# HITRainer/EAVSR

Measured on AMD Instinct MI355X. Metric: SR frames/sec at 4x 7-frame 180x320->720x1280, higher is better.
Workload: dtype f32

## Files before the change

### eavsr_amd/_native.py

```python
from __future__ import annotations

import ctypes as C
import os
import threading

_HERE = os.path.dirname(os.path.abspath(__file__))
LIB_PATH = os.environ.get("EAVSR_LIB_PATH") or os.path.join(
    _HERE, "lib", "libeavsr_lab.so" if os.environ.get("EAVSR_BUILD_LAB", "0") == "1" else "libeavsr_hip.so")

ABI_VERSION = 32

p_f32 = C.c_void_p
i32 = C.c_int32
i64 = C.c_int64
f32 = C.c_float
vp = C.c_void_p


class ConvDesc(C.Structure):
    _fields_ = [
        ("src", vp * 5),
        ("src_c", i32 * 5),
        ("n_src", i32),
        ("ksize", i32),
        ("weight_packed", vp),
        ("bias", vp),
        ("residual", vp),
        ("out", vp),
        ("chan_partial", vp),
        ("n", i32), ("h", i32), ("w", i32), ("cin", i32), ("cout", i32),
        ("act", i32),
        ("slope", f32),
        ("ca_scale", vp),
        ("ca_x", vp),
        ("ca_out", vp),
        ("out_shuffle", i32),
        ("res_scale", vp),
        ("border_pieces", vp),
        ("border_stride", i32),
        ("sum_mul", vp),
    ]


SIGNATURES = {
    "eavsr_abi_version": (C.c_int, []),
    "eavsr_version": (C.c_char_p, []),
    "eavsr_conv2d_desc_size": (C.c_size_t, []),
    "eavsr_lab_build": (C.c_int, []),
    "eavsr_last_error": (C.c_char_p, []),
    "eavsr_selftest_mfma_f32": (C.c_int, [vp, vp]),
    "eavsr_flow_warp_f32": (C.c_int, [vp, vp, vp, vp, i32, i32, i32, i32, i32, i32, vp]),
    "eavsr_flow_warp_pair_f32": (C.c_int, [vp, vp, vp, vp, vp, vp, i32, i32, i32, i32, i32, vp]),
    "eavsr_dcnv2_f32": (C.c_int, [vp, vp, vp, vp, vp, vp, i32, i32, i32, i32, i32, i32, vp]),
    "eavsr_dcnv2_generic_f32": (C.c_int, [vp] * 6 + [i32] * 15 + [vp]),
    "eavsr_dcn_weight_x9_bytes": (C.c_int64, [i32, i32]),
    "eavsr_pack_dcn_weight_x9": (C.c_int, [vp, vp, i32, i32, vp]),
    "eavsr_nchw_to_il8_f32": (C.c_int, [vp, vp, i32, i32, i32, i32, vp]),
    "eavsr_dcnv2_il_f32": (C.c_int, [vp, vp, vp, vp, vp, vp, i32, i32, i32, i32, i32, i32, i32, i32, vp]),
    "eavsr_dcn_weight_il2_bytes": (C.c_int64, [i32, i32]),
    "eavsr_pack_dcn_weight_il2": (C.c_int, [vp, vp, i32, i32, vp]),
    "eavsr_dcnv2_il2_f32": (C.c_int, [vp, vp, vp, vp, vp, vp, i32, i32, i32, i32, i32, i32, i32, i32, vp]),
    "eavsr_dcn_il16_weight_bytes": (C.c_int64, [i32, i32]),
    "eavsr_pack_dcn_il16_weight": (C.c_int, [vp, vp, i32, i32, i32, vp]),
    "eavsr_nchw_to_il8_h16": (C.c_int, [vp, vp, i32, i32, i32, i32, i32, vp]),
    "eavsr_dcnv2_il16": (C.c_int, [vp, vp, vp, vp, vp, vp, i32, i32, i32, i32, i32, i32, i32, i32, vp]),
    "eavsr_wino4_schedule": (C.c_int, []),
    "eavsr_conv3x3_wino4_border_pieces": (C.c_int, [i32, i32, C.POINTER(i32), C.POINTER(i32)]),
    "eavsr_ca_scale_pre_pieces": (C.c_int, [vp, vp, i32, vp, i32, i32, i32, vp, vp, vp, vp, vp, vp, vp, i32, i32, i32, i32, i32, vp]),
    "eavsr_conv2d_f32": (C.c_int, [C.POINTER(ConvDesc), vp]),
    "eavsr_wino4_weight_elems": (C.c_int64, [i32, i32]),
    "eavsr_pack_conv_weight_wino4": (C.c_int, [vp, vp, i32, i32, vp]),
    "eavsr_conv3x3_wino4_tiles": (i32, [i32, i32]),
    "eavsr_conv3x3_wino4_f32": (C.c_int, [vp, vp, vp]),
    "eavsr_wgrad3_mode": (C.c_int, []),
    "eavsr_conv3x3_x6s_tiles": (i32, [i32, i32]),
    "eavsr_conv3x3_f32x6s": (C.c_int, [vp, vp, vp]),
    "eavsr_pack_conv_weight_wino5x5": (C.c_int, [vp, vp, i32, i32, vp]),
    "eavsr_conv5x5_wino_tiles": (i32, [i32, i32]),
    "eavsr_conv5x5_wino_f32": (C.c_int, [vp, vp, vp]),
    "eavsr_conv2d_ck": (i32, [i32]),
    "eavsr_conv2d_tile_rows": (i32, [i32, i32, i32, i32]),
    "eavsr_conv2d_tiles": (i32, [i32, i32, i32, i32]),
    "eavsr_route_batch": (i32, [i32]),
    "eavsr_packed_weight_elems": (i64, [i32, i32, i32]),
    "eavsr_pack_conv_weight_f32": (C.c_int, [vp, vp, i32, i32, i32, vp]),
    "eavsr_conv3x3_smallco_f32": (C.c_int, [vp, vp, vp, vp, vp, i32, i32, i32, i32, i32, i32, f32, vp]),
    "eavsr_smallco_packed_elems": (C.c_int64, [i32, i32]),
    "eavsr_pack_smallco_weight": (C.c_int, [vp, vp, i32, i32, vp]),
    "eavsr_conv3x3_smallco_lite_f32": (C.c_int, [vp, vp, vp, vp, vp, i32, i32, i32, i32, i32, i32, f32, vp]),
    "eavsr_conv_weight_x6_bytes": (C.c_size_t, [i32, i32, i32]),
    "eavsr_pack_conv_weight_x6": (C.c_int, [vp, vp, i32, i32, i32, vp]),
    "eavsr_pack_conv_weight_x6_dgrad": (C.c_int, [vp, vp, i32, i32, i32, vp]),
    "eavsr_pack_conv_weight_x6_multi": (C.c_int, [vp, vp, vp, i32, i32, i32, vp]),
    "eavsr_conv_f32x6": (C.c_int, [vp, vp, vp, vp, i32, i32, i32, i32, i32, i32, i32, f32, i32, vp]),
    "eavsr_ca_scale_f32": (C.c_int, [vp, i32, i32, vp, vp, vp, vp, vp, i32, i32, i32, vp]),
    "eavsr_ca_scale_mean_f32": (C.c_int, [vp, i32, i32, vp, vp, vp, vp, vp, vp, i32, i32, i32, vp]),
    "eavsr_scale_residual_f32": (C.c_int, [vp, vp, vp, vp, i32, i32, i32, vp]),
    "eavsr_ca_tail_f32": (C.c_int, [vp, vp, i32, vp, vp, vp, vp, vp, vp, i32, i32, i32, i32, vp]),
    "eavsr_ca_tail_stats_f32": (C.c_int, [vp, vp, i32, vp, vp, vp, vp, vp, vp, vp, vp, i32, i32, i32, i32, vp]),
    "eavsr_adapt_frontend_f32": (C.c_int, [vp, vp, vp, vp, vp, vp, vp, i32, i32, i32, i32, vp]),
    "eavsr_affine_offsets_f32": (C.c_int, [vp, vp, vp, i32, i32, i32, i32, vp]),
    "eavsr_resize_bilinear_ac_f32": (C.c_int, [vp, vp, vp, vp, i32, i32, i32, i32, i32, i32, f32, vp]),
    "eavsr_pyramid_f32": (C.c_int, [vp, vp, vp, i32, i32, i32, vp]),
    "eavsr_add_f32": (C.c_int, [vp, vp, vp, vp, i64, vp]),
    "eavsr_normalize_f32": (C.c_int, [vp, vp, vp, vp, i32, i32, i32, vp]),
    "eavsr_avg_pool2_f32": (C.c_int, [vp, vp, i32, i32, i32, vp]),
    "eavsr_resize_bilinear_f32": (C.c_int, [vp, vp, i32, i32, i32, i32, i32, i32, i32, f32, f32, vp]),
    "eavsr_concat3_f32": (C.c_int, [vp, i32, vp, i32, vp, i32, vp, i32, i32, vp]),
    "eavsr_act_bwd_f32": (C.c_int, [vp, vp, vp, i64, i32, f32, vp]),
    "eavsr_plane_sum_f32": (C.c_int, [vp, vp, vp, i32, i32, f32, vp]),
    "eavsr_channel_sum_f32": (C.c_int, [vp, vp, i32, i32, i32, i32, vp]),
    "eavsr_channel_sum_multi_f32": (C.c_int, [vp, i32, vp, i32, i32, i32, i32, vp]),
    "eavsr_scale_residual_bwd_f32": (C.c_int, [vp, vp, vp, vp, i32, i32, i32, vp]),
    "eavsr_rcab_tail_bwd_f32": (C.c_int, [vp] * 13 + [i32] * 7 + [vp]),
    "eavsr_ca_mlp_bwd_f32": (C.c_int, [vp] * 11 + [i32, i32, i32, vp]),
    "eavsr_flow_warp_bwd_f32": (C.c_int, [vp] * 6 + [i32, i32, i32, i32, vp]),
    "eavsr_resize_bilinear_ac_bwd_f32": (C.c_int, [vp, vp, i32, i32, i32, i32, i32, i32, f32, vp]),
    "eavsr_pyramid_bwd_f32": (C.c_int, [vp, vp, vp, i32, i32, i32, vp]),
    "eavsr_affine_offsets_bwd_f32": (C.c_int, [vp, vp, vp, vp, i32, i32, i32, i32, vp]),
    "eavsr_conv_wgrad_blocks": (i32, [i32, i32, i32, i32]),
    "eavsr_conv_wgrad_f32": (C.c_int, [vp, vp, vp, vp] + [i32] * 11 + [vp]),
    "eavsr_conv_wgrad_multi_f32": (C.c_int, [vp, vp, i32, vp, vp] + [i32] * 11 + [vp]),
    "eavsr_conv_wgrad_span_f32": (C.c_int, [vp, vp, vp, vp] + [i32] * 9 + [vp]),
# ... 136 lines not shown
```

### eavsr_amd/csrc/common.h

```cpp
#pragma once
#include <hip/hip_runtime.h>
#include <stdint.h>
#include <stddef.h>

#include <mutex>

#include "../../include/eavsr_hip.h"

#ifndef EAVSR_LAB
#define EAVSR_LAB 0
#endif

namespace eavsr {

void set_error(const char* fmt, ...);
void clear_error();
int launch_status(const char* what);

static inline hipStream_t as_stream(void* s) { return reinterpret_cast<hipStream_t>(s); }

static inline int cdiv(int a, int b) { return (a + b - 1) / b; }

constexpr int kMaxDevices = 64;
struct PerDeviceOnce {
  std::once_flag flag[kMaxDevices];
};
static inline int current_device() {
  int d = 0;
  (void)hipGetDevice(&d);
  return (d >= 0 && d < kMaxDevices) ? d : 0;
}

}

#define EAVSR_REQUIRE(cond, code, ...)      \
  do {                                      \
    if (!(cond)) {                          \
      ::eavsr::set_error(__VA_ARGS__);      \
      return (code);                        \
    }                                       \
  } while (0)

typedef float f32x16 __attribute__((ext_vector_type(16)));
typedef float f32x4 __attribute__((ext_vector_type(4)));

#ifdef __HIPCC__
__device__ __forceinline__ int eavsr_xcd_remap(int bid, int nblk) {
  const int q = nblk >> 3, r = nblk & 7;
  const int xcd = bid & 7, pos = bid >> 3;
  const int base = xcd < r ? xcd * (q + 1) : r * (q + 1) + (xcd - r) * q;
  return base + pos;
}
#endif

#ifdef __HIPCC__
__device__ __forceinline__ void eavsr_stagger_priority(int wave) {
#if defined(EAVSR_PRIO_LOW_HALF)
  if (wave < 4) __builtin_amdgcn_s_setprio(3);
#elif !defined(EAVSR_NO_WAVE_PRIO)
  if (wave >= 4) __builtin_amdgcn_s_setprio(3);
#else
  (void)wave;
#endif
}
#endif


#ifdef __HIPCC__
__device__ __forceinline__ float eavsr_sigmoid_fast(float x) { return __builtin_amdgcn_rcpf(1.f + __expf(-x)); }

__device__ __forceinline__ float eavsr_mul_legacy(float a, float b) {
  float r;
  asm("v_mul_legacy_f32 %0, %1, %2" : "=v"(r) : "v"(a), "v"(b));
  return r;
}

__device__ __forceinline__ float eavsr_act(float v, float act_s) {
  const float z = eavsr_mul_legacy(v, act_s);
  return !(v <= 0.f) ? v : z;
}
#endif

#define EAVSR_CONV_TW 32
```

### eavsr_amd/csrc/conv3_h16.hip

```cpp
#include "common.h"

#include <hip/hip_bf16.h>
#include <mutex>

namespace {

typedef const __attribute__((address_space(1))) void* gptr_t;
typedef __attribute__((address_space(3))) void* lptr_t;
typedef unsigned u32x4 __attribute__((ext_vector_type(4)));
typedef __bf16 bf16x8 __attribute__((ext_vector_type(8)));
typedef _Float16 h16x8 __attribute__((ext_vector_type(8)));

constexpr int G_TH = 16, G_TW = 32, G_CO = 64, G_CK = 16;
constexpr int G_IH = G_TH + 2;
constexpr int G_QW = 10;
constexpr int G_IW = G_TW + 2;
constexpr int G_PLANE_B = G_IH * G_IW * 16;
constexpr int G_PATCH_B = 2 * G_PLANE_B;
constexpr int G_W_B = 9 * 2 * G_CO * 16;
constexpr int G_STAGE_B = G_PATCH_B + G_W_B;
constexpr int G_LDS_BYTES = 2 * G_STAGE_B + G_CO * 4;
constexpr int G_UNITS = 2 * G_IH * G_QW;

struct G16Args {
// ... 137 lines not shown
    }
    asm volatile("s_waitcnt vmcnt(0) lgkmcnt(0)" ::: "memory");
    __syncthreads();
  }

  const float act_s = a.act == EAVSR_ACT_NONE ? 1.f : a.act == EAVSR_ACT_RELU ? 0.f : a.slope;
  const int gx = x0 + l31;
  if (gx < w) {
#pragma unroll
    for (int t = 0; t < 2; ++t) {
      const int gy = y0 + 2 * wave + t;
      if (gy < h) {
#pragma unroll
        for (int m = 0; m < 2; ++m)
#pragma unroll
          for (int e = 0; e < 16; ++e) {
            const int co = cot * G_CO + m * 32 + (e & 3) + 8 * (e >> 2) + 4 * half;
            if (co < a.cout) {
              const float v = acc[m][t][e];
              a.out[((size_t)bn * a.cout + co) * plane + (size_t)gy * w + gx] = eavsr_act(v, act_s);
            }
          }
      }
    }
  }
}

template <bool BF16>
__global__ void pack_weight_h16g_kernel(const float* __restrict__ w, unsigned short* __restrict__ p, int cout, int cin, long total) {
  const long i = (long)blockIdx.x * 256 + threadIdx.x;
  if (i >= total) return;
  const int j = (int)(i & 7), co = (int)((i >> 3) & 63), hf = (int)((i >> 9) & 1);
  long r = i >> 10;
  const int tap = (int)(r % 9);
  r /= 9;
  const int nch = cin / G_CK;
  const int ch = (int)(r % nch), cot = (int)(r / nch);
  const int o = cot * G_CO + co, ci = ch * G_CK + hf * 8 + j;
  const float v = o < cout ? w[((size_t)o * cin + ci) * 9 + tap] : 0.f;
  p[i] = BF16 ? __builtin_bit_cast(unsigned short, __float2bfloat16(v)) : __builtin_bit_cast(unsigned short, (_Float16)v);
}

template <bool BF16>
int launch_h16g(const G16Args& a, dim3 grid, hipStream_t st) {
  static eavsr::PerDeviceOnce once_pd;
  const int dev_ = eavsr::current_device();
  static hipError_t attr_err_pd[eavsr::kMaxDevices] = {};
  hipError_t& attr_err = attr_err_pd[dev_];
  std::call_once(once_pd.flag[dev_], [&] {
    attr_err = hipFuncSetAttribute(reinterpret_cast<const void*>(&conv3x3_h16g_kernel<BF16>),
                                   hipFuncAttributeMaxDynamicSharedMemorySize, G_LDS_BYTES);
  });
  if (attr_err != hipSuccess) {
    eavsr::set_error("conv3x3_h16g: hipFuncSetAttribute: %s", hipGetErrorString(attr_err));
    return (int)attr_err;
  }
  hipLaunchKernelGGL(conv3x3_h16g_kernel<BF16>, grid, dim3(512), G_LDS_BYTES, st, a);
  return eavsr::launch_status("conv3x3_h16g");
}

}

extern "C" int64_t eavsr_conv3x3_h16g_weight_bytes(int32_t cout, int32_t cin) {
  if (cout <= 0 || cin <= 0 || cin % G_CK) return -1;
  return (int64_t)eavsr::cdiv(cout, G_CO) * (cin / G_CK) * G_W_B;
}

extern "C" int eavsr_pack_conv3x3_h16g(const float* weight, void* packed, int32_t cout, int32_t cin, int32_t dtype, void* stream) {
  EAVSR_REQUIRE(weight && packed, -1, "pack_conv3x3_h16g: NULL pointer");
  EAVSR_REQUIRE(dtype == 1 || dtype == 2, -1, "pack_conv3x3_h16g: dtype %d (1 = f16, 2 = bf16)", dtype);
  EAVSR_REQUIRE(cout > 0 && cin > 0 && cin % G_CK == 0, -2, "pack_conv3x3_h16g: cin %d must be a multiple of 16", cin);
  const long total = eavsr_conv3x3_h16g_weight_bytes(cout, cin) / 2;
  hipStream_t st = eavsr::as_stream(stream);
  const unsigned blocks = (unsigned)((total + 255) / 256);
  if (dtype == 2) hipLaunchKernelGGL(pack_weight_h16g_kernel<true>, dim3(blocks), dim3(256), 0, st, weight, (unsigned short*)packed, cout, cin, total);
  else hipLaunchKernelGGL(pack_weight_h16g_kernel<false>, dim3(blocks), dim3(256), 0, st, weight, (unsigned short*)packed, cout, cin, total);
  return eavsr::launch_status("pack_conv3x3_h16g");
}

extern "C" int eavsr_conv3x3_h16g_f32(const eavsr_conv2d_desc* d, int32_t dtype, void* stream) {
  EAVSR_REQUIRE(d && d->out && d->weight_packed, -1, "conv3x3_h16g: NULL pointer");
  EAVSR_REQUIRE(dtype == 1 || dtype == 2, -1, "conv3x3_h16g: dtype %d (1 = f16, 2 = bf16)", dtype);
  EAVSR_REQUIRE(d->ksize == 3 && d->n_src >= 1 && d->n_src <= 5, -2, "conv3x3_h16g: 3x3, 1..5 sources");
  EAVSR_REQUIRE(!d->residual && !d->chan_partial && !d->ca_scale && !d->ca_x && !d->ca_out && d->out_shuffle == 0 && !d->res_scale && !d->border_pieces && !d->sum_mul, -2,
                "conv3x3_h16g: plain convolution only (no residual / channel sums / channel-attention prologue / pixel shuffle)");
  EAVSR_REQUIRE(d->n >= 0 && d->h > 0 && d->w > 0 && d->cout > 0 && d->w % 4 == 0, -2, "conv3x3_h16g: bad dims (w %% 4 == 0)");
  int cin = 0;
  G16Args a;
  for (int i = 0; i < 5; ++i) {
    a.src[i] = i < d->n_src ? d->src[i] : nullptr;
    a.src_c[i] = i < d->n_src ? d->src_c[i] : 0;
    if (i < d->n_src) {
      EAVSR_REQUIRE(d->src[i] && d->src_c[i] > 0 && d->src_c[i] % G_CK == 0, -2, "conv3x3_h16g: source %d: %d channels (multiples of 16)", i, d->src_c[i]);
      EAVSR_REQUIRE(((uintptr_t)d->src[i] & 15) == 0, -2, "conv3x3_h16g: sources must be 16-byte aligned");
      cin += d->src_c[i];
    }
  }
  EAVSR_REQUIRE(cin == d->cin, -1, "conv3x3_h16g: cin %d != sum of the sources %d", d->cin, cin);
  if (d->n == 0) return 0;
  a.n_src = d->n_src; a.wp = d->weight_packed; a.bias = d->bias; a.out = d->out;
  a.n = d->n; a.h = d->h; a.w = d->w; a.cin = cin; a.cout = d->cout;
  a.tiles_x = eavsr::cdiv(d->w, G_TW);
  a.tiles_y = eavsr::cdiv(d->h, G_TH);
  a.act = d->act; a.slope = d->slope;
  const long blocks = (long)a.tiles_x * a.tiles_y * d->n;
  EAVSR_REQUIRE(blocks < (1L << 31), -1, "conv3x3_h16g: too many tiles");
  dim3 grid((unsigned)blocks, (unsigned)eavsr::cdiv(d->cout, G_CO));
  return dtype == 2 ? launch_h16g<true>(a, grid, eavsr::as_stream(stream)) : launch_h16g<false>(a, grid, eavsr::as_stream(stream));
}
```

### eavsr_amd/csrc/conv3_x6s.hip

```cpp
#include "common.h"

#include <mutex>

namespace {

typedef const __attribute__((address_space(1))) void* gptr_t;
typedef __attribute__((address_space(3))) void* lptr_t;
typedef unsigned u32x4 __attribute__((ext_vector_type(4)));
typedef __bf16 bf16x8 __attribute__((ext_vector_type(8)));

constexpr int Q_NW = 8, Q_TW = 32, Q_TH = 8;
constexpr int Q_IW = Q_TW + 2, Q_IH = Q_TH + 2, Q_NPIX = Q_IW * Q_IH;
constexpr int Q_PLANE_B = Q_NPIX * 16;
constexpr int Q_KSTEPS = 5;

template <int NCH, int NP> struct QCfg {
  static constexpr int CHUNK_B = NP * Q_PLANE_B;
  static constexpr int SLAB_U4 = Q_KSTEPS * NP * 64;
  static constexpr int PATCH_B = NCH * CHUNK_B;
  static constexpr size_t LDS_BYTES = (size_t)PATCH_B + 2 * (size_t)SLAB_U4 * 16 + 32 * 4 + Q_NW * 32 * 4;
  static_assert(LDS_BYTES <= 160 * 1024, "LDS");
  static_assert(PATCH_B >= Q_NW * 32 * 36 * 4, "the VEC epilogue's transpose tiles live in the patch region");
};

// ... 376 lines not shown
      sum = v;
      a.out[obase + (size_t)cu * plane] = a.act == EAVSR_ACT_RELU_MASK ? (rr[r] > 0.f ? v : 0.f) : v + rr[r];
    }
    if (a.chan_partial) {
      sum += __shfl_xor(sum, 16);
      sum += __shfl_xor(sum, 8);
      sum += __shfl_xor(sum, 4);
      sum += __shfl_xor(sum, 2);
      sum += __shfl_xor(sum, 1);
      if (l31 == 0) s_red[wave * 32 + cu + 4 * kg] = sum;
    }
  }
#ifdef EAVSR_X6S_STAMPS
  Q_STAMP(4);
  asm volatile("s_waitcnt vmcnt(0)" ::: "memory");
  Q_STAMP(5);
  if (tid == 0)
    for (int i = 0; i < 8; ++i) atomicAdd(&g_q_stamps[i], st_acc[i]);
#endif
  if (a.chan_partial) {
    __syncthreads();
    if (tid < 32) {
      const int co = cot * 32 + tid;
      if (co < a.cout) {
        float v = s_red[tid];
#pragma unroll
        for (int k = 1; k < Q_NW; ++k) v += s_red[k * 32 + tid];
        a.chan_partial[((size_t)bn * (a.tiles_x * a.tiles_y) + ty * a.tiles_x + tx) * a.cout + co] = v;
      }
    }
  }
}

template <int NCH, bool VEC, int NP>
int launch_q(const QArgs& a, void* stream, const char* name) {
  using K = QCfg<NCH, NP>;
  static eavsr::PerDeviceOnce once_pd;
  const int dev_ = eavsr::current_device();
  static hipError_t attr_err_pd[eavsr::kMaxDevices] = {};
  hipError_t& attr_err = attr_err_pd[dev_];
  std::call_once(once_pd.flag[dev_], [&] {
    attr_err = hipFuncSetAttribute(reinterpret_cast<const void*>(&conv3x3_x6s_kernel<NCH, VEC, NP>), hipFuncAttributeMaxDynamicSharedMemorySize,
                                   (int)K::LDS_BYTES);
  });
  if (attr_err != hipSuccess) {
    eavsr::set_error("%s: hipFuncSetAttribute(%zu B of LDS): %s", name, K::LDS_BYTES, hipGetErrorString(attr_err));
    return (int)attr_err;
  }
  const long blocks = (long)a.tiles_x * a.tiles_y * a.n;
  EAVSR_REQUIRE(blocks < (1L << 31), -1, "%s: too many tiles", name);
  dim3 grid((unsigned)blocks, eavsr::cdiv(a.cout, 32));
  hipLaunchKernelGGL((conv3x3_x6s_kernel<NCH, VEC, NP>), grid, dim3(64 * Q_NW), K::LDS_BYTES, eavsr::as_stream(stream), a);
  return eavsr::launch_status(name);
}

}

#ifdef EAVSR_X6S_STAMPS
extern "C" int eavsr_debug_x6s_stamps(unsigned long long* host_out, int reset) {
  hipError_t e = hipMemcpyFromSymbol(host_out, HIP_SYMBOL(g_q_stamps), sizeof(unsigned long long) * 8);
  if (e != hipSuccess) return (int)e;
  if (reset) {
    unsigned long long z[8] = {0, 0, 0, 0, 0, 0, 0, 0};
    e = hipMemcpyToSymbol(HIP_SYMBOL(g_q_stamps), z, sizeof(z));
  }
  return (int)e;
}
#endif

extern "C" int32_t eavsr_conv3x3_x6s_tiles(int32_t h, int32_t w) {
  if (h <= 0 || w <= 0) return 0;
  return eavsr::cdiv(h, Q_TH) * eavsr::cdiv(w, Q_TW);
}

namespace {

int q_args(const eavsr_conv2d_desc* d, const void* wpacked, const char* name, QArgs& a, bool& vec) {
  EAVSR_REQUIRE(d && wpacked, -1, "%s: NULL pointer", name);
  EAVSR_REQUIRE(d->ksize == 3 && d->n_src == 1 && d->src_c[0] == d->cin, -2, "%s: one source, 3x3", name);
  EAVSR_REQUIRE(d->cin == 64, -2, "%s: cin %d (64 only; use eavsr_conv2d_f32)", name, d->cin);
  EAVSR_REQUIRE(d->n >= 0 && d->cout > 0 && d->h > 0 && d->w > 0, -1, "%s: bad dims", name);
  if (d->n == 0) return 1;
  EAVSR_REQUIRE(d->src[0] && d->out, -1, "%s: NULL pointer", name);
  EAVSR_REQUIRE(d->ca_scale == nullptr && d->ca_x == nullptr && d->ca_out == nullptr && d->out_shuffle == 0 && d->res_scale == nullptr && d->border_pieces == nullptr, -2,
                "%s: no channel-attention prologue, no pixel-shuffle store", name);
  EAVSR_REQUIRE(d->act >= 0 && d->act <= EAVSR_ACT_RELU_MASK, -1, "%s: act %d", name, d->act);
  EAVSR_REQUIRE(d->act != EAVSR_ACT_LRELU || (d->slope >= 0.f && d->slope <= 1.f), -2,
                "%s: leaky-ReLU slope %g outside [0, 1] (the epilogue evaluates max(v, slope v))", name, (double)d->slope);
  EAVSR_REQUIRE(d->act != EAVSR_ACT_RELU_MASK || (d->residual != nullptr && d->chan_partial == nullptr), -1,
                "%s: EAVSR_ACT_RELU_MASK takes the mask source in `residual` (no channel sums)", name);
  EAVSR_REQUIRE(d->sum_mul == nullptr || d->act != EAVSR_ACT_RELU_MASK, -1, "%s: sum_mul with EAVSR_ACT_RELU_MASK", name);
  EAVSR_REQUIRE((long)d->h * d->w < (1L << 31), -1, "%s: image plane too large for 32-bit pixel offsets", name);
  a.x = d->src[0]; a.wsplit = reinterpret_cast<const u32x4*>(wpacked); a.bias = d->bias; a.residual = d->residual;
  a.out = d->out; a.chan_partial = d->chan_partial; a.sum_mul = d->sum_mul;
  a.n = d->n; a.cout = d->cout; a.h = d->h; a.w = d->w;
  a.tiles_x = eavsr::cdiv(d->w, Q_TW); a.tiles_y = eavsr::cdiv(d->h, Q_TH);
  a.wmt = d->cout > 32 ? 2 : 1;
  a.act = d->act; a.slope = d->slope;
  vec = d->w % 4 == 0 && ((reinterpret_cast<uintptr_t>(a.x) | reinterpret_cast<uintptr_t>(a.out) |
                           reinterpret_cast<uintptr_t>(a.residual)) & 15) == 0;
  EAVSR_REQUIRE(a.sum_mul == nullptr || (a.chan_partial != nullptr && vec && (reinterpret_cast<uintptr_t>(a.sum_mul) & 15) == 0), -2,
                "%s: sum_mul needs chan_partial, w %% 4 == 0 and 16-byte aligned tensors", name);
  return 0;
}

}

extern "C" int eavsr_conv3x3_f32x6s(const eavsr_conv2d_desc* d, const void* weight_x6, void* stream) {
  QArgs a;
  bool vec = false;
  const int rc = q_args(d, weight_x6, "conv3x3_f32x6s", a, vec);
  if (rc) return rc > 0 ? 0 : rc;
#ifdef EAVSR_X6S_NO_VEC
  return launch_q<8, false, 3>(a, stream, "conv3x3_f32x6s");
#endif
  return vec ? launch_q<8, true, 3>(a, stream, "conv3x3_f32x6s") : launch_q<8, false, 3>(a, stream, "conv3x3_f32x6s");
}

extern "C" int eavsr_conv3x3_bf16x1s(const eavsr_conv2d_desc* d, const void* weight_bf16x1, void* stream) {
  QArgs a;
  bool vec = false;
  const int rc = q_args(d, weight_bf16x1, "conv3x3_bf16x1s", a, vec);
  if (rc) return rc > 0 ? 0 : rc;
  return vec ? launch_q<8, true, 1>(a, stream, "conv3x3_bf16x1s") : launch_q<8, false, 1>(a, stream, "conv3x3_bf16x1s");
}
```

### eavsr_amd/csrc/conv_mfma.hip

```cpp
#include "common.h"

#include <atomic>
#include <mutex>

namespace {

struct ConvArgs {
  const float* src[5];
  int src_c[5];
  int n_src;
  const float* wp;
  const float* bias;
  const float* residual;
  float* out;
  float* chan_partial;
  const float* ca_scale;
  const float* ca_x;
  float* ca_out;
  int n, h, w, cin, cout, cin_pad, tiles_x, tiles_y;
  int act;
  float slope;
};

__device__ float g_zero_word[4];
// ... 512 lines not shown
  static hipError_t attr_err_pd[eavsr::kMaxDevices] = {};
  hipError_t& attr_err = attr_err_pd[dev_];
  std::call_once(once, [&] {
    attr_err = hipFuncSetAttribute(reinterpret_cast<const void*>(&conv2d_mfma_kernel<KS, MT, VEC, FUSE, NT_>),
                                   hipFuncAttributeMaxDynamicSharedMemorySize, (int)Cfg::LDS_BYTES);
  });
  if (attr_err != hipSuccess) {
    eavsr::set_error("conv2d: hipFuncSetAttribute(%zu B of LDS): %s", Cfg::LDS_BYTES, hipGetErrorString(attr_err));
    return (int)attr_err;
  }
  hipLaunchKernelGGL((conv2d_mfma_kernel<KS, MT, VEC, FUSE, NT_>), grid, dim3(64 * Cfg::NW), Cfg::LDS_BYTES, st, a);
  return eavsr::launch_status("conv2d");
}

template <int KS, int NT_>
int launch_ks(const ConvArgs& a, dim3 grid, int CO, bool vec, hipStream_t st) {
  if (vec) return CO == 32 ? launch_one<KS, 1, true, false, NT_>(a, grid, st) : launch_one<KS, 2, true, false, NT_>(a, grid, st);
  return CO == 32 ? launch_one<KS, 1, false, false, NT_>(a, grid, st) : launch_one<KS, 2, false, false, NT_>(a, grid, st);
}

std::atomic<int> g_route_batch{0};

inline int tile_rows_of(int n, int h, int w, int ksize) {
  if (ksize == 7) return 4;
  const int routed = g_route_batch.load(std::memory_order_relaxed);
  if (routed > 0) n = routed;
  int best = 4;
  long best_cost = -1;
  for (int nt = 4; nt >= 1; nt >>= 1) {
    const long tiles = (long)n * eavsr::cdiv(h, 8 * nt) * eavsr::cdiv(w, EAVSR_CONV_TW);
    const long rounds = (tiles + 255) / 256;
    const long cost = rounds * (2 * nt + 1);
    if (best_cost < 0 || cost < best_cost) { best_cost = cost; best = nt; }
  }
  return best;
}

template <int KS>
int launch_nt(const ConvArgs& a, dim3 grid, int CO, bool vec, int nt, hipStream_t st) {
  if (nt == 1) return launch_ks<KS, 1>(a, grid, CO, vec, st);
  if (nt == 2) return launch_ks<KS, 2>(a, grid, CO, vec, st);
  return launch_ks<KS, 4>(a, grid, CO, vec, st);
}

}

extern "C" int32_t eavsr_conv2d_ck(int32_t ksize) { return chunk_of(ksize); }

extern "C" int32_t eavsr_route_batch(int32_t n) { return g_route_batch.exchange(n > 0 ? n : 0, std::memory_order_relaxed); }

extern "C" int32_t eavsr_conv2d_tile_rows(int32_t n, int32_t h, int32_t w, int32_t ksize) {
  return 8 * tile_rows_of(n > 0 ? n : 1, h, w, ksize);
}

extern "C" int32_t eavsr_conv2d_tiles(int32_t n, int32_t h, int32_t w, int32_t ksize) {
  return eavsr::cdiv(h, eavsr_conv2d_tile_rows(n, h, w, ksize)) * eavsr::cdiv(w, EAVSR_CONV_TW);
}

extern "C" int64_t eavsr_packed_weight_elems(int32_t cout, int32_t cin, int32_t ksize) {
  if (cout <= 0 || cin <= 0 || !(ksize == 1 || ksize == 3 || ksize == 5 || ksize == 7)) return -1;
  const int CO = co_tile_of(cout), ck = chunk_of(ksize);
  const int64_t cots = eavsr::cdiv(cout, CO), cin_pad = (int64_t)eavsr::cdiv(cin, ck) * ck;
  return cots * cin_pad * ksize * ksize * CO;
}

extern "C" int eavsr_pack_conv_weight_f32(const float* weight, float* packed, int32_t cout, int32_t cin,
                                          int32_t ksize, void* stream) {
  EAVSR_REQUIRE(weight && packed, -1, "pack_conv_weight: NULL pointer");
  const int64_t total = eavsr_packed_weight_elems(cout, cin, ksize);
  EAVSR_REQUIRE(total > 0, -1, "pack_conv_weight: bad shape cout=%d cin=%d k=%d", cout, cin, ksize);
  const int CO = co_tile_of(cout), ck = chunk_of(ksize);
  const int cin_pad = eavsr::cdiv(cin, ck) * ck;
  hipLaunchKernelGGL(pack_weight_kernel, dim3((unsigned)((total + 255) / 256)), dim3(256), 0,
                     eavsr::as_stream(stream), weight, packed, cout, cin, ksize * ksize, cin_pad, CO, (long)total);
  return eavsr::launch_status("pack_conv_weight");
}

extern "C" int eavsr_conv2d_f32(const eavsr_conv2d_desc* d, void* stream) {
  EAVSR_REQUIRE(d != nullptr, -1, "conv2d: NULL descriptor");
  EAVSR_REQUIRE(d->n_src >= 1 && d->n_src <= 5, -1, "conv2d: n_src %d not in 1..5", d->n_src);
  EAVSR_REQUIRE(d->ksize == 1 || d->ksize == 3 || d->ksize == 5 || d->ksize == 7, -2,
                "conv2d: kernel size %d unsupported (1,3,5,7)", d->ksize);
  EAVSR_REQUIRE(d->weight_packed && d->out, -1, "conv2d: NULL weight/out");
  EAVSR_REQUIRE(d->out_shuffle == 0 && d->res_scale == nullptr && d->border_pieces == nullptr && d->sum_mul == nullptr, -2, "conv2d: the pixel-shuffle and scaled-residual epilogues exist in eavsr_conv3x3_wino4_f32 only");
  EAVSR_REQUIRE(d->n >= 0 && d->h > 0 && d->w > 0 && d->cin > 0 && d->cout > 0, -1, "conv2d: bad dims");
  EAVSR_REQUIRE(d->act >= 0 && d->act <= EAVSR_ACT_RELU_MASK, -1, "conv2d: act %d", d->act);
  EAVSR_REQUIRE(d->act != EAVSR_ACT_RELU_MASK || (d->residual != nullptr && d->chan_partial == nullptr && d->ca_scale == nullptr), -1,
                "conv2d: EAVSR_ACT_RELU_MASK takes the mask source in `residual` (no channel sums, no fused prologue)");
  EAVSR_REQUIRE(d->act != EAVSR_ACT_LRELU || (d->slope >= 0.f && d->slope <= 1.f), -2,
                "conv2d: leaky-ReLU slope %g outside [0, 1] (the epilogue evaluates max(v, slope v))", (double)d->slope);
  const int ck = chunk_of(d->ksize);
  ConvArgs a;
  int csum = 0;
  for (int s = 0; s < 5; ++s) {
    a.src[s] = s < d->n_src ? d->src[s] : nullptr;
    a.src_c[s] = s < d->n_src ? d->src_c[s] : 0;
    if (s < d->n_src) {
      EAVSR_REQUIRE(d->src[s] != nullptr && d->src_c[s] > 0, -1, "conv2d: source %d is empty", s);
      EAVSR_REQUIRE(s == d->n_src - 1 || d->src_c[s] % ck == 0, -2,
                    "conv2d: source %d has %d channels, not a multiple of %d (only the last may be ragged)", s,
                    d->src_c[s], ck);
      csum += d->src_c[s];
    }
  }
  EAVSR_REQUIRE(csum == d->cin, -1, "conv2d: sources sum to %d channels, cin = %d", csum, d->cin);
  if (d->n == 0) return 0;
  const int CO = co_tile_of(d->cout);
  a.n_src = d->n_src;
  a.wp = d->weight_packed;
  a.bias = d->bias;
  a.residual = d->residual;
  a.out = d->out;
  a.chan_partial = d->chan_partial;
  a.ca_scale = d->ca_scale;
  a.ca_x = d->ca_x;
  a.ca_out = d->ca_out;
  a.n = d->n; a.h = d->h; a.w = d->w; a.cin = d->cin; a.cout = d->cout;
  a.cin_pad = eavsr::cdiv(d->cin, ck) * ck;
  const int nt = tile_rows_of(d->n, d->h, d->w, d->ksize);
  a.tiles_x = eavsr::cdiv(d->w, EAVSR_CONV_TW);
  a.tiles_y = eavsr::cdiv(d->h, 8 * nt);
  a.act = d->act;
  a.slope = d->slope;
  const long blocks = (long)a.tiles_x * a.tiles_y * d->n;
  EAVSR_REQUIRE(blocks < (1L << 31), -1, "conv2d: too many tiles");
  EAVSR_REQUIRE((long)d->h * d->w * 16 < (1L << 31), -1, "conv2d: image plane too large for 32-bit tile offsets");
  dim3 grid((unsigned)blocks, eavsr::cdiv(d->cout, CO));
  hipStream_t st = eavsr::as_stream(stream);
  bool vec = (d->w % 4) == 0;
  for (int s = 0; s < d->n_src; ++s)
    vec = vec && (((uintptr_t)d->src[s]) & 15) == 0 && (d->src_c[s] % ck) == 0;
  if (d->ca_scale != nullptr) {
    EAVSR_REQUIRE(d->ca_x != nullptr, -1, "conv2d: ca_scale without ca_x");
    EAVSR_REQUIRE(d->ksize == 3 && d->n_src == 1 && vec && (((uintptr_t)d->ca_x) & 15) == 0 && d->cin % 4 == 0 &&
                      d->cin <= 256 && CO == 64 && d->cout <= 64,
                  -2, "conv2d: the fused channel-attention prologue needs a single 16-byte aligned source, k = 3, "
                      "w %% 4 == 0, cin %% 4 == 0, cin <= 256 and 33..64 output channels; use eavsr_scale_residual_f32 + "
                      "a plain conv otherwise");
    EAVSR_REQUIRE(nt == 4, -2, "conv2d: the fused channel-attention prologue exists for the 32-row tile only "
                               "(this problem size runs %d-row tiles)", 8 * nt);
    return launch_one<3, 2, true, true>(a, grid, st);
  }
  EAVSR_REQUIRE(d->ca_x == nullptr && d->ca_out == nullptr, -1, "conv2d: ca_x / ca_out without ca_scale");
  switch (d->ksize) {
    case 1: return launch_nt<1>(a, grid, CO, vec, nt, st);
    case 3:
      if (nt == 1 && vec) {
        if (CO == 32) return launch_small<1>(a, grid, st);
        if (blocks * grid.y <= 128) return launch_small<1, true>(a, grid, st);
        return launch_small<2>(a, grid, st);
      }
      return launch_nt<3>(a, grid, CO, vec, nt, st);
    case 5: return launch_nt<5>(a, grid, CO, vec, nt, st);
    default: return launch_ks<7, 4>(a, grid, CO, vec, st);
  }
}
```

### eavsr_amd/csrc/conv_wino.hip

```cpp
#include "common.h"

#include <mutex>

namespace {

typedef const __attribute__((address_space(1))) void* gptr_t;
typedef __attribute__((address_space(3))) void* lptr_t;
typedef float f32x2 __attribute__((ext_vector_type(2)));

__device__ __attribute__((aligned(16))) float g_wino_zero[4];

struct WnArgs {
  const float* src[5];
  int src_c[5];
  int n_src;
  const float* wu;
  const float* bias;
  const float* residual;
  float* out;
  float* chan_partial;
  const float* ca_scale;
  const float* ca_x;
  float* ca_out;
  int n, h, w, cin, cout, tiles_x, tiles_y;
// ... 291 lines not shown
    }
    if (a.chan_partial) {
      __syncthreads();
#pragma unroll
      for (int r = 0; r < 4; ++r) {
        float v = csum[r];
        v += __shfl_xor(v, 8);
        v += __shfl_xor(v, 4);
        v += __shfl_xor(v, 2);
        v += __shfl_xor(v, 1);
        if (l15 == 0) s_red[(wave & 1) * 64 + cb * 16 + 4 * kq + r] = v;
      }
      __syncthreads();
      if (tid < 64) {
        const int co = cot * 64 + tid;
        if (co < a.cout)
          a.chan_partial[((size_t)bn * (a.tiles_x * a.tiles_y) + tile_lin) * a.cout + co] = s_red[tid] + s_red[64 + tid];
      }
    }
#pragma unroll
    for (int b = 0; b < 2; ++b)
#pragma unroll
      for (int x = 0; x < 16; ++x) acc[b][x] = f32x4{0.f, 0.f, 0.f, 0.f};
    if (it + 1 < total_iters) {
      tile_coords((it + 1) / total_chunks, bn, y0, x0, tile_lin);
      if (FUSE) {
        for (int c = tid; c < a.cin; c += 64 * NW) s_y[c] = a.ca_scale[(size_t)bn * a.cin + c];
      }
    }
  }
  }
}


__global__ void pack_wino_kernel(const float* __restrict__ wt, float* __restrict__ out, int cout, int cin, long total) {
  const long e = (long)blockIdx.x * 256 + threadIdx.x;
  if (e >= total) return;
  const int col = (int)(e & 63);
  long u = e >> 6;
  const int c = (int)(u % CK); u /= CK;
  const int xi = (int)(u % 16); u /= 16;
  const int nchunks = cin / CK;
  const int chunk = (int)(u % nchunks);
  const int cot = (int)(u / nchunks);
  const int co = cot * 64 + col, ci = chunk * CK + c;
  float v = 0.f;
  if (co < cout) {
    const float* g = wt + ((size_t)co * cin + ci) * 9;
    const int r = xi >> 2, q = xi & 3;
    float gr[3];
#pragma unroll
    for (int j = 0; j < 3; ++j) {
      const float g0 = g[0 * 3 + j], g1 = g[1 * 3 + j], g2 = g[2 * 3 + j];
      gr[j] = r == 0 ? g0 : (r == 1 ? 0.5f * (g0 + g1 + g2) : (r == 2 ? 0.5f * (g0 - g1 + g2) : g2));
    }
    v = q == 0 ? gr[0] : (q == 1 ? 0.5f * (gr[0] + gr[1] + gr[2]) : (q == 2 ? 0.5f * (gr[0] - gr[1] + gr[2]) : gr[2]));
  }
  out[e - col + (col ^ ((c & 1) << 4))] = v;
}

}

extern "C" int64_t eavsr_wino_weight_elems(int32_t cout, int32_t cin) {
  if (cout <= 0 || cin <= 0 || cin % CK != 0) return 0;
  return (int64_t)eavsr::cdiv(cout, 64) * (cin / CK) * UV;
}

extern "C" int eavsr_pack_conv_weight_wino(const float* weight, float* packed, int32_t cout, int32_t cin, void* stream) {
  EAVSR_REQUIRE(weight && packed, -1, "pack_conv_weight_wino: NULL pointer");
  EAVSR_REQUIRE(cout > 0 && cin > 0 && cin % CK == 0, -1, "pack_conv_weight_wino: cin %d must be a multiple of 8", cin);
  const long total = eavsr_wino_weight_elems(cout, cin);
  hipLaunchKernelGGL(pack_wino_kernel, dim3((unsigned)((total + 255) / 256)), dim3(256), 0, eavsr::as_stream(stream), weight, packed,
                     cout, cin, total);
  return eavsr::launch_status("pack_conv_weight_wino");
}

extern "C" int32_t eavsr_conv3x3_wino_tiles(int32_t h, int32_t w) { return eavsr::cdiv(h, TOH) * eavsr::cdiv(w, TOW); }

extern "C" int eavsr_conv3x3_wino_f32(const eavsr_conv2d_desc* d, const float* weight_wino, void* stream) {
  EAVSR_REQUIRE(d != nullptr && weight_wino != nullptr, -1, "conv3x3_wino: NULL descriptor / weights");
  EAVSR_REQUIRE(d->n_src >= 1 && d->n_src <= 5, -1, "conv3x3_wino: n_src %d not in 1..5", d->n_src);
  EAVSR_REQUIRE(d->ksize == 3, -2, "conv3x3_wino: kernel size %d (3 only)", d->ksize);
  EAVSR_REQUIRE(d->out, -1, "conv3x3_wino: NULL out");
  EAVSR_REQUIRE(d->out_shuffle == 0 && d->res_scale == nullptr && d->border_pieces == nullptr && d->sum_mul == nullptr, -2, "conv3x3_wino: the pixel-shuffle and scaled-residual epilogues exist in eavsr_conv3x3_wino4_f32 only");
  EAVSR_REQUIRE(d->n >= 0 && d->h > 0 && d->w > 0 && d->cin > 0 && d->cout > 0, -1, "conv3x3_wino: bad dims");
  EAVSR_REQUIRE(d->act >= 0 && d->act <= 2, -1, "conv3x3_wino: act %d", d->act);
  EAVSR_REQUIRE(d->act != EAVSR_ACT_LRELU || (d->slope >= 0.f && d->slope <= 1.f), -2,
                "conv3x3_wino: leaky-ReLU slope %g outside [0, 1] (the epilogue evaluates max(v, slope v))", (double)d->slope);
  const bool fuse = d->ca_scale != nullptr;
  if (fuse) {
    EAVSR_REQUIRE(d->ca_x != nullptr, -1, "conv3x3_wino: ca_scale without ca_x");
    EAVSR_REQUIRE(d->n_src == 1 && d->cin <= F_MAXC && (((uintptr_t)d->ca_x) & 15) == 0 &&
                      (d->ca_out == nullptr || (((uintptr_t)d->ca_out) & 7) == 0), -2,
                  "conv3x3_wino: the fused channel-attention prologue needs a single source, cin <= %d and aligned ca_x / "
                  "ca_out", F_MAXC);
  } else {
    EAVSR_REQUIRE(d->ca_x == nullptr && d->ca_out == nullptr, -1, "conv3x3_wino: ca_x / ca_out without ca_scale");
  }
  EAVSR_REQUIRE(d->w % 4 == 0, -2, "conv3x3_wino: w %% 4 != 0 (use eavsr_conv2d_f32)");
  EAVSR_REQUIRE((((uintptr_t)d->out) & 7) == 0 && (d->residual == nullptr || (((uintptr_t)d->residual) & 7) == 0), -2,
                "conv3x3_wino: out / residual must be 8-byte aligned");
  WnArgs a;
  int csum = 0;
  for (int s = 0; s < 5; ++s) {
    a.src[s] = s < d->n_src ? d->src[s] : nullptr;
    a.src_c[s] = s < d->n_src ? d->src_c[s] : 0;
    if (s < d->n_src) {
      EAVSR_REQUIRE(d->src[s] != nullptr && d->src_c[s] > 0 && d->src_c[s] % CK == 0 && (((uintptr_t)d->src[s]) & 15) == 0, -2,
                    "conv3x3_wino: source %d must be 16-byte aligned with a multiple of 8 channels", s);
      csum += d->src_c[s];
    }
  }
  EAVSR_REQUIRE(csum == d->cin, -1, "conv3x3_wino: sources sum to %d channels, cin = %d", csum, d->cin);
  if (d->n == 0) return 0;
  a.n_src = d->n_src;
  a.wu = weight_wino;
  a.bias = d->bias; a.residual = d->residual; a.out = d->out; a.chan_partial = d->chan_partial;
  a.ca_scale = d->ca_scale; a.ca_x = d->ca_x; a.ca_out = d->ca_out;
  a.n = d->n; a.h = d->h; a.w = d->w; a.cin = d->cin; a.cout = d->cout;
  a.tiles_x = eavsr::cdiv(d->w, TOW);
  a.tiles_y = eavsr::cdiv(d->h, TOH);
  a.act = d->act; a.slope = d->slope;
  const long blocks = (long)a.tiles_x * a.tiles_y * d->n;
  EAVSR_REQUIRE(blocks < (1L << 31), -1, "conv3x3_wino: too many tiles");
  EAVSR_REQUIRE((long)d->h * d->w * 16 < (1L << 31), -1, "conv3x3_wino: image plane too large for 32-bit tile offsets");
  static eavsr::PerDeviceOnce once_pd;
  const int dev_ = eavsr::current_device();
  std::once_flag& once = once_pd.flag[dev_];
  static hipError_t attr_err_pd[eavsr::kMaxDevices] = {};
  hipError_t& attr_err = attr_err_pd[dev_];
  std::call_once(once, [&] {
    attr_err = hipFuncSetAttribute(reinterpret_cast<const void*>(&conv3x3_wino_kernel<false>),
                                   hipFuncAttributeMaxDynamicSharedMemorySize, (int)LDS_BYTES);
    if (attr_err == hipSuccess)
      attr_err = hipFuncSetAttribute(reinterpret_cast<const void*>(&conv3x3_wino_kernel<true>),
                                     hipFuncAttributeMaxDynamicSharedMemorySize, (int)F_LDS_BYTES);
  });
  if (attr_err != hipSuccess) {
    eavsr::set_error("conv3x3_wino: hipFuncSetAttribute(%zu B of LDS): %s", LDS_BYTES, hipGetErrorString(attr_err));
    return (int)attr_err;
  }
  const long per_cot = blocks < 256 ? blocks : 256;
  dim3 grid((unsigned)per_cot, eavsr::cdiv(d->cout, 64));
  if (fuse) hipLaunchKernelGGL(conv3x3_wino_kernel<true>, grid, dim3(64 * NW), F_LDS_BYTES, eavsr::as_stream(stream), a);
  else hipLaunchKernelGGL(conv3x3_wino_kernel<false>, grid, dim3(64 * NW), LDS_BYTES, eavsr::as_stream(stream), a);
  return eavsr::launch_status("conv3x3_wino");
}
```

### eavsr_amd/csrc/conv_wino6.hip

```cpp
#include "common.h"

#ifdef EAVSR_W4_REG_WEIGHTS
#define EAVSR_W4_UREGS 1
#endif
#ifndef EAVSR_W4_ROUND2_DUTY
#define EAVSR_W4_DUTY_NO_U 1
#define EAVSR_W4_DUTYPRIO 1
#endif

#include <mutex>
#include <type_traits>
#include <cstdlib>
#include <cstring>

namespace {

static bool w6_grouped_schedule() {
#ifdef EAVSR_W4_NOGRP
  return false;
#else
  static const bool on = [] { const char* e = getenv("EAVSR_W4_GRP"); return e == nullptr || atoi(e) != 0; }();
  return on;
#endif
}

typedef const __attribute__((address_space(1))) void* gptr_t;
typedef __attribute__((address_space(3))) void* lptr_t;
typedef float f32x2 __attribute__((ext_vector_type(2)));

__device__ __attribute__((aligned(16))) float g_wino4_zero[4];

typedef __amdgpu_buffer_rsrc_t w6_rsrc;
constexpr unsigned W6_OOB = 0x80000000u;
__device__ __forceinline__ w6_rsrc w6_make_rsrc(const void* base, unsigned bytes) {
  return __builtin_amdgcn_make_buffer_rsrc(const_cast<void*>(base), 0, (int)bytes, 0x00020000);
}
__device__ __forceinline__ f32x4 w6_ld4(w6_rsrc r, unsigned voff, unsigned soff) {
  return __builtin_bit_cast(f32x4, __builtin_amdgcn_raw_buffer_load_b128(r, voff, soff, 0));
}
__device__ __forceinline__ void w6_st4(w6_rsrc r, unsigned voff, unsigned off, f32x4 v) {
  typedef unsigned u32x4_t __attribute__((ext_vector_type(4)));
  __builtin_amdgcn_raw_buffer_store_b128(__builtin_bit_cast(u32x4_t, v), r, voff + off, 0, 0);
}

struct W4Args {
  const float* src[5];
  int src_c[5];
  int n_src;
  const float* wu;
  const float* bias;
  const float* residual;
  float* out;
  float* chan_partial;
  const float* ca_scale;
  const float* ca_x;
  float* ca_out;
  int n, h, w, cin, cout, tiles_x, tiles_y;
  int act;
  float slope;
  int out_shuffle;
  const float* res_scale;
  float* border;
  int border_stride;
};

constexpr int CK = 4, NW = 8, NPOS = 36;
constexpr int MARG = 4;
constexpr int U_ELEMS = NPOS * CK * 64;
constexpr int U_SEGS = U_ELEMS / 256;
constexpr int U_IT = (U_SEGS + NW - 1) / NW;
constexpr int V_ELEMS = NPOS * CK * 32;

__host__ __device__ constexpr int w6_pair_of(int q) { return (q == 1 || q == 2) ? 0 : (q == 3 || q == 4) ? 1 : 2; }
__host__ __device__ constexpr int w6_half_of(int q) { return (q == 1 || q == 3 || q == 0) ? 0 : 1; }
__host__ __device__ constexpr int w6_slot(int i, int q) { return 2 * (3 * i + w6_pair_of(q)) + w6_half_of(q); }
__host__ __device__ constexpr int w6_col_of(int pp, int half) { return pp == 0 ? 1 + half : pp == 1 ? 3 + half : (half ? 5 : 0); }

template <int R>
struct WCfg {
  static_assert(R == 3 || R == 5, "F(4x4,3x3) or F(2x2,5x5)");
  static constexpr int M = 7 - R, PADR = R / 2;
  static constexpr int TOH = 2 * M, TOW = 16 * M;
  static constexpr int IH = TOH + 2 * PADR, IW = TOW + 2 * MARG;
  static constexpr int IN_ELEMS = CK * IH * IW;
  static constexpr int IN_SEGS = (IN_ELEMS / 4 + 63) / 64;
  static constexpr int IN_PAD = IN_SEGS * 256;
  static constexpr int IN_IT = (IN_SEGS + NW - 1) / NW;
  static constexpr int OFF_U = 2 * IN_PAD;
  static constexpr int OFF_V = OFF_U + 2 * U_ELEMS;
  static constexpr int LDS_MAIN = OFF_V + 2 * V_ELEMS;
#ifdef EAVSR_W4_ITSTAMP
  static constexpr int LDS_FLOATS = LDS_MAIN + 128 + 512;
#else
  static constexpr int LDS_FLOATS = LDS_MAIN + 128;
#endif
  static constexpr size_t LDS_BYTES = (size_t)LDS_FLOATS * sizeof(float);
};

template <typename T>
__device__ __forceinline__ void in1d(const T (&d)[6], T (&t)[6]) {
  const T a = d[4] - 4.f * d[2];
  const T b = d[3] - 4.f * d[1];
  const T c = d[4] - d[2];
  const T e = d[3] - d[1];
  t[0] = 4.f * d[0] + (d[4] - 5.f * d[2]);
  t[1] = a + b;
  t[2] = a - b;
  t[3] = c + 2.f * e;
  t[4] = c - 2.f * e;
  t[5] = 4.f * d[1] + (d[5] - 5.f * d[3]);
}

__device__ __forceinline__ void out1d(const float (&m)[6], float (&s)[4]) {
  const float p1 = m[1] + m[2], p2 = m[1] - m[2], p3 = m[3] + m[4], p4 = m[3] - m[4];
  s[0] = m[0] + p1 + p3;
  s[1] = p2 + 2.f * p4;
  s[2] = p1 + 4.f * p3;
  s[3] = (p2 + 8.f * p4) + m[5];
}

#ifdef EAVSR_W4_STAMPS
__device__ unsigned long long g_w4_stamps[32];
#define W4_STAMP(i)                                                   \
  do {                                                                \
    const unsigned long long t_ = __builtin_amdgcn_s_memtime();       \
    st_acc[i] += t_ - st_last;                                        \
    st_last = t_;                                                     \
  } while (0)
#else
#define W4_STAMP(i) do { } while (0)
#endif

#ifdef EAVSR_W4_TIMELINE
__device__ unsigned long long g_w4_tl[512 * 16];
#define W4_TL(i)                                                                           \
  do {                                                                                     \
    if (tid == 0) {                                                                        \
      g_w4_tl[(blockIdx.y * gridDim.x + blockIdx.x) * 16 + 2 * (i)] = __builtin_amdgcn_s_memrealtime(); \
      g_w4_tl[(blockIdx.y * gridDim.x + blockIdx.x) * 16 + 2 * (i) + 1] = __builtin_amdgcn_s_memtime(); \
    }                                                                                      \
  } while (0)
#else
#define W4_TL(i) do { } while (0)
#endif

#ifdef EAVSR_W4_ITSTAMP
__device__ unsigned long long g_w4_it[256 * 256];
#define W4_IT(i)                                                                                       \
  do {                                                                                                 \
    if (it >= 8 && it < 12 && lane == 0) s_its[((it - 8) * 8 + wave) * 8 + (i)] = __builtin_amdgcn_s_memtime(); \
  } while (0)
#else
#define W4_IT(i) do { } while (0)
#endif

template <int R, bool FUSE = false, bool GRP = false, bool RSC = false>
__global__ __launch_bounds__(512, 2) void conv_wino6_kernel(W4Args a) {
  static_assert(!RSC || (GRP && R == 3 && !FUSE), "the scaled-residual epilogue exists for the grouped 3x3 kernel");
  static_assert(!FUSE || R == 3, "the fused channel-attention prologue exists for the 3x3 kernel");
  static_assert(!GRP || (R == 3 && !FUSE), "the grouped schedule exists for the plain 3x3 kernel");
  using C = WCfg<R>;
  constexpr int M = C::M, PADR = C::PADR, TOH = C::TOH, TOW = C::TOW, IH = C::IH, IW = C::IW, IN_ELEMS = C::IN_ELEMS;
  constexpr int IN_SEGS = C::IN_SEGS, IN_PAD = C::IN_PAD, IN_IT = C::IN_IT;
  constexpr int X_OFF = 2 * IN_PAD;
  constexpr int OFF_U = C::OFF_U + (FUSE ? 2 * IN_PAD : 0), OFF_V = C::OFF_V + (FUSE ? 2 * IN_PAD : 0);
  constexpr int LDS_MAIN = C::LDS_MAIN + (FUSE ? 2 * IN_PAD : 0);
  extern __shared__ __attribute__((aligned(16))) float smem[];
  float* s_v = smem + OFF_V;
  float* s_red = smem + LDS_MAIN;
#ifdef EAVSR_W4_ITSTAMP
  unsigned long long* s_its = reinterpret_cast<unsigned long long*>(smem + LDS_MAIN + 128);
#endif

  const int tid = threadIdx.x;
  const int lane = tid & 63;
  const int wave = __builtin_amdgcn_readfirstlane(tid >> 6);
  W4_TL(0);
#ifndef EAVSR_W4_UREGS
  {
    const char* usrc0 = reinterpret_cast<const char*>(a.wu + (size_t)blockIdx.y * (a.cin / CK) * U_ELEMS) + wave * 1024;
#pragma unroll
    for (int i = 0; i < U_IT; ++i) {
      const int seg = i * NW + wave;
      if (seg < U_SEGS)
        __builtin_amdgcn_global_load_lds((gptr_t)(usrc0 + i * (NW * 1024) + (tid & 63) * 16u), (lptr_t)(smem + OFF_U + seg * 256), 16, 0, 0);
    }
  }
#endif

  const int cot = blockIdx.y;
  const int h = a.h, w = a.w;
  const size_t plane = (size_t)h * w;
  const int total_tiles = a.tiles_x * a.tiles_y * a.n;
  const int my_tiles = (total_tiles - (int)blockIdx.x + (int)gridDim.x - 1) / (int)gridDim.x;
  const unsigned u_tx = (unsigned)a.tiles_x, u_ty = (unsigned)a.tiles_y;
  auto tile_coords = [&](int k, int& bn_, int& y0_, int& x0_, int& lin_) __attribute__((always_inline)) {
    unsigned t = (unsigned)eavsr_xcd_remap((int)blockIdx.x + k * (int)gridDim.x, total_tiles);
    const unsigned q1 = t / u_tx;
    const unsigned tx_ = t - q1 * u_tx;
    const unsigned q2 = q1 / u_ty;
    const unsigned ty_ = q1 - q2 * u_ty;
    bn_ = (int)q2;
    y0_ = (int)ty_ * TOH;
    x0_ = (int)tx_ * TOW;
    lin_ = (int)(ty_ * u_tx + tx_);
  };

  const int l15 = lane & 15, kq = lane >> 4;
  const unsigned lane16 = lane * 16u;
  const int cb = wave >> 1, tg = wave & 1;
  eavsr_stagger_priority(wave);
#ifdef EAVSR_W4_DUTYPRIO
  if (wave >= 4) __builtin_amdgcn_s_setprio(1);
#endif
  float bias_r[4];
#pragma unroll
  for (int r = 0; r < 4; ++r) {
    const int co = cot * 64 + cb * 16 + 4 * kq + r;
    bias_r[r] = (co < a.cout && a.bias != nullptr) ? a.bias[co] : 0.f;
  }
  f32x4 acc[NPOS];
#pragma unroll
  for (int x = 0; x < NPOS; ++x) acc[x] = f32x4{0.f, 0.f, 0.f, 0.f};
  const float act_s = a.act == EAVSR_ACT_NONE ? 1.f : a.act == EAVSR_ACT_RELU ? 0.f : a.slope;

  int total_chunks = 0;
  for (int s = 0; s < a.n_src; ++s) total_chunks += a.src_c[s] / CK;
  const int total_iters = my_tiles * total_chunks;

  int p_k = 0, p_cs = 0, p_cc0 = 0, p_bn = 0, p_y0 = 0, p_x0 = 0, p_lin = 0;
  unsigned voff[IN_IT];
  auto p_setup_lanes = [&]() __attribute__((always_inline)) {
#pragma unroll
    for (int i = 0; i < IN_IT; ++i) {
      const int seg = i * NW + wave;
      const int e4 = seg * 64 + lane;
      const int ci = e4 / (IH * (IW / 4));
      const int rem = e4 - ci * (IH * (IW / 4));
      const int r = rem / (IW / 4);
      const int c4 = rem - r * (IW / 4);
// ... 150 lines not shown
        for (int r = 0; r < 6; ++r) d[r] = f32x2{q[r][0], q[r][1]};
        in1d(d, t12);
#pragma unroll
        for (int r = 0; r < 6; ++r) d[r] = f32x2{q[r][2], q[r][3]};
        in1d(d, t34);
      }
      {
        f32x2 d[6];
        if constexpr (HAND_READS) {
          asm volatile("s_waitcnt lgkmcnt(0)" : "+v"(e05[0]), "+v"(e05[1]), "+v"(e05[2]), "+v"(e05[3]), "+v"(e05[4]), "+v"(e05[5]));
#pragma unroll
          for (int r = 0; r < 6; ++r) d[r] = e05[r];
        } else {
#pragma unroll
          for (int r = 0; r < 6; ++r) d[r] = f32x2{pp[r * IW + 3], pp[r * IW + 8]};
        }
        if (FUSE) {
#pragma unroll
          for (int r = 0; r < 6; ++r) {
            d[r].x = fmaf(d[r].x, sc_use, pp[X_OFF + r * IW + 3]);
            d[r].y = fmaf(d[r].y, sc_use, pp[X_OFF + r * IW + 8]);
          }
        }
        in1d(d, t05);
      }
    } else {
      const float* pp = smem + ps * IN_PAD + kq * (IH * IW) + (M * tg) * IW + (MARG - PADR) + 2 * l15;
      f32x2 d[6];
#pragma unroll
      for (int r = 0; r < 6; ++r) d[r] = *reinterpret_cast<const f32x2*>(pp + r * IW);
      in1d(d, t05);
#pragma unroll
      for (int r = 0; r < 6; ++r) d[r] = *reinterpret_cast<const f32x2*>(pp + r * IW + 2);
      in1d(d, t12);
#pragma unroll
      for (int r = 0; r < 6; ++r) d[r] = *reinterpret_cast<const f32x2*>(pp + r * IW + 4);
      in1d(d, t34);
    }
#pragma unroll
    for (int i = 0; i < 6; ++i) {
      f32x2 o12, o34, o05;
      if (R == 3) {
        const f32x2 ba = t34[i] - 4.f * t12[i];
        const f32x2 ec = t34[i] - t12[i];
        asm("v_pk_add_f32 %0, %1, %1 op_sel:[1,0] op_sel_hi:[1,0] neg_hi:[0,1]" : "=v"(o12) : "v"(ba));
        asm("v_pk_fma_f32 %0, %1, 2.0, %1 op_sel:[0,0,1] op_sel_hi:[0,0,1] neg_hi:[1,0,0]" : "=v"(o34) : "v"(ec));
        o05 = f32x2{4.f * t05[i].x + (t34[i].y - 5.f * t12[i].y), 4.f * t12[i].x + (t05[i].y - 5.f * t34[i].x)};
      } else {
        const float d5[6] = {t05[i].x, t05[i].y, t12[i].x, t12[i].y, t34[i].x, t34[i].y};
        float o[6];
        in1d(d5, o);
        o12 = f32x2{o[1], o[2]};
        o34 = f32x2{o[3], o[4]};
        o05 = f32x2{o[0], o[5]};
      }
      *reinterpret_cast<f32x2*>(vd + (i * 3 + 0) * (CK * 64)) = o12;
      *reinterpret_cast<f32x2*>(vd + (i * 3 + 1) * (CK * 64)) = o34;
      *reinterpret_cast<f32x2*>(vd + (i * 3 + 2) * (CK * 64)) = o05;
    }
#endif
  };

#ifdef EAVSR_W4_STAMPS
  unsigned long long st_acc[8] = {0, 0, 0, 0, 0, 0, 0, 0};
  unsigned long long st_last = __builtin_amdgcn_s_memtime();
#endif
  issue_patch(0);
  const float sc_first = sc_next;
#ifdef EAVSR_W4_UREGS
  const __amdgpu_buffer_rsrc_t u_rsrc = __builtin_amdgcn_make_buffer_rsrc(
      const_cast<float*>(wu_base), 0, (int)((size_t)(a.cin / CK) * U_ELEMS * sizeof(float)), 0x00020000);
  const int lane_uoff = (kq * 128 + 2 * ((cb * 16 + l15) ^ ((kq & 1) << 4))) * 4;
  typedef unsigned u32x2_t __attribute__((ext_vector_type(2)));
  auto load_u = [&](int soff, int i) __attribute__((always_inline)) {
    const u32x2_t t = __builtin_amdgcn_raw_buffer_load_b64(u_rsrc, lane_uoff, soff + i * (CK * 128 * 4), 0);
    return __builtin_bit_cast(f32x2, t);
  };
  f32x2 ur[NPOS / 2];
#pragma unroll
  for (int i = 0; i < NPOS / 2; ++i) ur[i] = load_u(0, i);
#endif
  if (total_iters > 1) issue_patch(1);
  W4_TL(1);
  if constexpr (!GRP) {
    asm volatile("s_waitcnt vmcnt(0)" ::: "memory");
    __syncthreads();
    W4_TL(2);
    if ((wave >> 1) == 3) { sc_use = sc_first; transform(0, 0, bn, y0, x0, 0); }
  }
  sc_use = sc_next;
  int chunk = 0;
  W4_STAMP(0);
  for (int it = 0; it < total_iters; ++it) {
    W4_IT(0);
#ifdef EAVSR_W4_UREGS
    __builtin_amdgcn_s_waitcnt(0x0F70);
#else
    asm volatile("s_waitcnt vmcnt(0)" ::: "memory");
#endif
    W4_STAMP(1);
    W4_IT(1);
    __syncthreads();
    W4_IT(2);
    W4_STAMP(2);
    const int chunk_n = chunk + 1 == total_chunks ? 0 : chunk + 1;
    const bool on_duty = !GRP && (wave >> 1) == (it & 3);
    if constexpr (GRP) {
      if (it == 0) W4_TL(2);
      if ((it & 1) == 0) {
        if (wave < 4) {
          transform(wave >> 1, wave >> 1, bn, y0, x0, chunk + (wave >> 1));
        } else {
#if !defined(EAVSR_WINO_EXP_NODMA) && !defined(EAVSR_WINO_EXP_NOUDMA)
          const int rank = wave - 4;
          float* s_u = smem + OFF_U + U_ELEMS;
          const char* usrc = reinterpret_cast<const char*>(wu_base + (size_t)chunk_n * U_ELEMS) + rank * 1024;
#pragma unroll
          for (int i = 0; i < U_SEGS / 4; ++i)
            __builtin_amdgcn_global_load_lds((gptr_t)(usrc + i * (4 * 1024) + lane16), (lptr_t)(s_u + (i * 4 + rank) * 256), 16, 0, 0);
#endif
        }
        asm volatile("s_waitcnt lgkmcnt(0)" ::: "memory");
        __builtin_amdgcn_s_barrier();
      }
    }
    auto issue_dma = [&]() __attribute__((always_inline)) {
      if constexpr (GRP) {
#ifndef EAVSR_WINO_EXP_NODMA
        if ((it & 1) == 0) {
          if (it + 2 < total_iters) { issue_patch(0); issue_patch(1); }
        } else {
#ifndef EAVSR_WINO_EXP_NOUDMA
          if (it + 1 < total_iters) issue_u(chunk_n, 0);
#endif
        }
#endif
        return;
      }
#ifndef EAVSR_WINO_EXP_NODMA
#if !defined(EAVSR_WINO_EXP_NOUDMA) && !defined(EAVSR_W4_UREGS)
#ifdef EAVSR_W4_DUTY_NO_U
      if (it + 1 < total_iters && !on_duty) {
        const int rank = wave < 2 * (it & 3) ? wave : wave - 2;
        float* s_u = smem + OFF_U + ((it + 1) & 1) * U_ELEMS;
        const char* usrc = reinterpret_cast<const char*>(wu_base + (size_t)chunk_n * U_ELEMS) + rank * 1024;
#pragma unroll
        for (int i = 0; i < U_SEGS / 6; ++i)
          __builtin_amdgcn_global_load_lds((gptr_t)(usrc + i * (6 * 1024) + lane16), (lptr_t)(s_u + (i * 6 + rank) * 256), 16, 0, 0);
      }
#else
      if (it + 1 < total_iters) issue_u(chunk_n, (it + 1) & 1);
#endif
#endif
      if (it + 2 < total_iters) issue_patch(it & 1);
#endif
    };
    const bool dma_late = wave >= 4;
#ifndef EAVSR_W4_SPREAD
#ifdef EAVSR_W4_DUTY_NO_U
    if (!dma_late && !on_duty) issue_dma();
#else
    if (!dma_late) issue_dma();
#endif
#endif
    W4_IT(3);
    W4_STAMP(3);
// ... 78 lines not shown
      bv[i] = *reinterpret_cast<const f32x2*>(vb + i * (CK * 64));
    }
#ifndef EAVSR_WINO_EXP_NOMFMA
#pragma unroll
    for (int i = 0; i < NSTEP; ++i) {
#ifdef EAVSR_W4_SPREAD
#ifndef EAVSR_W4_SPREAD_STRIDE
#define EAVSR_W4_SPREAD_STRIDE 1
#endif
      constexpr int SS = EAVSR_W4_SPREAD_STRIDE;
      if (!FUSE && i % SS == SS - 1 && i / SS < U_IT + IN_IT) {
        constexpr int dummy_ = 0; (void)dummy_;
        const int k = i / SS;
        __builtin_amdgcn_sched_barrier(0);
        if (k < U_IT) { if (it + 1 < total_iters) issue_u_piece(k, chunk_n, (it + 1) & 1); }
        else if (it + 2 < total_iters) {
          issue_patch_piece(k - U_IT, it & 1);
          if (k == U_IT + IN_IT - 1) patch_advance();
        }
        __builtin_amdgcn_sched_barrier(0);
      }
      if (FUSE && i == NSTEP / 2) {
        __builtin_amdgcn_sched_barrier(0);
        issue_dma();
        __builtin_amdgcn_sched_barrier(0);
      }
#else
      if (i == NSTEP / 2) {
        __builtin_amdgcn_sched_barrier(0);
        W4_IT(5);
        if (dma_late) issue_dma();
        W4_IT(6);
        __builtin_amdgcn_sched_barrier(0);
      }
#endif
      if (i + AHEAD < NSTEP) {
#if defined(EAVSR_W4_UREGS)
#elif defined(EAVSR_WINO_EXP_UREGS)
        av[(i + AHEAD) % (AHEAD + 1)] = f32x2{bias_r[(i + AHEAD) & 3], bias_r[i & 3]};
#else
        av[(i + AHEAD) % (AHEAD + 1)] = *reinterpret_cast<const f32x2*>(ua + (i + AHEAD) * (CK * 128));
#endif
        bv[(i + AHEAD) % (AHEAD + 1)] = *reinterpret_cast<const f32x2*>(vb + (i + AHEAD) * (CK * 64));
      }
      const int cur = i % (AHEAD + 1);
#ifdef EAVSR_W4_UREGS
      acc[2 * i] = __builtin_amdgcn_mfma_f32_16x16x4f32(ur[i].x, bv[cur].x, acc[2 * i], 0, 0, 0);
      acc[2 * i + 1] = __builtin_amdgcn_mfma_f32_16x16x4f32(ur[i].y, bv[cur].y, acc[2 * i + 1], 0, 0, 0);
      ur[i] = load_u(u_next, i);
      __builtin_amdgcn_sched_group_barrier(0x100, 1, 0);
      __builtin_amdgcn_sched_group_barrier(0x008, 2, 0);
      __builtin_amdgcn_sched_group_barrier(0x020, 1, 0);
    }
#else
      acc[2 * i] = __builtin_amdgcn_mfma_f32_16x16x4f32(av[cur].x, bv[cur].x, acc[2 * i], 0, 0, 0);
      acc[2 * i + 1] = __builtin_amdgcn_mfma_f32_16x16x4f32(av[cur].y, bv[cur].y, acc[2 * i + 1], 0, 0, 0);
#ifdef EAVSR_WINO_EXP_UREGS
      __builtin_amdgcn_sched_group_barrier(0x100, 1, 0);
#else
      __builtin_amdgcn_sched_group_barrier(0x100, 2, 0);
#endif
      __builtin_amdgcn_sched_group_barrier(0x008, 2, 0);
    }
#endif
#else
    if (dma_late) issue_dma();
    acc[0][0] += av[0].x + bv[0].x;
#endif
#endif
#ifdef EAVSR_W4_UREGS
    __builtin_amdgcn_sched_barrier(0);
    duty_transform();
#endif
    if (FUSE) sc_use = sc_next;
    chunk = chunk_n;
    W4_IT(7);
    W4_STAMP(5);
    if (chunk != 0) continue;
    if (it + 1 == total_iters) W4_TL(3);

    {
      float csum[4] = {0.f, 0.f, 0.f, 0.f};
      constexpr bool fast_done = GRP;
      if constexpr (GRP) {
       {
        const int gx = x0 + 4 * l15;
        const int gy0 = y0 + 4 * tg;
        const int rows = h - gy0;
        const int cblk = a.cout - cot * 64 < 64 ? a.cout - cot * 64 : 64;
        const size_t img_off = ((size_t)bn * a.cout + (size_t)cot * 64) * plane;
        const unsigned blk_bytes = (unsigned)((size_t)cblk * plane * sizeof(float));
        const w6_rsrc r_out = w6_make_rsrc(a.out + img_off, blk_bytes);
        const bool has_res = a.residual != nullptr;
        const w6_rsrc r_res = w6_make_rsrc(has_res ? a.residual + img_off : a.out + img_off, blk_bytes);
        const unsigned lane_off = gx < w ? (unsigned)((((size_t)(cb * 16 + 4 * kq)) * plane + (size_t)gy0 * w + gx) * sizeof(float)) : W6_OOB;
        const unsigned plane_b = (unsigned)(plane * sizeof(float)), row_b = (unsigned)(w * sizeof(float));
        const bool shuf = a.out_shuffle == 2;
        const unsigned lane_off_ps = gx < w ? (unsigned)((((size_t)(cb * 4 + kq)) * 4 * plane + (size_t)(2 * gy0) * (2 * w) + 2 * gx) * sizeof(float)) : W6_OOB;
        const bool has_act = a.act != EAVSR_ACT_NONE;
        float sc4[4] = {1.f, 1.f, 1.f, 1.f};
        if constexpr (RSC) {
#pragma unroll
          for (int r = 0; r < 4; ++r) {
            const int co = cot * 64 + cb * 16 + 4 * kq + r;
            sc4[r] = co < a.cout ? a.res_scale[(size_t)bn * a.cout + co] : 0.f;
          }
        }
        f32x4 rr[2][2] = {{f32x4{0.f, 0.f, 0.f, 0.f}, f32x4{0.f, 0.f, 0.f, 0.f}}, {f32x4{0.f, 0.f, 0.f, 0.f}, f32x4{0.f, 0.f, 0.f, 0.f}}};
        auto load_rr = [&](int step) __attribute__((always_inline)) {
#pragma unroll
          for (int ch = 0; ch < 2; ++ch)
            rr[step & 1][ch] = w6_ld4(r_res, lane_off, (unsigned)(2 * (step >> 2) + ch) * plane_b + (unsigned)(step & 3) * row_b);
        };
        if (has_res) load_rr(0);
        f32x2 cs2[4] = {f32x2{0.f, 0.f}, f32x2{0.f, 0.f}, f32x2{0.f, 0.f}, f32x2{0.f, 0.f}};
        const bool b_tile = !RSC && a.border != nullptr && (y0 == 0 || y0 + TOH >= h || x0 == 0 || x0 + TOW >= w);
        float btop[4] = {0.f, 0.f, 0.f, 0.f}, bbot[4] = {0.f, 0.f, 0.f, 0.f}, blft[4] = {0.f, 0.f, 0.f, 0.f}, brgt[4] = {0.f, 0.f, 0.f, 0.f};
#pragma unroll
        for (int rp = 0; rp < 2; ++rp) {
          const f32x2 b2 = f32x2{bias_r[2 * rp], bias_r[2 * rp + 1]};
#pragma unroll
          for (int dy = 0; dy < 4; ++dy) {
            __builtin_amdgcn_sched_barrier(0);
            const int step = 4 * rp + dy;
            if (has_res && step < 7) load_rr(step + 1);
            f32x2 sq[6];
#pragma unroll
            for (int q = 0; q < 6; ++q) {
              f32x2 m[6];
#pragma unroll
              for (int i = 0; i < 6; ++i) m[i] = f32x2{acc[w6_slot(i, q)][2 * rp], acc[w6_slot(i, q)][2 * rp + 1]};
              if (dy == 0) sq[q] = m[0] + (m[1] + m[2]) + (m[3] + m[4]);
              else if (dy == 1) sq[q] = (m[1] - m[2]) + 2.f * (m[3] - m[4]);
              else if (dy == 2) sq[q] = (m[1] + m[2]) + 4.f * (m[3] + m[4]);
              else sq[q] = ((m[1] - m[2]) + 8.f * (m[3] - m[4])) + m[5];
            }
            const f32x2 p1 = sq[1] + sq[2], p2 = sq[1] - sq[2], p3 = sq[3] + sq[4], p4 = sq[3] - sq[4];
            f32x2 y[4];
            y[0] = (sq[0] + p1 + p3) + b2;
            y[1] = (p2 + 2.f * p4) + b2;
            y[2] = (p1 + 4.f * p3) + b2;
            y[3] = ((p2 + 8.f * p4) + sq[5]) + b2;
            f32x4 vc[2];
            if (!RSC || has_act) {
#pragma unroll
              for (int ch = 0; ch < 2; ++ch)
#pragma unroll
                for (int j = 0; j < 4; ++j) vc[ch][j] = eavsr_act(ch == 0 ? y[j].x : y[j].y, act_s);
            } else {
#pragma unroll
              for (int ch = 0; ch < 2; ++ch)
#pragma unroll
                for (int j = 0; j < 4; ++j) vc[ch][j] = ch == 0 ? y[j].x : y[j].y;
            }
            if (!RSC && shuf) {
              if (dy < rows) {
                const unsigned so = (unsigned)(2 * dy + rp) * (2 * row_b);
                w6_st4(r_out, lane_off_ps, so, f32x4{vc[0][0], vc[1][0], vc[0][1], vc[1][1]});
                w6_st4(r_out, lane_off_ps, so + 16u, f32x4{vc[0][2], vc[1][2], vc[0][3], vc[1][3]});
              }
            } else {
#pragma unroll
              for (int ch = 0; ch < 2; ++ch) {
                const int r = 2 * rp + ch;
                const f32x4 v = vc[ch];
                f32x4 o;
#pragma unroll
                for (int j = 0; j < 4; ++j) o[j] = __builtin_fmaf(v[j], sc4[r], rr[step & 1][ch][j]);
                if (dy < rows) {
                  if constexpr (!RSC) {
                    const f32x2 h2 = f32x2{v[0], v[1]} + f32x2{v[2], v[3]};
                    cs2[r] += h2;
                    if (b_tile) {
                      if (gy0 + dy == 0) btop[r] += h2.x + h2.y;
                      if (gy0 + dy == h - 1) bbot[r] += h2.x + h2.y;
                      blft[r] += v[0];
                      brgt[r] += v[3];
                    }
                  }
                  w6_st4(r_out, lane_off, (unsigned)r * plane_b + (unsigned)dy * row_b, o);
                }
              }
            }
          }
        }
#pragma unroll
        for (int r = 0; r < 4; ++r) {
          const int co = cot * 64 + cb * 16 + 4 * kq + r;
          csum[r] = (co < a.cout && gx < w) ? cs2[r].x + cs2[r].y : 0.f;
        }
        if constexpr (!RSC) {
          if (b_tile) {
            const int txi = x0 / TOW, tyi = y0 / TOH;
            float* bp = a.border + (size_t)bn * 4 * a.border_stride * 64 + cb * 16 + 4 * kq;
            const bool has_top = gy0 == 0 && rows > 0, has_bot = gy0 <= h - 1 && h - 1 < gy0 + M;
            if (has_top || has_bot) {
#pragma unroll
              for (int r = 0; r < 4; ++r) {
                float vt = gx < w ? btop[r] : 0.f, vb = gx < w ? bbot[r] : 0.f;
                vt += __shfl_xor(vt, 8); vb += __shfl_xor(vb, 8);
                vt += __shfl_xor(vt, 4); vb += __shfl_xor(vb, 4);
                vt += __shfl_xor(vt, 2); vb += __shfl_xor(vb, 2);
                vt += __shfl_xor(vt, 1); vb += __shfl_xor(vb, 1);
                if (l15 == 0) {
                  if (has_top) bp[(size_t)(0 * a.border_stride + txi) * 64 + r] = vt;
                  if (has_bot) bp[(size_t)(1 * a.border_stride + txi) * 64 + r] = vb;
                }
              }
            }
            if (x0 == 0 && l15 == 0) {
#pragma unroll
              for (int r = 0; r < 4; ++r) bp[(size_t)(2 * a.border_stride + 2 * tyi + tg) * 64 + r] = blft[r];
            }
            if (x0 + TOW >= w && gx == w - 4) {
#pragma unroll
              for (int r = 0; r < 4; ++r) bp[(size_t)(3 * a.border_stride + 2 * tyi + tg) * 64 + r] = brgt[r];
            }
          }
        }
       }
      }
      if constexpr (fast_done) {
      } else if constexpr (R == 3) {
        const int gx = x0 + 4 * l15;
#pragma unroll
        for (int rp = 0; rp < 2; ++rp) {
          const int co0 = cot * 64 + cb * 16 + 4 * kq + 2 * rp;
#pragma unroll
          for (int dy = 0; dy < 4; ++dy) {
            __builtin_amdgcn_sched_barrier(0);
            const int gy = y0 + 4 * tg + dy;
            const bool pok = gy < h && gx < w;
            f32x4 rr[2];
#pragma unroll
            for (int ch = 0; ch < 2; ++ch) {
              rr[ch] = f32x4{0.f, 0.f, 0.f, 0.f};
              if (a.residual != nullptr && co0 + ch < a.cout && pok)
                rr[ch] = *reinterpret_cast<const f32x4*>(a.residual + ((size_t)bn * a.cout + co0 + ch) * plane + (size_t)gy * w + gx);
            }
            f32x2 s[6];
#pragma unroll
            for (int q = 0; q < 6; ++q) {
              f32x2 m[6];
#pragma unroll
              for (int i = 0; i < 6; ++i) m[i] = f32x2{acc[w6_slot(i, q)][2 * rp], acc[w6_slot(i, q)][2 * rp + 1]};
              if (dy == 0) s[q] = m[0] + (m[1] + m[2]) + (m[3] + m[4]);
              else if (dy == 1) s[q] = (m[1] - m[2]) + 2.f * (m[3] - m[4]);
              else if (dy == 2) s[q] = (m[1] + m[2]) + 4.f * (m[3] + m[4]);
              else s[q] = ((m[1] - m[2]) + 8.f * (m[3] - m[4])) + m[5];
            }
            const f32x2 p1 = s[1] + s[2], p2 = s[1] - s[2], p3 = s[3] + s[4], p4 = s[3] - s[4];
            f32x2 y[4];
            y[0] = s[0] + p1 + p3;
            y[1] = p2 + 2.f * p4;
            y[2] = p1 + 4.f * p3;
            y[3] = (p2 + 8.f * p4) + s[5];
            float vv[2][4];
#pragma unroll
            for (int ch = 0; ch < 2; ++ch) {
              const int r = 2 * rp + ch;
#pragma unroll
              for (int j = 0; j < 4; ++j) {
                float t = (ch == 0 ? y[j].x : y[j].y) + bias_r[r];
                t = eavsr_act(t, act_s);
                vv[ch][j] = t;
              }
            }
            if (a.out_shuffle == 2) {
              if (co0 + 1 < a.cout && pok) {
                float* o = a.out + ((size_t)bn * (a.cout >> 2) + (co0 >> 2)) * (4 * plane) + (size_t)(2 * gy + rp) * (2 * w) + 2 * gx;
                *reinterpret_cast<f32x4*>(o) = f32x4{vv[0][0], vv[1][0], vv[0][1], vv[1][1]};
                *reinterpret_cast<f32x4*>(o + 4) = f32x4{vv[0][2], vv[1][2], vv[0][3], vv[1][3]};
              }
            } else {
#pragma unroll
              for (int ch = 0; ch < 2; ++ch) {
                const int r = 2 * rp + ch, co = co0 + ch;
                if (co < a.cout && pok) {
                  csum[r] += (vv[ch][0] + vv[ch][1]) + (vv[ch][2] + vv[ch][3]);
                  if constexpr (RSC) {
                    const float sc = a.res_scale[(size_t)bn * a.cout + co];
                    *reinterpret_cast<f32x4*>(a.out + ((size_t)bn * a.cout + co) * plane + (size_t)gy * w + gx) =
                        f32x4{vv[ch][0] * sc + rr[ch][0], vv[ch][1] * sc + rr[ch][1], vv[ch][2] * sc + rr[ch][2], vv[ch][3] * sc + rr[ch][3]};
                  } else {
                    *reinterpret_cast<f32x4*>(a.out + ((size_t)bn * a.cout + co) * plane + (size_t)gy * w + gx) =
                        f32x4{vv[ch][0] + rr[ch][0], vv[ch][1] + rr[ch][1], vv[ch][2] + rr[ch][2], vv[ch][3] + rr[ch][3]};
                  }
                }
              }
            }
          }
        }
      } else {
        const int gx = x0 + 2 * l15;
#pragma unroll
        for (int r = 0; r < 4; ++r) {
          const int co = cot * 64 + cb * 16 + 4 * kq + r;
          const bool cok = co < a.cout;
          const float bb = bias_r[r];
          __builtin_amdgcn_sched_barrier(0);
          f32x2 rr[2];
#pragma unroll
          for (int dy = 0; dy < 2; ++dy) {
            const int gy = y0 + 2 * tg + dy;
            rr[dy] = f32x2{0.f, 0.f};
            if (a.residual != nullptr && cok && gy < h && gx < w)
              rr[dy] = *reinterpret_cast<const f32x2*>(a.residual + ((size_t)bn * a.cout + co) * plane + (size_t)gy * w + gx);
          }
          float s[2][6];
#pragma unroll
          for (int q = 0; q < 6; ++q) {
            const float m0 = acc[w6_slot(0, q)][r], m1 = acc[w6_slot(1, q)][r], m2 = acc[w6_slot(2, q)][r], m3 = acc[w6_slot(3, q)][r],
                        m4 = acc[w6_slot(4, q)][r], m5 = acc[w6_slot(5, q)][r];
            s[0][q] = m0 + (m1 + m2) + (m3 + m4);
            s[1][q] = ((m1 - m2) + 2.f * (m3 - m4)) + m5;
          }
#pragma unroll
          for (int dy = 0; dy < 2; ++dy) {
            float y[2];
            y[0] = s[dy][0] + (s[dy][1] + s[dy][2]) + (s[dy][3] + s[dy][4]);
            y[1] = ((s[dy][1] - s[dy][2]) + 2.f * (s[dy][3] - s[dy][4])) + s[dy][5];
            const int gy = y0 + 2 * tg + dy;
#pragma unroll
            for (int j = 0; j < 2; ++j) {
              y[j] += bb;
              y[j] = eavsr_act(y[j], act_s);
            }
            if (cok && gy < h && gx < w) {
              csum[r] += y[0] + y[1];
              *reinterpret_cast<f32x2*>(a.out + ((size_t)bn * a.cout + co) * plane + (size_t)gy * w + gx) =
                  f32x2{y[0] + rr[dy].x, y[1] + rr[dy].y};
            }
          }
        }
      }
      if (a.chan_partial) {
        __syncthreads();
#pragma unroll
        for (int r = 0; r < 4; ++r) {
          float v = csum[r];
          v += __shfl_xor(v, 8);
          v += __shfl_xor(v, 4);
          v += __shfl_xor(v, 2);
          v += __shfl_xor(v, 1);
          if (l15 == 0) s_red[tg * 64 + cb * 16 + 4 * kq + r] = v;
        }
        __syncthreads();
        if (tid < 64) {
          const int co = cot * 64 + tid;
          if (co < a.cout)
            a.chan_partial[((size_t)bn * (a.tiles_x * a.tiles_y) + tile_lin) * a.cout + co] = s_red[tid] + s_red[64 + tid];
        }
      }
#pragma unroll
      for (int x = 0; x < NPOS; ++x) acc[x] = f32x4{0.f, 0.f, 0.f, 0.f};
      if (it + 1 < total_iters) tile_coords((it + 1) / total_chunks, bn, y0, x0, tile_lin);
    }
    W4_STAMP(6);
  }
  W4_TL(4);
#ifdef EAVSR_W4_ITSTAMP
  __syncthreads();
  if (tid < 256) g_w4_it[(blockIdx.y * gridDim.x + blockIdx.x) * 256 + tid] = s_its[tid];
#endif
#ifdef EAVSR_W4_TIMELINE
  asm volatile("s_waitcnt vmcnt(0)" ::: "memory");
  W4_TL(5);
#endif
#ifdef EAVSR_W4_STAMPS
  if (lane == 0 && (wave & 1) == 0) {
    for (int i = 0; i < 8; ++i) atomicAdd(&g_w4_stamps[(wave >> 1) * 8 + i], st_acc[i]);
  }
#endif
}

template <int R>
__global__ void pack_wino6_kernel(const float* __restrict__ wt, float* __restrict__ out, int cout, int cin, long total) {
  const long e = (long)blockIdx.x * 256 + threadIdx.x;
  if (e >= total) return;
  const int lo = (int)(e & 1);
  const int colsw = (int)((e >> 1) & 63);
  long u = e >> 7;
  const int c = (int)(u % CK); u /= CK;
  const int pair = (int)(u % (NPOS / 2)); u /= NPOS / 2;
  const int xi = 6 * (pair / 3) + w6_col_of(pair % 3, lo);
  const int col = colsw ^ ((c & 1) << 4);
  const int nchunks = cin / CK;
  const int chunk = (int)(u % nchunks);
  const int cot = (int)(u / nchunks);
  const int co = cot * 64 + col, ci = chunk * CK + c;
  float v = 0.f;
  if (co < cout) {
    const float* g = wt + ((size_t)co * cin + ci) * (R * R);
    const int r = xi / 6, q = xi - 6 * r;
    const double pt[5] = {0., 1., -1., 2., -2.}, sc[5] = {0.25, -1. / 6, -1. / 6, 1. / 24, 1. / 24};
    double Gr[R], Gq[R];
#pragma unroll
    for (int k = 0; k < R; ++k) {
      double pr = 1., pq = 1.;
      for (int e2 = 0; e2 < k; ++e2) { pr *= pt[r < 5 ? r : 0]; pq *= pt[q < 5 ? q : 0]; }
      Gr[k] = r < 5 ? sc[r] * pr : (k == R - 1 ? 1. : 0.);
      Gq[k] = q < 5 ? sc[q] * pq : (k == R - 1 ? 1. : 0.);
    }
    double s = 0.;
#pragma unroll
    for (int i = 0; i < R; ++i)
#pragma unroll
      for (int j = 0; j < R; ++j) s += Gr[i] * (double)g[i * R + j] * Gq[j];
    v = (float)s;
  }
  out[e] = v;
}

}

#ifdef EAVSR_W4_STAMPS
extern "C" int eavsr_debug_w4_stamps(unsigned long long* host_out, int reset) {
  hipDeviceSynchronize();
  hipMemcpyFromSymbol(host_out, HIP_SYMBOL(g_w4_stamps), sizeof(g_w4_stamps));
  if (reset) {
    unsigned long long z[32] = {0};
    hipMemcpyToSymbol(HIP_SYMBOL(g_w4_stamps), z, sizeof(z));
  }
  return 0;
}
#endif

#ifdef EAVSR_W4_ITSTAMP
extern "C" int eavsr_debug_w4_itstamps(unsigned long long* host_out) {
  hipDeviceSynchronize();
  hipMemcpyFromSymbol(host_out, HIP_SYMBOL(g_w4_it), sizeof(g_w4_it));
  return 0;
}
#endif

#ifdef EAVSR_W4_TIMELINE
extern "C" int eavsr_debug_w4_timeline(unsigned long long* host_out) {
  hipDeviceSynchronize();
  hipMemcpyFromSymbol(host_out, HIP_SYMBOL(g_w4_tl), sizeof(g_w4_tl));
  return 0;
}
#endif

extern "C" int64_t eavsr_wino4_weight_elems(int32_t cout, int32_t cin) {
  if (cout <= 0 || cin <= 0 || cin % CK != 0) return 0;
  return (int64_t)eavsr::cdiv(cout, 64) * (cin / CK) * U_ELEMS;
}

namespace {

template <int R>
int pack_wino6(const float* weight, float* packed, int32_t cout, int32_t cin, void* stream) {
  EAVSR_REQUIRE(weight && packed, -1, "pack_conv_weight_wino: NULL pointer");
  EAVSR_REQUIRE(cout > 0 && cin > 0 && cin % CK == 0, -1, "pack_conv_weight_wino: cin %d must be a multiple of 4", cin);
  const long total = eavsr_wino4_weight_elems(cout, cin);
  hipLaunchKernelGGL(pack_wino6_kernel<R>, dim3((unsigned)((total + 255) / 256)), dim3(256), 0, eavsr::as_stream(stream),
                     weight, packed, cout, cin, total);
  return eavsr::launch_status("pack_conv_weight_wino");
}

template <int R>
int launch_wino6(const eavsr_conv2d_desc* d, const float* weight_wino, void* stream) {
  using C = WCfg<R>;
  EAVSR_REQUIRE(d != nullptr && weight_wino != nullptr, -1, "conv_wino6: NULL descriptor / weights");
  EAVSR_REQUIRE(d->n_src >= 1 && d->n_src <= 5, -1, "conv_wino6: n_src %d not in 1..5", d->n_src);
  EAVSR_REQUIRE(d->ksize == R, -2, "conv_wino6: kernel size %d (this entry point: %d)", d->ksize, R);
  EAVSR_REQUIRE(d->out, -1, "conv_wino6: NULL out");
  EAVSR_REQUIRE(d->n >= 0 && d->h > 0 && d->w > 0 && d->cin > 0 && d->cout > 0, -1, "conv_wino6: bad dims");
  EAVSR_REQUIRE(d->act >= 0 && d->act <= 2, -1, "conv_wino6: act %d", d->act);
  EAVSR_REQUIRE(d->act != EAVSR_ACT_LRELU || (d->slope >= 0.f && d->slope <= 1.f), -2,
                "conv_wino6: leaky-ReLU slope %g outside [0, 1] (the epilogue evaluates max(t, slope t))", (double)d->slope);
  const bool fuse = d->ca_scale != nullptr;
#if !EAVSR_LAB
  EAVSR_REQUIRE(!fuse, -2, "conv_wino6: the fused channel-attention prologue is a lab-build instantiation (python -m eavsr_amd.build --lab); "
                           "use eavsr_scale_residual_f32 + a plain convolution, or desc.res_scale on the previous convolution");
#endif
  if (fuse) {
    EAVSR_REQUIRE(R == 3, -2, "conv_wino6: the fused channel-attention prologue exists for the 3x3 kernel only");
    EAVSR_REQUIRE(d->ca_x != nullptr, -1, "conv_wino6: ca_scale without ca_x");
    EAVSR_REQUIRE(d->n_src == 1 && (((uintptr_t)d->ca_x) & 15) == 0 && (d->ca_out == nullptr || (((uintptr_t)d->ca_out) & 15) == 0),
                  -2, "conv_wino6: the fused channel-attention prologue needs a single source and 16-byte aligned ca_x / ca_out");
  } else {
    EAVSR_REQUIRE(d->ca_x == nullptr && d->ca_out == nullptr, -1, "conv_wino6: ca_x / ca_out without ca_scale");
  }
  EAVSR_REQUIRE(d->w % 4 == 0, -2, "conv_wino6: w %% 4 != 0 (use eavsr_conv2d_f32)");
  constexpr uintptr_t AL = R == 3 ? 15 : 7;
  EAVSR_REQUIRE((((uintptr_t)d->out) & AL) == 0 && (d->residual == nullptr || (((uintptr_t)d->residual) & AL) == 0), -2,
                "conv_wino6: out / residual must be %d-byte aligned", (int)AL + 1);
  W4Args a;
  int csum = 0;
  for (int s = 0; s < 5; ++s) {
    a.src[s] = s < d->n_src ? d->src[s] : nullptr;
    a.src_c[s] = s < d->n_src ? d->src_c[s] : 0;
    if (s < d->n_src) {
      EAVSR_REQUIRE(d->src[s] != nullptr && d->src_c[s] > 0 && d->src_c[s] % CK == 0 && (((uintptr_t)d->src[s]) & 15) == 0, -2,
                    "conv_wino6: source %d must be 16-byte aligned with a multiple of 4 channels", s);
      csum += d->src_c[s];
    }
  }
  EAVSR_REQUIRE(csum == d->cin, -1, "conv_wino6: sources sum to %d channels, cin = %d", csum, d->cin);
  if (d->n == 0) return 0;
  a.n_src = d->n_src;
  a.wu = weight_wino;
  a.bias = d->bias; a.residual = d->residual; a.out = d->out; a.chan_partial = d->chan_partial;
  a.ca_scale = d->ca_scale; a.ca_x = d->ca_x; a.ca_out = d->ca_out;
  a.n = d->n; a.h = d->h; a.w = d->w; a.cin = d->cin; a.cout = d->cout;
  a.tiles_x = eavsr::cdiv(d->w, C::TOW);
  a.tiles_y = eavsr::cdiv(d->h, C::TOH);
  a.act = d->act; a.slope = d->slope;
  a.out_shuffle = d->out_shuffle;
  EAVSR_REQUIRE(d->sum_mul == nullptr, -2, "conv3x3_wino4: sum_mul exists in eavsr_conv3x3_f32x6s only");
  a.res_scale = d->res_scale;
  a.border = d->border_pieces;
  a.border_stride = d->border_stride;
  if (d->border_pieces != nullptr) {
    EAVSR_REQUIRE(R == 3 && d->cout == 64 && d->out_shuffle == 0 && d->res_scale == nullptr && d->ca_scale == nullptr &&
                      (d->cin / CK) % 2 == 0 && w6_grouped_schedule(), -2,
                  "conv_wino6: border_pieces needs the grouped 3x3 kernel, 64 output channels, no shuffle / scaled residual / prologue");
    EAVSR_REQUIRE(d->border_stride >= a.tiles_x && d->border_stride >= 2 * a.tiles_y, -1,
                  "conv_wino6: border_stride %d < max(tiles_x %d, 2 tiles_y %d)", d->border_stride, a.tiles_x, 2 * a.tiles_y);
  }
  EAVSR_REQUIRE(d->res_scale == nullptr || (R == 3 && d->residual != nullptr && d->out_shuffle == 0 && d->ca_scale == nullptr &&
                                            (d->cin / CK) % 2 == 0 && w6_grouped_schedule()), -2,
                "conv_wino6: res_scale needs the (grouped) 3x3 kernel, a residual, no prologue, an even number of 4-channel chunks");
  EAVSR_REQUIRE(d->out_shuffle == 0 || d->out_shuffle == 2, -1, "conv_wino6: out_shuffle %d (0 or 2)", d->out_shuffle);
  if (d->out_shuffle == 2)
    EAVSR_REQUIRE(R == 3 && d->cout % 4 == 0 && d->residual == nullptr && d->chan_partial == nullptr, -2,
                  "conv_wino6: the pixel-shuffle epilogue needs the 3x3 kernel, cout %% 4 == 0, no residual, no channel sums");
  const long blocks = (long)a.tiles_x * a.tiles_y * d->n;
  EAVSR_REQUIRE(blocks < (1L << 31), -1, "conv_wino6: too many tiles");
  EAVSR_REQUIRE((long)d->h * d->w * 16 < (1L << 31), -1, "conv_wino6: image plane too large for 32-bit tile offsets");
  EAVSR_REQUIRE(R != 3 || (long)d->h * d->w * 64 * 4 < (1L << 31), -1,
                "conv_wino6: image plane too large for the epilogue's 32-bit offsets (64 channels x h x w x 4 bytes must be < 2 GiB)");
  [[maybe_unused]] constexpr size_t LDS_FUSE = C::LDS_BYTES + 2 * C::IN_PAD * sizeof(float);
  static eavsr::PerDeviceOnce once_pd;
  const int dev_ = eavsr::current_device();
  std::once_flag& once = once_pd.flag[dev_];
  static hipError_t attr_err_pd[eavsr::kMaxDevices] = {};
  hipError_t& attr_err = attr_err_pd[dev_];
  std::call_once(once, [&] {
    attr_err = hipFuncSetAttribute(reinterpret_cast<const void*>(&conv_wino6_kernel<R, false>),
                                   hipFuncAttributeMaxDynamicSharedMemorySize, (int)C::LDS_BYTES);
#if EAVSR_LAB
    if (R == 3 && attr_err == hipSuccess)
      attr_err = hipFuncSetAttribute(reinterpret_cast<const void*>(&conv_wino6_kernel<3, true>),
                                     hipFuncAttributeMaxDynamicSharedMemorySize, (int)(WCfg<3>::LDS_BYTES + 2 * WCfg<3>::IN_PAD * sizeof(float)));
#endif
    if (R == 3 && attr_err == hipSuccess)
      attr_err = hipFuncSetAttribute(reinterpret_cast<const void*>(&conv_wino6_kernel<3, false, true>),
                                     hipFuncAttributeMaxDynamicSharedMemorySize, (int)WCfg<3>::LDS_BYTES);
    if (R == 3 && attr_err == hipSuccess)
      attr_err = hipFuncSetAttribute(reinterpret_cast<const void*>(&conv_wino6_kernel<3, false, true, true>),
                                     hipFuncAttributeMaxDynamicSharedMemorySize, (int)WCfg<3>::LDS_BYTES);
  });
  if (attr_err != hipSuccess) {
    eavsr::set_error("conv_wino6: hipFuncSetAttribute(%zu B of LDS): %s", C::LDS_BYTES, hipGetErrorString(attr_err));
    return (int)attr_err;
  }
  const long per_cot = blocks < 256 ? blocks : 256;
  dim3 grid((unsigned)per_cot, eavsr::cdiv(d->cout, 64));
  if (fuse) {
#if EAVSR_LAB
    if constexpr (R == 3)
      hipLaunchKernelGGL((conv_wino6_kernel<3, true>), grid, dim3(64 * NW), LDS_FUSE, eavsr::as_stream(stream), a);
#endif
  } else {
    const bool grp_on = w6_grouped_schedule();
    if constexpr (R == 3) {
      if (grp_on && (d->cin / CK) % 2 == 0) {
        if (d->res_scale != nullptr)
          hipLaunchKernelGGL((conv_wino6_kernel<3, false, true, true>), grid, dim3(64 * NW), C::LDS_BYTES, eavsr::as_stream(stream), a);
        else
          hipLaunchKernelGGL((conv_wino6_kernel<3, false, true>), grid, dim3(64 * NW), C::LDS_BYTES, eavsr::as_stream(stream), a);
        return eavsr::launch_status("conv_wino6");
      }
    }
    hipLaunchKernelGGL((conv_wino6_kernel<R, false>), grid, dim3(64 * NW), C::LDS_BYTES, eavsr::as_stream(stream), a);
  }
  return eavsr::launch_status("conv_wino6");
}

}

extern "C" int eavsr_pack_conv_weight_wino4(const float* weight, float* packed, int32_t cout, int32_t cin, void* stream) {
  return pack_wino6<3>(weight, packed, cout, cin, stream);
}
extern "C" int eavsr_pack_conv_weight_wino5x5(const float* weight, float* packed, int32_t cout, int32_t cin, void* stream) {
  return pack_wino6<5>(weight, packed, cout, cin, stream);
}

extern "C" int32_t eavsr_conv3x3_wino4_tiles(int32_t h, int32_t w) {
  return eavsr::cdiv(h, WCfg<3>::TOH) * eavsr::cdiv(w, WCfg<3>::TOW);
}
extern "C" int eavsr_conv3x3_wino4_border_pieces(int32_t h, int32_t w, int32_t* p_rows, int32_t* p_cols) {
  EAVSR_REQUIRE(h > 0 && w > 0 && p_rows && p_cols, -1, "conv3x3_wino4_border_pieces: bad arguments");
  *p_rows = eavsr::cdiv(w, WCfg<3>::TOW);
  *p_cols = 2 * eavsr::cdiv(h, WCfg<3>::TOH);
  return 0;
}
extern "C" int32_t eavsr_conv5x5_wino_tiles(int32_t h, int32_t w) {
  return eavsr::cdiv(h, WCfg<5>::TOH) * eavsr::cdiv(w, WCfg<5>::TOW);
}

extern "C" int eavsr_conv3x3_wino4_f32(const eavsr_conv2d_desc* d, const float* weight_wino4, void* stream) {
  return launch_wino6<3>(d, weight_wino4, stream);
}
extern "C" int eavsr_conv5x5_wino_f32(const eavsr_conv2d_desc* d, const float* weight_wino5x5, void* stream) {
  return launch_wino6<5>(d, weight_wino5x5, stream);
}

extern "C" int eavsr_wino4_schedule(void) { return w6_grouped_schedule() ? 1 : 0; }
```

### eavsr_amd/csrc/conv_x9.hip

```cpp
#include "common.h"

#include <mutex>

namespace {

typedef const __attribute__((address_space(1))) void* gptr_t;
typedef __attribute__((address_space(3))) void* lptr_t;
typedef unsigned u32x4 __attribute__((ext_vector_type(4)));
typedef __bf16 bf16x8 __attribute__((ext_vector_type(8)));

struct CxArgs {
  const float* src[5];
  int src_c[5];
  int n_src;
  const u32x4* wsplit;
  const float* bias;
  const float* residual;
  float* out;
  float* chan_partial;
  int n, h, w, cin, cout, tiles_x, tiles_y;
  int act;
  float slope;
};

// ... 179 lines not shown
          c_ = mfma_bf16(wa[0][mt], bcur[1], c_);
          c_ = mfma_bf16(wa[0][mt], bcur[0], c_);
          acc[mt][t] = c_;
        }
        __builtin_amdgcn_sched_group_barrier(0x100, 14, 0);
#pragma unroll
        for (int i = 0; i < 18; ++i) {
          __builtin_amdgcn_sched_group_barrier(0x008, 1, 0);
          __builtin_amdgcn_sched_group_barrier(0x002, 3, 0);
        }
        __builtin_amdgcn_sched_barrier(0);
#pragma unroll
        for (int pl = 0; pl < 3; ++pl) bcur[pl] = bnext[pl];
#pragma unroll
        for (int c = 0; c < CK; ++c) vnext[c] = vfar[c];
      }
#pragma unroll
      for (int pl = 0; pl < 3; ++pl)
#pragma unroll
        for (int mt = 0; mt < 2; ++mt) wa[pl][mt] = wan[pl][mt];
    }
  }

  const int gx = x0 + l31;
  const bool xok = gx < w;
  float csum[2][16];
#pragma unroll
  for (int m = 0; m < 2; ++m) {
#pragma unroll
    for (int r = 0; r < 16; ++r) {
      const int co = cot * 64 + m * 32 + (r & 3) + 8 * (r >> 2) + 4 * kgrp;
      const bool cok = co < a.cout;
      const float b = (cok && a.bias) ? a.bias[co] : 0.f;
      float sum = 0.f;
#pragma unroll
      for (int t = 0; t < NT; ++t) {
        const int gy = y0 + wave * NT + t;
        float v = acc[m][t][r] + b;
        v = eavsr_act(v, a.act == EAVSR_ACT_NONE ? 1.f : a.act == EAVSR_ACT_RELU ? 0.f : a.slope);
        if (cok && xok && gy < h) {
          const size_t o = ((size_t)bn * a.cout + co) * plane + (size_t)gy * w + gx;
          sum += v;
          if (a.residual) v += a.residual[o];
          a.out[o] = v;
        }
      }
      csum[m][r] = sum;
    }
  }
  if (a.chan_partial) {
#pragma unroll
    for (int m = 0; m < 2; ++m)
#pragma unroll
      for (int r = 0; r < 16; ++r) {
        float v = csum[m][r];
        v += __shfl_xor(v, 16);
        v += __shfl_xor(v, 8);
        v += __shfl_xor(v, 4);
        v += __shfl_xor(v, 2);
        v += __shfl_xor(v, 1);
        if (l31 == 0) s_red[wave * 64 + m * 32 + (r & 3) + 8 * (r >> 2) + 4 * kgrp] = v;
      }
    __syncthreads();
    if (tid < 64) {
      const int co = cot * 64 + tid;
      if (co < a.cout) {
        float v = s_red[tid];
#pragma unroll
        for (int k = 1; k < NW; ++k) v += s_red[k * 64 + tid];
        const int tile = ty * a.tiles_x + tx;
        a.chan_partial[((size_t)bn * (a.tiles_x * a.tiles_y) + tile) * a.cout + co] = v;
      }
    }
  }
}

}

extern "C" int eavsr_conv3x3_f32x9(const eavsr_conv2d_desc* d, const void* weight_x9, void* stream) {
  EAVSR_REQUIRE(d != nullptr && weight_x9 != nullptr, -1, "conv3x3_f32x9: NULL descriptor / weights");
  EAVSR_REQUIRE(d->n_src >= 1 && d->n_src <= 5, -1, "conv3x3_f32x9: n_src %d not in 1..5", d->n_src);
  EAVSR_REQUIRE(d->ksize == 3, -2, "conv3x3_f32x9: kernel size %d (3 only)", d->ksize);
  EAVSR_REQUIRE(d->out, -1, "conv3x3_f32x9: NULL out");
  EAVSR_REQUIRE(d->out_shuffle == 0 && d->res_scale == nullptr && d->border_pieces == nullptr && d->sum_mul == nullptr, -2, "conv3x3_f32x9: the pixel-shuffle and scaled-residual epilogues exist in eavsr_conv3x3_wino4_f32 only");
  EAVSR_REQUIRE(d->n >= 0 && d->h > 0 && d->w > 0 && d->cin > 0 && d->cout > 0, -1, "conv3x3_f32x9: bad dims");
  EAVSR_REQUIRE(d->act >= 0 && d->act <= 2, -1, "conv3x3_f32x9: act %d", d->act);
  EAVSR_REQUIRE(d->act != EAVSR_ACT_LRELU || (d->slope >= 0.f && d->slope <= 1.f), -2,
                "conv3x3_f32x9: leaky-ReLU slope %g outside [0, 1] (the epilogue evaluates max(v, slope v))", (double)d->slope);
  EAVSR_REQUIRE(d->ca_scale == nullptr && d->ca_x == nullptr && d->ca_out == nullptr, -2,
                "conv3x3_f32x9: no fused channel-attention prologue");
  EAVSR_REQUIRE(d->w % 4 == 0, -2, "conv3x3_f32x9: w %% 4 != 0 (use eavsr_conv2d_f32)");
  CxArgs a;
  int csum = 0;
  for (int s = 0; s < 5; ++s) {
    a.src[s] = s < d->n_src ? d->src[s] : nullptr;
    a.src_c[s] = s < d->n_src ? d->src_c[s] : 0;
    if (s < d->n_src) {
      EAVSR_REQUIRE(d->src[s] != nullptr && d->src_c[s] > 0 && d->src_c[s] % CK == 0 && (((uintptr_t)d->src[s]) & 15) == 0, -2,
                    "conv3x3_f32x9: source %d must be 16-byte aligned with a multiple of 8 channels", s);
      csum += d->src_c[s];
    }
  }
  EAVSR_REQUIRE(csum == d->cin, -1, "conv3x3_f32x9: sources sum to %d channels, cin = %d", csum, d->cin);
  EAVSR_REQUIRE(eavsr_conv2d_tile_rows(d->n, d->h, d->w, 3) == TH, -2,
                "conv3x3_f32x9: exists for the 32-row tile only (this problem size runs shorter tiles)");
  if (d->n == 0) return 0;
  a.n_src = d->n_src;
  a.wsplit = reinterpret_cast<const u32x4*>(weight_x9);
  a.bias = d->bias; a.residual = d->residual; a.out = d->out; a.chan_partial = d->chan_partial;
  a.n = d->n; a.h = d->h; a.w = d->w; a.cin = d->cin; a.cout = d->cout;
  a.tiles_x = eavsr::cdiv(d->w, TW);
  a.tiles_y = eavsr::cdiv(d->h, TH);
  a.act = d->act; a.slope = d->slope;
  const long blocks = (long)a.tiles_x * a.tiles_y * d->n;
  EAVSR_REQUIRE(blocks < (1L << 31), -1, "conv3x3_f32x9: too many tiles");
  EAVSR_REQUIRE((long)d->h * d->w * 16 < (1L << 31), -1, "conv3x3_f32x9: image plane too large for 32-bit tile offsets");
  static eavsr::PerDeviceOnce once_pd;
  const int dev_ = eavsr::current_device();
  std::once_flag& once = once_pd.flag[dev_];
  static hipError_t attr_err_pd[eavsr::kMaxDevices] = {};
  hipError_t& attr_err = attr_err_pd[dev_];
  std::call_once(once, [&] {
    attr_err = hipFuncSetAttribute(reinterpret_cast<const void*>(&conv3x3_x9_kernel), hipFuncAttributeMaxDynamicSharedMemorySize,
                                   (int)LDS_BYTES);
  });
  if (attr_err != hipSuccess) {
    eavsr::set_error("conv3x3_f32x9: hipFuncSetAttribute(%zu B of LDS): %s", LDS_BYTES, hipGetErrorString(attr_err));
    return (int)attr_err;
  }
  dim3 grid((unsigned)blocks, eavsr::cdiv(d->cout, 64));
  hipLaunchKernelGGL(conv3x3_x9_kernel, grid, dim3(64 * NW), LDS_BYTES, eavsr::as_stream(stream), a);
  return eavsr::launch_status("conv3x3_f32x9");
}
```

### eavsr_amd/networks.py

```python
from __future__ import annotations

import math
from collections import OrderedDict
from typing import List, Sequence, Union

import torch
import torch.nn as nn

from . import autograd as AG
from . import ops

Tensor = torch.Tensor
TensorOrList = Union[Tensor, Sequence[Tensor]]


def seq(*args):
    if len(args) == 1:
        args = args[0]
    if isinstance(args, nn.Module):
        return args
    return nn.Sequential(*[seq(a) for a in args])


class Conv2d(nn.Conv2d):
# ... 189 lines not shown
                and self.kernel_size == (3, 3) and self.stride == (1, 1) and self.padding == (1, 1)
                and self.dilation == (1, 1) and self.groups == 1 and self.in_channels % 8 == 0
                and (self.in_channels // self.deform_groups) % 8 == 0 and self.adastn.D == self.deform_groups
                and ((self.in_channels // self.deform_groups) // 8) & ((self.in_channels // self.deform_groups) // 8 - 1) == 0
                and nbr.shape == feat_prop.shape)

    def forward(self, nbr_feat_l, ref_feat_l, feat_prop, offset, flag=False):
        n, _, h, w = offset.shape
        if not flag:
            h4, w4 = int(math.floor(h * 0.25)), int(math.floor(w * 0.25))
            h2, w2 = int(math.floor(h * 0.5)), int(math.floor(w * 0.5))
            off_d4 = AG.resize_bilinear_ac(offset, (h4, w4), 0.25)
            off_d2 = AG.resize_bilinear_ac(offset, (h2, w2), 0.5)
            warp4 = AG.flow_warp(nbr_feat_l[2], off_d4)
            p1 = self._level(self.flow_l3, self.trans_l3, warp4, ref_feat_l[2])
            p1_up = AG.resize_bilinear_ac(p1, (2 * h4, 2 * w4), 2.0)
            warp2 = AG.flow_warp(nbr_feat_l[1], off_d2, flow2=p1_up)
            p2 = self._level(self.flow_l2, self.trans_l2, warp2, ref_feat_l[1])
            p2_up = AG.resize_bilinear_ac(p2, (2 * h2, 2 * w2), 2.0, pre_add=p1_up)
            warp1 = AG.flow_warp(nbr_feat_l[0], offset, flow2=p2_up)
            p3 = self._level(self.flow_l1, self.trans_l1, warp1, ref_feat_l[0])
            offset = AG.add(p3, p2_up, offset)
        if self._fused_alignment(nbr_feat_l[0], feat_prop, offset):
            if BACKBONE_DTYPE is not None:
                nbr, feat_il = ops.flow_warp_pair(nbr_feat_l[0], feat_prop, offset, b_il8=BACKBONE_DTYPE)
                heads = self.adastn.heads(nbr, ref_feat_l[0])
                return ops.dcnv2_il16(feat_il, heads, None, self.weight, self.bias, self.deform_groups, heads=True)
            nbr, feat_il = ops.flow_warp_pair(nbr_feat_l[0], feat_prop, offset, b_il8=True)
            act = ops.heads_mask_activated(int(self.weight.shape[1]), self.deform_groups)
            heads = self.adastn.heads(nbr, ref_feat_l[0], mask_activated=act)
            return ops.dcnv2_il(feat_il, heads, None, self.weight, self.bias, self.deform_groups,
                                nprod=int(ops.DCN_MODE[2]), heads=True, mask_activated=act)
        nbr = AG.flow_warp(nbr_feat_l[0], offset)
        feat = AG.flow_warp(feat_prop, offset)
        de_offset, mask = self.adastn(nbr, ref_feat_l[0])
        return modulated_deform_conv2d(feat, de_offset, mask, self.weight, self.bias, self.stride, self.padding,
                                       self.dilation, self.groups, self.deform_groups)


class CALayer(nn.Module):
    def __init__(self, channel=64, reduction=16):
        super().__init__()
        self.conv_du = nn.Sequential(
            nn.Conv2d(channel, channel // reduction, 1, padding=0, bias=True), _Act("relu"),
            nn.Conv2d(channel // reduction, channel, 1, padding=0, bias=True), _Act("sigmoid"))

    def scale_from_partial(self, partial: Tensor, hw: int) -> Tensor:
        a, b = self.conv_du[0], self.conv_du[2]
        return ops.ca_scale(partial, hw, a.weight, a.bias, b.weight, b.bias)

    def forward(self, x):
        n, c, h, w = x.shape
        a, b = self.conv_du[0], self.conv_du[2]
        if AG.needs_grad(x, a.weight, b.weight):
            return AG.rcab_tail(x, torch.zeros_like(x), a.weight, a.bias, b.weight, b.bias)
        partial = x.sum(dim=(2, 3)).view(n, 1, c)
        return ops.scale_residual(x, self.scale_from_partial(partial, h * w), torch.zeros_like(x))


class RCABlock(nn.Module):
    def __init__(self, in_channels=64, out_channels=64, kernel_size=3, stride=1, padding=1, bias=True,
                 mode="CRC", reduction=16):
        super().__init__()
        assert in_channels == out_channels
        if mode[0] in "RL":
            mode = mode[0].lower() + mode[1:]
        self.res = conv(in_channels, out_channels, kernel_size, stride, padding, bias=bias, mode=mode)
        self.ca = CALayer(out_channels, reduction)

    def forward(self, x):
        a, b = self.ca.conv_du[0], self.ca.conv_du[2]
        if AG.needs_grad(x, list(self.parameters())):
            if (RCAB_ONE_NODE and len(self.res) == 3 and isinstance(self.res[1], _Act) and self.res[1].kind == "relu"
                    and torch.is_grad_enabled()):
                c1, c2 = self.res[0], self.res[2]
                ps = [c1.weight, c1.bias, c2.weight, c2.bias, a.weight, a.bias, b.weight, b.bias]
                if AG.rcab_supported(x, ps):
                    return AG.rcab(x, *ps)
            r = _run_fused(self.res, x)
            return AG.rcab_tail(r, x, a.weight, a.bias, b.weight, b.bias)
        if (RCAB_PRE and x.shape[1] == 64 and len(self.res) == 3 and isinstance(self.res[1], _Act) and self.res[1].kind == "relu"
                and tuple(self.res[2].weight.shape) == (64, 64, 3, 3) and int(a.weight.shape[0]) <= 8):
            c1, c2 = self.res[0], self.res[2]
            t, tpart, pieces = ops.conv2d(x, c1.weight, c1.bias, act="relu", chan_partial=True, border=True)
            if not RCAB_PRE_PIECES:
                pieces = None
            scale = ops.ca_scale_pre(t, tpart, c2.weight, c2.bias, a.weight, a.bias, b.weight, b.bias, border=pieces)
            return ops.conv2d(t, c2.weight, c2.bias, residual=x, res_scale=scale)
        r, partial = _run_fused(self.res, x, chan_partial=True)
        if FUSE_CA_TAIL:
            return ops.ca_tail(r, partial, a.weight, a.bias, b.weight, b.bias, x)
        scale = self.ca.scale_from_partial(partial, x.shape[2] * x.shape[3])
        return ops.scale_residual(r, scale, x)


import os as _os
FUSE_CA_TAIL = _os.environ.get("EAVSR_FUSE_CA_TAIL", "0") == "1"
RCAB_PRE = _os.environ.get("EAVSR_RCAB_PRE", "1") == "1"
RCAB_PRE_PIECES = _os.environ.get("EAVSR_RCAB_PRE_PIECES", "1") == "1"


def set_rcab_pre(on: bool) -> None:
    global RCAB_PRE
    RCAB_PRE = bool(on)
RCAB_ONE_NODE = _os.environ.get("EAVSR_RCAB_ONE_NODE", "1") != "0"
FUSE_CA_INTO_CONV = _os.environ.get("EAVSR_FUSE_CA", "0") == "1"
FUSE_FLOW_LEVEL = _os.environ.get("EAVSR_FUSE_LEVEL", "0") == "1"


def set_fuse_flow_level(on: bool) -> None:
    global FUSE_FLOW_LEVEL
    if on:
        ops.require_lab("the one-kernel-per-pyramid-level form (eavsr_flow_level_f32)")
    FUSE_FLOW_LEVEL = bool(on)


HEADS_IN_16BIT = _os.environ.get("EAVSR_HEADS_16BIT", "1") == "1"
BACKBONE_DTYPE = _os.environ.get("EAVSR_BACKBONE_DTYPE") or None
RCAB_H16_FUSED = _os.environ.get("EAVSR_RCAB_H16_FUSED", "0") == "1"


def set_rcab_h16_fused(on: bool) -> None:
    global RCAB_H16_FUSED
    if on:
        ops.require_lab("the one-launch 16-bit RCAB (eavsr_rcab_convs_h16)")
    RCAB_H16_FUSED = bool(on)


RCAB_H16_PRE = _os.environ.get("EAVSR_RCAB_H16_PRE", "1") == "1"


def set_rcab_h16_pre(on: bool) -> None:
    global RCAB_H16_PRE
    RCAB_H16_PRE = bool(on)
if BACKBONE_DTYPE is not None:
    ops.set_conv3_h16(BACKBONE_DTYPE)


def set_backbone_dtype(dtype):
    global BACKBONE_DTYPE
    if dtype is not None:
        ops.h16_code(dtype)
    BACKBONE_DTYPE = dtype
    ops.set_conv3_h16(dtype)


import contextlib as _contextlib


@_contextlib.contextmanager
def backbone_dtype(dtype):
    prev = BACKBONE_DTYPE
    set_backbone_dtype(dtype)
    try:
        yield
    finally:
        set_backbone_dtype(prev)


TRAIN_PRECISIONS = ops.TRAIN_PRECISIONS


def set_train_precision(mode: str) -> None:
    ops.TRAIN_PRECISION = ops.check_precision(mode)


def get_train_precision() -> str:
    return ops.TRAIN_PRECISION


@_contextlib.contextmanager
def train_precision(mode: str):
    prev = ops.TRAIN_PRECISION
    set_train_precision(mode)
    try:
        yield
    finally:
        ops.TRAIN_PRECISION = prev


def set_deterministic(flag: bool) -> None:
    if not isinstance(flag, bool):
# ... 108 lines not shown
```

### eavsr_amd/ops.py

```python
from __future__ import annotations

import contextlib
import ctypes as C
import os
from typing import List, Optional, Sequence, Tuple, Union

import torch

from . import _native as N
from .weight_cache import WEIGHT_CACHES, WeightCache

Tensor = torch.Tensor

ACT = {"none": 0, None: 0, "relu": 1, "lrelu": 2, "relu_mask": 3}


def _chk(t: Tensor, name: str) -> Tensor:
    if not isinstance(t, torch.Tensor):
        raise TypeError(f"{name}: expected a tensor, got {type(t)}")
    if not t.is_cuda:
        raise RuntimeError(f"{name}: tensor is on {t.device}; eavsr_amd runs on the GPU only (no CPU path)")
    if t.dtype != torch.float32:
        raise RuntimeError(f"{name}: dtype {t.dtype} unsupported (fp32 only in this round)")
    return t if t.is_contiguous() else t.contiguous()
# ... 425 lines not shown
    wp = _packed_h16g(weights, code)
    b = _bias_of(biases)
    out = torch.empty((n, cout, h, w), device=srcs[0].device, dtype=torch.float32)
    d = N.ConvDesc()
    for i in range(5):
        d.src[i] = _p(srcs[i]) if i < len(srcs) else None
        d.src_c[i] = int(srcs[i].shape[1]) if i < len(srcs) else 0
    d.n_src = len(srcs)
    d.ksize = 3
    d.weight_packed = _p(wp)
    d.bias = _p(b)
    d.out = _p(out)
    d.n, d.h, d.w, d.cin, d.cout = n, h, w, cin, cout
    d.act = ACT[act]
    d.slope = float(slope)
    st = _stream(out)
    px = float(n) * h * w
    _launch(f"conv3x3_{cin}to{cout}_h16g", 2.0 * cin * cout * 9 * px, 4.0 * px * (cin + cout), out,
            lambda: lib().eavsr_conv3x3_h16g_f32(C.byref(d), code, st), "conv3x3_h16g")
    return out


def _conv3x3_smallco(x: Tensor, weights, biases, act, slope, residual):
    n, cin, h, w = x.shape
    wt = _cat_weights(weights)
    cout = int(wt.shape[0])
    b = _bias_of(biases)
    out = torch.empty((n, cout, h, w), device=x.device, dtype=torch.float32)
    if residual is not None:
        residual = _chk(residual, "residual")
        if residual.shape != out.shape:
            raise ValueError("residual shape mismatch")
    st = _stream(x)
    px = float(n) * h * w
    if (SMALLCO_LITE and cout in (2, 3, 4, 6) and w % 4 == 0 and x.data_ptr() % 16 == 0 and h * w * cin * 4 < 2 ** 32
            and _rn(n) * ((h + 7) // 8) * ((w + 63) // 64) >= SMALLCO_LITE_MIN_TILES):
        wp = _packed_smallco(list(weights))
        _launch(f"conv3x3_{cin}to{cout}", 2.0 * cin * cout * 9 * px, 4.0 * px * (cin + cout + (cout if residual is not None else 0)), x,
                lambda: lib().eavsr_conv3x3_smallco_lite_f32(_p(x), _p(wp), _p(b), _p(residual), _p(out), n, cin, h, w, cout,
                                                             ACT[act], float(slope), st), "conv3x3_smallco_lite")
        return out
    _launch(f"conv3x3_{cin}to{cout}", 2.0 * cin * cout * 9 * px, 4.0 * px * (cin + cout + (cout if residual is not None else 0)), x,
            lambda: lib().eavsr_conv3x3_smallco_f32(_p(x), _p(wt), _p(b), _p(residual), _p(out), n, cin, h, w, cout,
                                                    ACT[act], float(slope), st), "conv3x3_smallco")
    return out


def _wino_fusable(x: Tensor) -> bool:
    return (lab_available() and CONV_MODE in ("winograd", "winograd4") and x.dim() == 4 and x.shape[3] % 4 == 0 and x.shape[1] % 8 == 0 and x.shape[1] <= 256
            and x.is_contiguous() and x.data_ptr() % 16 == 0
            and _rn(int(x.shape[0])) * _wino_tiles(int(x.shape[2]), int(x.shape[3])) >= WINO_MIN_TILES)


def ca_fusable(x: Tensor, cout: int = 64) -> bool:
    if _wino_fusable(x):
        return True
    return (x.dim() == 4 and x.shape[3] % 4 == 0 and x.shape[1] % 4 == 0 and x.shape[1] <= 256 and 32 < cout <= 64
            and x.is_contiguous() and x.data_ptr() % 16 == 0
            and lib().eavsr_conv2d_tile_rows(int(x.shape[0]), int(x.shape[2]), int(x.shape[3]), 3) == 32)


FUSE_PIXEL_SHUFFLE = os.environ.get("EAVSR_FUSE_SHUFFLE", "1") == "1"


_dgrad_w_cache = WeightCache()


def dgrad_weight(w: Tensor) -> Tensor:
    hit = _dgrad_w_cache.lookup((w,))
    if hit is not None:
        return hit
    return _dgrad_w_cache.store((w,), None, w.detach().flip(2, 3).transpose(0, 1).contiguous())


class BorderPieces:
    __slots__ = ("data", "p_rows", "p_cols")

    def __init__(self, data: Tensor, p_rows: int, p_cols: int):
        self.data, self.p_rows, self.p_cols = data, int(p_rows), int(p_cols)


def conv2d(srcs, weight, bias=None, act=None, slope: float = 0.0, residual=None, chan_partial: bool = False, ca=None, ca_out: bool = False,
           pixel_shuffle2: bool = False, sigmoid_from=None, dgrad: bool = False, res_scale=None, border: bool = False, sum_mul=None,
           precision: str = "fp32"):
    r = _conv2d(srcs, weight, bias, act, slope, residual, chan_partial, ca, ca_out, pixel_shuffle2, sigmoid_from, dgrad, res_scale, border,
                sum_mul, precision)
    if border and not (isinstance(r, tuple) and len(r) >= 2 and (r[-1] is None or isinstance(r[-1], BorderPieces))):
        r = (tuple(r) if isinstance(r, tuple) else (r,)) + (None,)
    return r


def _conv2d(srcs: Union[Tensor, Sequence[Tensor]], weight: Union[Tensor, Sequence[Tensor]],
           bias: Union[None, Tensor, Sequence[Optional[Tensor]]] = None, act: Optional[str] = None,
           slope: float = 0.0, residual: Optional[Tensor] = None, chan_partial: bool = False,
           ca: Optional[Tuple[Tensor, Tensor]] = None, ca_out: bool = False, pixel_shuffle2: bool = False,
           sigmoid_from: Optional[int] = None, dgrad: bool = False, res_scale: Optional[Tensor] = None, border: bool = False,
           sum_mul: Optional[Tensor] = None, precision: str = "fp32"):
    check_precision(precision)
    if sum_mul is not None:
        if not dgrad or chan_partial or ca is not None or pixel_shuffle2 or sigmoid_from is not None or res_scale is not None or act == "relu_mask":
            raise ValueError("sum_mul: input-gradient convolutions only (dgrad=True; no channel sums / prologue / shuffle / sigmoid / mask)")
        sum_mul = _chk(sum_mul, "sum_mul")
    if isinstance(srcs, torch.Tensor):
        srcs = [srcs]
    weights = [weight] if isinstance(weight, torch.Tensor) else list(weight)
    biases = [bias] if (bias is None or isinstance(bias, torch.Tensor)) else list(bias)
    srcs = [_chk(s, f"src{i}") for i, s in enumerate(srcs)]
    if not 1 <= len(srcs) <= 5:
        raise ValueError("1..5 sources")
    n, _, h, w = srcs[0].shape
    for s in srcs:
        if s.shape[0] != n or tuple(s.shape[2:]) != (h, w):
            raise ValueError("all sources must share n,h,w")
    cin = sum(int(s.shape[1]) for s in srcs)
    if dgrad:
        if len(weights) != 1 or biases != [None] or chan_partial or ca is not None or pixel_shuffle2 or sigmoid_from is not None:
            raise ValueError("dgrad: one forward weight, no bias / channel sums / prologue / shuffle / sigmoid")
        if int(weights[0].shape[0]) != cin:
            raise ValueError(f"dgrad: the forward weight has {int(weights[0].shape[0])} output channels, dY gives {cin}")
        k_ = int(weights[0].shape[-1])
        if not (CONV3_SMALL == "x6s" and CONV_MODE in ("winograd", "winograd4") and k_ == 3 and len(srcs) == 1 and cin == 64
                and int(weights[0].shape[1]) not in (2, 3, 4, 6) and CONV3_H16 is None
                and _rn(n) * lib().eavsr_conv3x3_x6s_tiles(h, w) <= X6S_MAX_TILES):
            y = conv2d(srcs, dgrad_weight(weights[0]), None, act, slope, residual)
            return y if sum_mul is None else (y, plane_sum(y, sum_mul).view(n, 1, -1))
    cout = sum(int(x.shape[0]) for x in weights) if not dgrad else int(weights[0].shape[1])
    k = int(weights[0].shape[-1])
    if not dgrad and any(int(x.shape[1]) != cin for x in weights):
        raise ValueError(f"weight expects {[int(x.shape[1]) for x in weights]} input channels, sources give {cin}")
    if pixel_shuffle2 and (cout % 4 or residual is not None or chan_partial or ca is not None):
        raise ValueError("pixel_shuffle2: cout % 4 == 0, no residual / channel sums / channel-attention prologue")
    if res_scale is not None:
        if residual is None or chan_partial or ca is not None or pixel_shuffle2 or sigmoid_from is not None or dgrad or act == "relu_mask":
            raise ValueError("res_scale: with `residual`; no channel sums / prologue / shuffle / sigmoid / dgrad / mask")
        res_scale = _chk(res_scale, "res_scale")
        if tuple(res_scale.shape) != (n, cout):
            raise ValueError(f"res_scale must be (n, cout) = ({n}, {cout})")
    masked = act == "relu_mask"
    if masked and (residual is None or chan_partial or ca is not None or pixel_shuffle2 or sigmoid_from is not None):
        raise ValueError("act='relu_mask': residual = the ReLU's forward output; no channel sums / prologue / shuffle / sigmoid")
    if ca_out and ca is None:
        raise ValueError("ca_out needs ca")
    if sigmoid_from is not None:
        sigmoid_from = int(sigmoid_from)
        if not 0 <= sigmoid_from < cout:
            raise ValueError(f"sigmoid_from {sigmoid_from}: 0 <= value < cout = {cout}")
        if residual is not None or chan_partial or ca is not None or pixel_shuffle2:
            raise ValueError("sigmoid_from: plain convolutions only")
        fused = (((k == 7 and CONV7_MODE == "bf16x6") or (k == 5 and CONV5_MODE == "bf16x6")) and len(srcs) == 1
                 and cin % 8 == 0 and sigmoid_from % 8 == 0)
        if not fused:
            y = conv2d(srcs, weights, biases, act, slope)
            y[:, sigmoid_from:] = torch.sigmoid(y[:, sigmoid_from:])
            return y
    if k == 3 and len(srcs) == 1 and cout in (2, 3, 4, 6) and not chan_partial and ca is None and not masked and res_scale is None:
        y = _conv3x3_smallco(srcs[0], weights, biases, act, slope, residual)
        return torch.nn.functional.pixel_shuffle(y, 2) if pixel_shuffle2 else y
    if (CONV3_H16 is not None and k == 7 and CONV7_H16_ENABLED and sigmoid_from is None and len(srcs) == 1 and cin % 8 == 0 and cout >= 16
            and residual is None and not chan_partial and ca is None and not pixel_shuffle2 and not torch.is_grad_enabled()):
        return _conv_h16x1(srcs[0], weights, biases, act, slope, CONV3_H16)
    if (((k == 7 and CONV7_MODE == "bf16x6") or (k == 5 and CONV5_MODE == "bf16x6")) and len(srcs) == 1 and cin % 8 == 0
            and residual is None and not chan_partial and ca is None and not pixel_shuffle2):
        return _conv_x6(srcs[0], weights, biases, act, slope, -1 if sigmoid_from is None else int(sigmoid_from))
    if (CONV3_H16 is not None and k == 3 and sigmoid_from is None and residual is None and not chan_partial and ca is None
            and not pixel_shuffle2 and w % 4 == 0 and cout >= 32 and not torch.is_grad_enabled()
            and all(int(s_.shape[1]) % 16 == 0 and s_.data_ptr() % 16 == 0 for s_ in srcs)):
        return _conv3x3_h16g(srcs, weights, biases, act, slope, CONV3_H16)
    ck = lib().eavsr_conv2d_ck(k)
    if any(int(s.shape[1]) % ck for s in srcs[:-1]):
        srcs = [torch.cat(srcs, 1)]
    b = _bias_of(biases)
    out = torch.empty((n, cout, h, w), device=srcs[0].device, dtype=torch.float32)
    base_ok = (k == 3 and w % 4 == 0 and all(int(s_.shape[1]) % 8 == 0 and s_.data_ptr() % 16 == 0 for s_ in srcs))
    x9_ok = base_ok and ca is None and not masked
    if CONV_MODE in ("winograd", "bf16x9"):
        require_lab(f"conv mode {CONV_MODE!r}")
    lab = lab_available()
    use_wino = (CONV_MODE in ("winograd", "winograd4") and base_ok and not masked
                and _rn(n) * _wino_tiles(h, w) >= WINO_MIN_TILES
                and (ca is None or (lab and len(srcs) == 1 and cin <= 256 and ca[1].data_ptr() % 16 == 0)))
    use_wino4 = (use_wino and CONV_MODE == "winograd4" and out.data_ptr() % 16 == 0
                 and (residual is None or residual.data_ptr() % 16 == 0)
                 and 2 * _rn(n) * lib().eavsr_conv3x3_wino4_tiles(h, w) >= WINO_MIN_TILES)
    if use_wino and not use_wino4 and not lab:
        use_wino = False
    if res_scale is not None and not (use_wino4 and cin % 8 == 0 and lib().eavsr_wino4_schedule() >= 1):
        return scale_residual(conv2d(srcs, weights, biases, act=act, slope=slope), res_scale, residual)
    if pixel_shuffle2 and not (use_wino4 and FUSE_PIXEL_SHUFFLE):
        return torch.nn.functional.pixel_shuffle(conv2d(srcs, weights, biases, act=act, slope=slope), 2)
    use_wino5 = (CONV_MODE == "winograd4" and k == 5 and ca is None and not masked and w % 4 == 0 and out.data_ptr() % 8 == 0
                 and all(int(s_.shape[1]) % 4 == 0 and s_.data_ptr() % 16 == 0 for s_ in srcs)
                 and (residual is None or residual.data_ptr() % 8 == 0)
                 and _rn(n) * lib().eavsr_conv5x5_wino_tiles(h, w) * ((cout + 63) // 64) >= 2 * WINO_MIN_TILES)
    use_x6s = (CONV3_SMALL == "x6s" and CONV_MODE in ("winograd", "winograd4") and k == 3 and len(srcs) == 1 and cin == 64
               and ca is None and not pixel_shuffle2 and not use_wino
               and _rn(n) * lib().eavsr_conv3x3_x6s_tiles(h, w) <= X6S_MAX_TILES)
    if sum_mul is not None and not (use_x6s and w % 4 == 0 and tuple(sum_mul.shape) == (n, cout, h, w) and
                                    all(t_ is None or t_.data_ptr() % 16 == 0 for t_ in (srcs[0], out, residual, sum_mul))):
        y = conv2d(srcs, weights, None, act, slope, residual, dgrad=True, precision=precision)
        return y, plane_sum(y, sum_mul).view(n, 1, -1)
    if dgrad and not use_x6s:
        weights, dgrad = [dgrad_weight(weights[0])], False
    wp = None if use_x6s else _packed_f32(weights)
    part = None
    if sum_mul is not None:
        part = torch.empty((n, lib().eavsr_conv3x3_x6s_tiles(h, w), cout), device=out.device, dtype=torch.float32)
    if chan_partial:
        tiles = (lib().eavsr_conv3x3_x6s_tiles(h, w) if use_x6s else lib().eavsr_conv5x5_wino_tiles(h, w) if use_wino5 else lib().eavsr_conv3x3_wino4_tiles(h, w) if use_wino4 else _wino_tiles(h, w) if use_wino
                 else lib().eavsr_conv2d_tiles(n, h, w, k))
        part = torch.empty((n, tiles, cout), device=out.device, dtype=torch.float32)
    if residual is not None:
        residual = _chk(residual, "residual")
        if residual.shape != out.shape:
            raise ValueError("residual shape mismatch")
    d = N.ConvDesc()
    for i in range(5):
        d.src[i] = _p(srcs[i]) if i < len(srcs) else None
        d.src_c[i] = int(srcs[i].shape[1]) if i < len(srcs) else 0
    d.n_src = len(srcs)
    d.ksize = k
    d.weight_packed = _p(wp) if wp is not None else None
    d.bias = _p(b)
    d.residual = _p(residual)
    d.out = _p(out)
    d.chan_partial = _p(part)
    d.n, d.h, d.w, d.cin, d.cout = n, h, w, cin, cout
    d.act = ACT[act]
    d.slope = float(slope)
    d.res_scale = _p(res_scale)
    d.sum_mul = _p(sum_mul)
    pieces = None
    if (border and chan_partial and use_wino4 and cout == 64 and cin % 8 == 0 and ca is None and not pixel_shuffle2 and res_scale is None
            and lib().eavsr_wino4_schedule() == 1):
        pr, pc = C.c_int32(0), C.c_int32(0)
        N.check(lib().eavsr_conv3x3_wino4_border_pieces(h, w, C.byref(pr), C.byref(pc)), "conv3x3_wino4_border_pieces")
        stride = max(pr.value, pc.value)
        pieces = BorderPieces(torch.empty((n, 4, stride, 64), device=out.device, dtype=torch.float32), pr.value, pc.value)
        d.border_pieces, d.border_stride = _p(pieces.data), stride
    if pixel_shuffle2 and use_wino4:
        d.out_shuffle = 2
        out = out.view(n, cout // 4, 2 * h, 2 * w)
    xs = None
    if ca is not None:
        scale, cx = _chk(ca[0], "ca scale"), _chk(ca[1], "ca x")
        if len(srcs) != 1 or cx.shape != srcs[0].shape or tuple(scale.shape) != (n, cin):
            raise ValueError("ca=(scale, x): one source, x of the same shape, scale (n, cin)")
        if not use_wino and (k != 3 or not ca_fusable(srcs[0], cout) or cx.data_ptr() % 16):
            raise NotImplementedError("fused channel-attention prologue unavailable for this shape; use "
                                      "scale_residual + conv2d (see ops.ca_fusable)")
        d.ca_scale, d.ca_x = _p(scale), _p(cx)
        if ca_out:
            xs = torch.empty_like(cx)
            d.ca_out = _p(xs)
    elif ca_out:
        raise ValueError("ca_out needs ca")
    st = _stream(out)
    px = float(n) * h * w
    if use_x6s and precision == "bf16":
        wq = _packed_conv3_bf16(weights, dgrad=dgrad)
        _launch(f"conv3x3_{cin}to{cout}_bf16s", 2.0 * cin * cout * 9 * px,
                4.0 * px * (cin + cout + (cout if residual is not None else 0)), out,
                lambda: lib().eavsr_conv3x3_bf16x1s(C.byref(d), _p(wq), st), "conv3x3_bf16x1s")
        return out if not (chan_partial or sum_mul is not None) else (out, part)
    if use_x6s:
        wq = _packed_conv_x6(weights, dgrad=dgrad)
        _launch(f"conv3x3_{cin}to{cout}_x6s", 2.0 * cin * cout * 9 * px,
                4.0 * px * (cin + cout + (cout if residual is not None else 0)), out,
                lambda: lib().eavsr_conv3x3_f32x6s(C.byref(d), _p(wq), st), "conv3x3_f32x6s")
        return out if not (chan_partial or sum_mul is not None) else (out, part)
    if use_wino5:
        wu = _packed_wino(weights, kind="f5")
        _launch(f"conv5x5_{cin}to{cout}_wino", 2.0 * cin * cout * 25 * px,
                4.0 * px * (cin + cout + (cout if residual is not None else 0)), out,
                lambda: lib().eavsr_conv5x5_wino_f32(C.byref(d), _p(wu), st), "conv5x5_wino")
        return out if not chan_partial else (out, part)
    if use_wino4:
        wu = _packed_wino(weights, four=True)
        _launch(f"conv3x3_{cin}to{cout}_wino4" + ("_ca" if ca is not None else ""), 2.0 * cin * cout * 9 * px,
                4.0 * px * (cin * (1 if ca is None else (3 if ca_out else 2)) + cout + (cout if residual is not None else 0)), out,
                lambda: lib().eavsr_conv3x3_wino4_f32(C.byref(d), _p(wu), st), "conv3x3_wino4")
        res = [out] + ([part] if chan_partial else []) + ([xs] if xs is not None else []) + ([pieces] if border else [])
        return res[0] if len(res) == 1 else tuple(res)
    if use_wino:
        wu = _packed_wino(weights)
        _launch(f"conv3x3_{cin}to{cout}_wino" + ("_ca" if ca is not None else ""), 2.0 * cin * cout * 9 * px,
                4.0 * px * (cin * (1 if ca is None else (3 if ca_out else 2)) + cout + (cout if residual is not None else 0)), out,
                lambda: lib().eavsr_conv3x3_wino_f32(C.byref(d), _p(wu), st), "conv3x3_wino")
        res = [out] + ([part] if chan_partial else []) + ([xs] if xs is not None else [])
        return res[0] if len(res) == 1 else tuple(res)
    if CONV_MODE == "bf16x9" and x9_ok and lib().eavsr_conv2d_tile_rows(n, h, w, 3) == 32:
        wx = _packed_x9(weights)
        _launch(f"conv3x3_{cin}to{cout}_x9", 2.0 * cin * cout * 9 * px,
                4.0 * px * (cin + cout + (cout if residual is not None else 0)), out,
                lambda: lib().eavsr_conv3x3_f32x9(C.byref(d), _p(wx), st), "conv3x3_f32x9")
        return out if not chan_partial else (out, part)
    _launch(f"conv{k}x{k}_{cin}to{cout}" + ("_ca" if ca is not None else ""), 2.0 * cin * cout * k * k * px,
            4.0 * px * (cin * (1 if ca is None else (3 if ca_out else 2)) + cout + (cout if residual is not None else 0)), out,
            lambda: lib().eavsr_conv2d_f32(C.byref(d), st), "conv2d")
    if not chan_partial and xs is None:
        return out
    res = [out]
    if chan_partial:
        res.append(part)
    if xs is not None:
        res.append(xs)
    return tuple(res)


def _one(v):
    return int(v[0]) if isinstance(v, (tuple, list)) else int(v)


def modulated_deform_conv2d(input: Tensor, offset: Tensor, mask: Tensor, weight: Tensor,
                            bias: Optional[Tensor] = None, stride=1, padding=0, dilation=1, groups=1,
                            deform_groups=1) -> Tensor:
    x = _chk(input, "input")
    cout, cin_g, kh, kw = (int(v) for v in weight.shape)
    n, cin, h, w = x.shape
    two = lambda v: (int(v[0]), int(v[1])) if isinstance(v, (tuple, list)) else (int(v), int(v))
    (sh, sw), (ph, pw), (dh, dw) = two(stride), two(padding), two(dilation)
    if cin_g * groups != cin:
        raise ValueError("weight / input channel mismatch")
    if cin % deform_groups or cout % groups:
        raise ValueError("channels not divisible by groups / deform_groups")
    ho = (h + 2 * ph - (dh * (kh - 1) + 1)) // sh + 1
    wo = (w + 2 * pw - (dw * (kw - 1) + 1)) // sw + 1
    offset = _chk(offset, "offset")
    mask = _chk(mask, "mask")
    if tuple(offset.shape) != (n, deform_groups * 2 * kh * kw, ho, wo):
        raise ValueError(f"offset shape {tuple(offset.shape)} != {(n, deform_groups * 2 * kh * kw, ho, wo)}")
    if tuple(mask.shape) != (n, deform_groups * kh * kw, ho, wo):
        raise ValueError(f"mask shape {tuple(mask.shape)} != {(n, deform_groups * kh * kw, ho, wo)}")
    b = None if bias is None else _chk(bias.detach(), "bias")
    out = torch.empty((n, cout, ho, wo), device=x.device, dtype=torch.float32)
    on_path = ((kh, kw) == (3, 3) and (sh, sw, ph, pw, dh, dw) == (1, 1, 1, 1, 1, 1) and groups == 1
               and (cin // deform_groups) % 8 == 0)
    if not on_path:
        if groups > 1 and (cout // groups) % 8:
            raise NotImplementedError("modulated_deform_conv2d: with conv groups > 1 the output channels per group must be "
                                      "a multiple of 8")
        wt = _chk(weight.detach(), "weight")
        st = _stream(x)
        _launch("dcnv2_generic", 2.0 * cin_g * kh * kw * cout * n * ho * wo,
                4.0 * n * (cin * h * w + (3 * deform_groups * kh * kw + cout) * ho * wo), x,
                lambda: lib().eavsr_dcnv2_generic_f32(_p(x), _p(offset), _p(mask), _p(wt), _p(b), _p(out), n, cin, h, w, cout,
                                                      kh, kw, sh, sw, ph, pw, dh, dw, groups, deform_groups, st),
                "dcnv2_generic")
        return out
    st = _stream(x)
    px = float(n) * h * w
    flops, nbytes = 2.0 * cin * 9 * cout * px, 4.0 * px * (cin + 27 * deform_groups + cout)
    octets = (cin // deform_groups) // 8
    if DCN_MODE in ("il6", "il9") and octets & (octets - 1) == 0:
        return dcnv2_il(to_il8(x), offset, mask, weight, b, deform_groups, nprod=int(DCN_MODE[2]), heads=False)
    if DCN_MODE == "bf16x9":
        require_lab("dcn mode 'bf16x9'")
    if DCN_MODE == "bf16x9" and w % 4 == 0 and x.data_ptr() % 16 == 0:
        wx = _packed_dcn_x9(weight)
        _launch("dcnv2_x9", flops, nbytes, x,
                lambda: lib().eavsr_dcnv2_f32x9(_p(x), _p(offset), _p(mask), _p(wx), _p(b), _p(out), n, cin, h, w, cout,
                                                deform_groups, st), "dcnv2_f32x9")
        return out
    wp = _packed_f32([weight])
    _launch("dcnv2", flops, nbytes, x,
# ... 1557 lines not shown
```

### include/eavsr_hip.h

```cpp
#ifndef EAVSR_HIP_H
#define EAVSR_HIP_H

#include <stddef.h>
#include <stdint.h>

#ifdef __cplusplus
extern "C" {
#endif

#define EAVSR_ABI_VERSION 32

#define EAVSR_ACT_NONE 0
#define EAVSR_ACT_RELU 1
#define EAVSR_ACT_LRELU 2
#define EAVSR_ACT_RELU_MASK 3

#define EAVSR_PAD_ZEROS 0
#define EAVSR_PAD_BORDER 1
#define EAVSR_PAD_REFLECTION 2
#define EAVSR_WARP_NEAREST 0x10
#define EAVSR_WARP_NO_ALIGN_CORNERS 0x20

#define EAVSR_FLOW_NCHW 0
#define EAVSR_FLOW_NHWC 1

int eavsr_abi_version(void);
const char* eavsr_version(void);
const char* eavsr_last_error(void);
int eavsr_lab_build(void);

int eavsr_selftest_mfma_f32(float* scratch, void* stream);

int eavsr_flow_warp_f32(const float* x, const float* flow, const float* flow2, float* out,
                        int32_t n, int32_t c, int32_t h, int32_t w,
                        int32_t flow_layout, int32_t padding_mode, void* stream);

int eavsr_flow_warp_pair_f32(const float* xa, const float* xb, const float* flow, const float* flow2, float* outa,
                             float* outb, int32_t n, int32_t c, int32_t h, int32_t w, int32_t outb_il8, void* stream);


int eavsr_dcnv2_f32(const float* x, const float* offset, const float* mask,
                    const float* weight_packed, const float* bias, float* out,
                    int32_t n, int32_t cin, int32_t h, int32_t w, int32_t cout,
                    int32_t deform_groups, void* stream);

int64_t eavsr_dcn_weight_x9_bytes(int32_t cout, int32_t cin);
int eavsr_pack_dcn_weight_x9(const float* weight, void* weight_x9, int32_t cout, int32_t cin, void* stream);

int eavsr_nchw_to_il8_f32(const float* x, float* out_il8, int32_t n, int32_t c, int32_t h, int32_t w, void* stream);
int eavsr_dcnv2_il_f32(const float* x_il8, const float* offset_or_heads, const float* mask, const void* weight_x9,
                       const float* bias, float* out, int32_t n, int32_t cin, int32_t h, int32_t w, int32_t cout,
                       int32_t deform_groups, int32_t nprod, int32_t heads, void* stream);

int64_t eavsr_dcn_weight_il2_bytes(int32_t cout, int32_t cin);
int eavsr_pack_dcn_weight_il2(const float* weight, void* weight_il2, int32_t cout, int32_t cin, void* stream);
int eavsr_dcnv2_il2_f32(const float* x_il8, const float* offset_or_heads, const float* mask, const void* weight_il2,
                        const float* bias, float* out, int32_t n, int32_t cin, int32_t h, int32_t w, int32_t cout,
                        int32_t deform_groups, int32_t nprod, int32_t heads, void* stream);

int64_t eavsr_dcn_il16_weight_bytes(int32_t cout, int32_t cin);
int eavsr_pack_dcn_il16_weight(const float* weight, void* weight_il16, int32_t cout, int32_t cin, int32_t dtype, void* stream);
int eavsr_nchw_to_il8_h16(const float* x, void* out_il8_h16, int32_t n, int32_t c, int32_t h, int32_t w, int32_t dtype, void* stream);
int eavsr_dcnv2_il16(const void* x_il8_h16, const float* offset_or_heads, const float* mask, const void* weight_il16,
                     const float* bias, float* out, int32_t n, int32_t cin, int32_t h, int32_t w, int32_t cout,
                     int32_t deform_groups, int32_t dtype, int32_t heads, void* stream);

int eavsr_dcnv2_generic_f32(const float* x, const float* offset, const float* mask, const float* weight,
                            const float* bias, float* out, int32_t n, int32_t cin, int32_t h, int32_t w,
                            int32_t cout, int32_t kh, int32_t kw, int32_t stride_h, int32_t stride_w,
                            int32_t pad_h, int32_t pad_w, int32_t dil_h, int32_t dil_w, int32_t groups,
                            int32_t deform_groups, void* stream);

typedef struct eavsr_conv2d_desc {
  const float* src[5];
  int32_t src_c[5];
  int32_t n_src;
  int32_t ksize;
  const float* weight_packed;
  const float* bias;
  const float* residual;
  float* out;
  float* chan_partial;
  int32_t n, h, w, cin, cout;
  int32_t act;
  float slope;
  const float* ca_scale;
  const float* ca_x;
  float* ca_out;
  int32_t out_shuffle;
  const float* res_scale;
  float* border_pieces;
  int32_t border_stride;
  const float* sum_mul;
} eavsr_conv2d_desc;

size_t eavsr_conv2d_desc_size(void);
int eavsr_conv2d_f32(const eavsr_conv2d_desc* desc, void* stream);

int64_t eavsr_wino4_weight_elems(int32_t cout, int32_t cin);
int eavsr_pack_conv_weight_wino4(const float* weight, float* weight_wino4, int32_t cout, int32_t cin, void* stream);
int32_t eavsr_conv3x3_wino4_tiles(int32_t h, int32_t w);
int eavsr_conv3x3_wino4_border_pieces(int32_t h, int32_t w, int32_t* p_rows, int32_t* p_cols);
int eavsr_conv3x3_wino4_f32(const eavsr_conv2d_desc* desc, const float* weight_wino4, void* stream);

int eavsr_pack_conv_weight_wino5x5(const float* weight, float* weight_wino5x5, int32_t cout, int32_t cin, void* stream);
int32_t eavsr_conv5x5_wino_tiles(int32_t h, int32_t w);
int eavsr_conv5x5_wino_f32(const eavsr_conv2d_desc* desc, const float* weight_wino5x5, void* stream);
int32_t eavsr_conv2d_ck(int32_t ksize);
int32_t eavsr_conv2d_tile_rows(int32_t n, int32_t h, int32_t w, int32_t ksize);
int32_t eavsr_conv2d_tiles(int32_t n, int32_t h, int32_t w, int32_t ksize);
int32_t eavsr_route_batch(int32_t n);
int64_t eavsr_packed_weight_elems(int32_t cout, int32_t cin, int32_t ksize);
int eavsr_pack_conv_weight_f32(const float* weight, float* packed, int32_t cout, int32_t cin,
                               int32_t ksize, void* stream);

int eavsr_conv3x3_smallco_f32(const float* x, const float* weight, const float* bias, const float* residual,
                              float* out, int32_t n, int32_t cin, int32_t h, int32_t w, int32_t cout, int32_t act,
                              float slope, void* stream);

int64_t eavsr_smallco_packed_elems(int32_t cout, int32_t cin);
int eavsr_pack_smallco_weight(const float* weight, float* packed, int32_t cout, int32_t cin, void* stream);
int eavsr_conv3x3_smallco_lite_f32(const float* x, const float* weight_packed, const float* bias, const float* residual,
                                   float* out, int32_t n, int32_t cin, int32_t h, int32_t w, int32_t cout, int32_t act,
                                   float slope, void* stream);

size_t eavsr_conv_weight_x6_bytes(int32_t ksize, int32_t cout, int32_t cin);
int eavsr_pack_conv_weight_x6(const float* weight, void* packed, int32_t ksize, int32_t cout, int32_t cin, void* stream);
int eavsr_pack_conv_weight_x6_dgrad(const float* weight, void* packed, int32_t ksize, int32_t cout_w, int32_t cin_w, void* stream);
int eavsr_pack_conv_weight_x6_multi(const float* const* weights, void* const* packed, const int32_t* transposed, int32_t count,
                                    int32_t ksize, int32_t c, void* stream);
int eavsr_conv_f32x6(const float* x, const void* weight_x6, const float* bias, float* out, int32_t n, int32_t cin, int32_t cout,
                     int32_t h, int32_t w, int32_t ksize, int32_t act, float slope, int32_t sigmoid_from, void* stream);
int32_t eavsr_conv3x3_x6s_tiles(int32_t h, int32_t w);
int eavsr_conv3x3_f32x6s(const eavsr_conv2d_desc* desc, const void* weight_x6, void* stream);

int eavsr_wino4_schedule(void);

int eavsr_ca_scale_f32(const float* chan_partial, int32_t tiles, int32_t hw,
                       const float* w1, const float* b1, const float* w2, const float* b2,
                       float* scale, int32_t n, int32_t c, int32_t cr, void* stream);
int eavsr_ca_scale_mean_f32(const float* chan_partial, int32_t tiles, int32_t hw, const float* w1, const float* b1,
                            const float* w2, const float* b2, float* scale, float* mean_out, int32_t n, int32_t c, int32_t cr,
                            void* stream);
int eavsr_scale_residual_f32(const float* r, const float* scale, const float* x, float* out,
                             int32_t n, int32_t c, int32_t hw, void* stream);
int eavsr_ca_tail_f32(const float* r, const float* chan_partial, int32_t tiles, const float* w1, const float* b1,
                      const float* w2, const float* b2, const float* x, float* out, int32_t n, int32_t c, int32_t cr,
                      int32_t hw, void* stream);
int eavsr_ca_tail_stats_f32(const float* r, const float* chan_partial, int32_t tiles, const float* w1, const float* b1,
                            const float* w2, const float* b2, const float* x, float* out, float* scale_out, float* mean_out,
                            int32_t n, int32_t c, int32_t cr, int32_t hw, void* stream);

int eavsr_adapt_frontend_f32(const float* x, const float* h_hr, const float* w1, const float* b1,
                             const float* w2, const float* b2, float* out,
                             int32_t n, int32_t c, int32_t h, int32_t w, void* stream);

int eavsr_affine_offsets_f32(const float* heads, float* offset, float* mask,
                             int32_t n, int32_t D, int32_t h, int32_t w, void* stream);

int eavsr_resize_bilinear_ac_f32(const float* in, const float* in2, const float* addend, float* out,
                                 int32_t n, int32_t c, int32_t hin, int32_t win,
                                 int32_t hout, int32_t wout, float scale, void* stream);
int eavsr_pyramid_f32(const float* in, float* down2, float* down4,
                      int32_t nc, int32_t h, int32_t w, void* stream);
int eavsr_add_f32(const float* a, const float* b, const float* c, float* out, int64_t count,
                  void* stream);

int eavsr_normalize_f32(const float* in, const float* mean, const float* std, float* out,
                        int32_t n, int32_t c, int32_t hw, void* stream);
int eavsr_avg_pool2_f32(const float* in, float* out, int32_t nc, int32_t h, int32_t w, void* stream);
int eavsr_resize_bilinear_f32(const float* in, float* out, int32_t n, int32_t c, int32_t hin, int32_t win,
                              int32_t hout, int32_t wout, int32_t cmul, float m0, float m1, void* stream);
int eavsr_concat3_f32(const float* a, int32_t ca, const float* b, int32_t cb, const float* c, int32_t cc, float* out,
                      int32_t n, int32_t hw, void* stream);


// ... 191 lines not shown
```

Measured before the change: 134.7.

## Fuse RCAB channel attention into grouped Winograd conv kernels via per-tile moment sums

The first RCAB conv now also computes per-tile sums, using border corrections, of the next conv's input contracted with the next conv's weights (mtile). The second conv kernel reduces those per-tile sums at its start, runs the squeeze-excite MLP and sigmoid on-chip, and applies the scale in its scaled-residual epilogue. This removes the separate channel-attention scale kernel and its extra launches and passes over memory. In exchange it adds LDS usage, extra registers, a full-image reduction per block at kernel entry, and a more complex descriptor ABI. The path is on by default through an environment flag.

```diff
diff --git a/eavsr_amd/_native.py b/eavsr_amd/_native.py
--- a/eavsr_amd/_native.py
+++ b/eavsr_amd/_native.py
@@ -39,6 +39,14 @@
         ("border_pieces", vp),
         ("border_stride", i32),
         ("sum_mul", vp),
+        ("fca_next_weight", vp),
+        ("fca_mtile", vp),
+        ("fca_w1", vp),
+        ("fca_b1", vp),
+        ("fca_w2", vp),
+        ("fca_b2", vp),
+        ("fca_scale_out", vp),
+        ("fca_cr", i32),
     ]
 
 
diff --git a/eavsr_amd/csrc/common.h b/eavsr_amd/csrc/common.h
--- a/eavsr_amd/csrc/common.h
+++ b/eavsr_amd/csrc/common.h
@@ -41,6 +41,10 @@
     }                                       \
   } while (0)
 
+static inline bool eavsr_desc_has_fca(const eavsr_conv2d_desc* d) {
+  return d->fca_next_weight || d->fca_mtile || d->fca_w1 || d->fca_b1 || d->fca_w2 || d->fca_b2 || d->fca_scale_out;
+}
+
 typedef float f32x16 __attribute__((ext_vector_type(16)));
 typedef float f32x4 __attribute__((ext_vector_type(4)));
 
diff --git a/eavsr_amd/csrc/conv3_h16.hip b/eavsr_amd/csrc/conv3_h16.hip
--- a/eavsr_amd/csrc/conv3_h16.hip
+++ b/eavsr_amd/csrc/conv3_h16.hip
@@ -243,7 +243,7 @@
   EAVSR_REQUIRE(d && d->out && d->weight_packed, -1, "conv3x3_h16g: NULL pointer");
   EAVSR_REQUIRE(dtype == 1 || dtype == 2, -1, "conv3x3_h16g: dtype %d (1 = f16, 2 = bf16)", dtype);
   EAVSR_REQUIRE(d->ksize == 3 && d->n_src >= 1 && d->n_src <= 5, -2, "conv3x3_h16g: 3x3, 1..5 sources");
-  EAVSR_REQUIRE(!d->residual && !d->chan_partial && !d->ca_scale && !d->ca_x && !d->ca_out && d->out_shuffle == 0 && !d->res_scale && !d->border_pieces && !d->sum_mul, -2,
+  EAVSR_REQUIRE(!d->residual && !d->chan_partial && !d->ca_scale && !d->ca_x && !d->ca_out && d->out_shuffle == 0 && !d->res_scale && !d->border_pieces && !d->sum_mul && !eavsr_desc_has_fca(d), -2,
                 "conv3x3_h16g: plain convolution only (no residual / channel sums / channel-attention prologue / pixel shuffle)");
   EAVSR_REQUIRE(d->n >= 0 && d->h > 0 && d->w > 0 && d->cout > 0 && d->w % 4 == 0, -2, "conv3x3_h16g: bad dims (w %% 4 == 0)");
   int cin = 0;
diff --git a/eavsr_amd/csrc/conv3_x6s.hip b/eavsr_amd/csrc/conv3_x6s.hip
--- a/eavsr_amd/csrc/conv3_x6s.hip
+++ b/eavsr_amd/csrc/conv3_x6s.hip
@@ -482,7 +482,7 @@
   EAVSR_REQUIRE(d->n >= 0 && d->cout > 0 && d->h > 0 && d->w > 0, -1, "%s: bad dims", name);
   if (d->n == 0) return 1;
   EAVSR_REQUIRE(d->src[0] && d->out, -1, "%s: NULL pointer", name);
-  EAVSR_REQUIRE(d->ca_scale == nullptr && d->ca_x == nullptr && d->ca_out == nullptr && d->out_shuffle == 0 && d->res_scale == nullptr && d->border_pieces == nullptr, -2,
+  EAVSR_REQUIRE(d->ca_scale == nullptr && d->ca_x == nullptr && d->ca_out == nullptr && d->out_shuffle == 0 && d->res_scale == nullptr && d->border_pieces == nullptr && !eavsr_desc_has_fca(d), -2,
                 "%s: no channel-attention prologue, no pixel-shuffle store", name);
   EAVSR_REQUIRE(d->act >= 0 && d->act <= EAVSR_ACT_RELU_MASK, -1, "%s: act %d", name, d->act);
   EAVSR_REQUIRE(d->act != EAVSR_ACT_LRELU || (d->slope >= 0.f && d->slope <= 1.f), -2,
diff --git a/eavsr_amd/csrc/conv_mfma.hip b/eavsr_amd/csrc/conv_mfma.hip
--- a/eavsr_amd/csrc/conv_mfma.hip
+++ b/eavsr_amd/csrc/conv_mfma.hip
@@ -618,7 +618,7 @@
   EAVSR_REQUIRE(d->ksize == 1 || d->ksize == 3 || d->ksize == 5 || d->ksize == 7, -2,
                 "conv2d: kernel size %d unsupported (1,3,5,7)", d->ksize);
   EAVSR_REQUIRE(d->weight_packed && d->out, -1, "conv2d: NULL weight/out");
-  EAVSR_REQUIRE(d->out_shuffle == 0 && d->res_scale == nullptr && d->border_pieces == nullptr && d->sum_mul == nullptr, -2, "conv2d: the pixel-shuffle and scaled-residual epilogues exist in eavsr_conv3x3_wino4_f32 only");
+  EAVSR_REQUIRE(d->out_shuffle == 0 && d->res_scale == nullptr && d->border_pieces == nullptr && d->sum_mul == nullptr && !eavsr_desc_has_fca(d), -2, "conv2d: the pixel-shuffle and scaled-residual epilogues exist in eavsr_conv3x3_wino4_f32 only");
   EAVSR_REQUIRE(d->n >= 0 && d->h > 0 && d->w > 0 && d->cin > 0 && d->cout > 0, -1, "conv2d: bad dims");
   EAVSR_REQUIRE(d->act >= 0 && d->act <= EAVSR_ACT_RELU_MASK, -1, "conv2d: act %d", d->act);
   EAVSR_REQUIRE(d->act != EAVSR_ACT_RELU_MASK || (d->residual != nullptr && d->chan_partial == nullptr && d->ca_scale == nullptr), -1,
diff --git a/eavsr_amd/csrc/conv_wino.hip b/eavsr_amd/csrc/conv_wino.hip
--- a/eavsr_amd/csrc/conv_wino.hip
+++ b/eavsr_amd/csrc/conv_wino.hip
@@ -397,7 +397,7 @@
   EAVSR_REQUIRE(d->n_src >= 1 && d->n_src <= 5, -1, "conv3x3_wino: n_src %d not in 1..5", d->n_src);
   EAVSR_REQUIRE(d->ksize == 3, -2, "conv3x3_wino: kernel size %d (3 only)", d->ksize);
   EAVSR_REQUIRE(d->out, -1, "conv3x3_wino: NULL out");
-  EAVSR_REQUIRE(d->out_shuffle == 0 && d->res_scale == nullptr && d->border_pieces == nullptr && d->sum_mul == nullptr, -2, "conv3x3_wino: the pixel-shuffle and scaled-residual epilogues exist in eavsr_conv3x3_wino4_f32 only");
+  EAVSR_REQUIRE(d->out_shuffle == 0 && d->res_scale == nullptr && d->border_pieces == nullptr && d->sum_mul == nullptr && !eavsr_desc_has_fca(d), -2, "conv3x3_wino: the pixel-shuffle and scaled-residual epilogues exist in eavsr_conv3x3_wino4_f32 only");
   EAVSR_REQUIRE(d->n >= 0 && d->h > 0 && d->w > 0 && d->cin > 0 && d->cout > 0, -1, "conv3x3_wino: bad dims");
   EAVSR_REQUIRE(d->act >= 0 && d->act <= 2, -1, "conv3x3_wino: act %d", d->act);
   EAVSR_REQUIRE(d->act != EAVSR_ACT_LRELU || (d->slope >= 0.f && d->slope <= 1.f), -2,
diff --git a/eavsr_amd/csrc/conv_wino6.hip b/eavsr_amd/csrc/conv_wino6.hip
--- a/eavsr_amd/csrc/conv_wino6.hip
+++ b/eavsr_amd/csrc/conv_wino6.hip
@@ -63,6 +63,16 @@
   float* border;
   int border_stride;
 };
+struct W4ArgsF : W4Args {
+  const float* fca_wnext;
+  float* fca_mtile;
+  const float* fca_w1;
+  const float* fca_b1;
+  const float* fca_w2;
+  const float* fca_b2;
+  float* fca_scale_out;
+  int fca_cr;
+};
 
 constexpr int CK = 4, NW = 8, NPOS = 36;
 constexpr int MARG = 4;
@@ -95,6 +105,8 @@
   static constexpr int LDS_FLOATS = LDS_MAIN + 128;
 #endif
   static constexpr size_t LDS_BYTES = (size_t)LDS_FLOATS * sizeof(float);
+  static constexpr int FCA_FLOATS = 1024 + 576;
+  static constexpr size_t LDS_BYTES_FCA = (size_t)(LDS_FLOATS + FCA_FLOATS) * sizeof(float);
 };
 
 template <typename T>
@@ -154,8 +166,9 @@
 #define W4_IT(i) do { } while (0)
 #endif
 
-template <int R, bool FUSE = false, bool GRP = false, bool RSC = false>
-__global__ __launch_bounds__(512, 2) void conv_wino6_kernel(W4Args a) {
+template <int R, bool FUSE = false, bool GRP = false, bool RSC = false, bool FCA = false>
+__global__ __launch_bounds__(512, 2) void conv_wino6_kernel(std::conditional_t<FCA, W4ArgsF, W4Args> a) {
+  static_assert(!FCA || (GRP && R == 3 && !FUSE), "the in-convolution channel attention exists for the grouped 3x3 kernel");
   static_assert(!RSC || (GRP && R == 3 && !FUSE), "the scaled-residual epilogue exists for the grouped 3x3 kernel");
   static_assert(!FUSE || R == 3, "the fused channel-attention prologue exists for the 3x3 kernel");
   static_assert(!GRP || (R == 3 && !FUSE), "the grouped schedule exists for the plain 3x3 kernel");
@@ -472,6 +485,61 @@
 #endif
   if (total_iters > 1) issue_patch(1);
   W4_TL(1);
+  [[maybe_unused]] float* const s_fca = smem + C::LDS_FLOATS;
+  [[maybe_unused]] int fca_bn = -1;
+  [[maybe_unused]] auto fca_scale_of = [&](int img) __attribute__((always_inline)) {
+    if constexpr (FCA && RSC) {
+      const int rows = a.tiles_x * a.tiles_y, cr = a.fca_cr;
+      const float bc_v = (tid < 64 && a.bias != nullptr) ? a.bias[tid] : 0.f;
+      const float w1_v = wave < cr ? a.fca_w1[wave * 64 + lane] : 0.f, b1_v = wave < cr ? a.fca_b1[wave] : 0.f;
+      float w2_v[8];
+#pragma unroll
+      for (int j = 0; j < 8; ++j) w2_v[j] = (tid < 64 && j < cr) ? a.fca_w2[tid * cr + j] : 0.f;
+      const float b2_v = tid < 64 ? a.fca_b2[tid] : 0.f;
+      const float* p = a.fca_mtile + (size_t)img * rows * 64 + lane;
+      float s0 = 0.f, s1 = 0.f;
+      for (int r0 = wave; r0 < rows; r0 += 16 * NW) {
+        float v[16];
+#pragma unroll
+        for (int j = 0; j < 16; ++j) {
+          v[j] = 0.f;
+          if (r0 + NW * j < rows) v[j] = p[(size_t)(r0 + NW * j) * 64];
+        }
+#pragma unroll
+        for (int j = 0; j < 16; j += 4) {
+          s0 += v[j] + v[j + 1];
+          s1 += v[j + 2] + v[j + 3];
+        }
+      }
+      s_fca[wave * 64 + lane] = s0 + s1;
+      __syncthreads();
+      if (tid < 64) {
+        float v = 0.f;
+#pragma unroll
+        for (int k = 0; k < NW; ++k) v += s_fca[k * 64 + tid];
+        s_fca[512 + tid] = bc_v + v / ((float)h * (float)w);
+      }
+      __syncthreads();
+      if (wave < cr) {
+        float v = w1_v * s_fca[512 + lane];
+#pragma unroll
+        for (int off = 32; off > 0; off >>= 1) v += __shfl_xor(v, off);
+        if (lane == 0) s_fca[576 + wave] = fmaxf(v + b1_v, 0.f);
+      }
+      __syncthreads();
+      if (tid < 64) {
+        float v = b2_v;
+#pragma unroll
+        for (int j = 0; j < 8; ++j) v += j < cr ? w2_v[j] * s_fca[576 + j] : 0.f;
+        const float sc = 1.f / (1.f + expf(-v));
+        s_fca[640 + tid] = sc;
+        if (a.fca_scale_out != nullptr) a.fca_scale_out[(size_t)img * 64 + tid] = sc;
+      }
+      __syncthreads();
+      fca_bn = img;
+    }
+  };
+  if constexpr (FCA && RSC) fca_scale_of(bn);
   if constexpr (!GRP) {
     asm volatile("s_waitcnt vmcnt(0)" ::: "memory");
     __syncthreads();
@@ -716,6 +784,8 @@
     {
       float csum[4] = {0.f, 0.f, 0.f, 0.f};
       constexpr bool fast_done = GRP;
+      constexpr bool FCA_E = FCA && !RSC;
+      [[maybe_unused]] float o8[8][4];
       if constexpr (GRP) {
        {
         const int gx = x0 + 4 * l15;
@@ -733,7 +803,11 @@
         const unsigned lane_off_ps = gx < w ? (unsigned)((((size_t)(cb * 4 + kq)) * 4 * plane + (size_t)(2 * gy0) * (2 * w) + 2 * gx) * sizeof(float)) : W6_OOB;
         const bool has_act = a.act != EAVSR_ACT_NONE;
         float sc4[4] = {1.f, 1.f, 1.f, 1.f};
-        if constexpr (RSC) {
+        if constexpr (RSC && FCA) {
+          if (bn != fca_bn) fca_scale_of(bn);
+#pragma unroll
+          for (int r = 0; r < 4; ++r) sc4[r] = s_fca[640 + cb * 16 + 4 * kq + r];
+        } else if constexpr (RSC) {
 #pragma unroll
           for (int r = 0; r < 4; ++r) {
             const int co = cot * 64 + cb * 16 + 4 * kq + r;
@@ -748,8 +822,9 @@
         };
         if (has_res) load_rr(0);
         f32x2 cs2[4] = {f32x2{0.f, 0.f}, f32x2{0.f, 0.f}, f32x2{0.f, 0.f}, f32x2{0.f, 0.f}};
-        const bool b_tile = !RSC && a.border != nullptr && (y0 == 0 || y0 + TOH >= h || x0 == 0 || x0 + TOW >= w);
+        const bool b_tile = !RSC && (FCA || a.border != nullptr) && (y0 == 0 || y0 + TOH >= h || x0 == 0 || x0 + TOW >= w);
         float btop[4] = {0.f, 0.f, 0.f, 0.f}, bbot[4] = {0.f, 0.f, 0.f, 0.f}, blft[4] = {0.f, 0.f, 0.f, 0.f}, brgt[4] = {0.f, 0.f, 0.f, 0.f};
+        [[maybe_unused]] float ctl[4] = {0.f, 0.f, 0.f, 0.f}, ctr[4] = {0.f, 0.f, 0.f, 0.f}, cbl[4] = {0.f, 0.f, 0.f, 0.f}, cbr[4] = {0.f, 0.f, 0.f, 0.f};
 #pragma unroll
         for (int rp = 0; rp < 2; ++rp) {
           const f32x2 b2 = f32x2{bias_r[2 * rp], bias_r[2 * rp + 1]};
@@ -810,6 +885,10 @@
                       if (gy0 + dy == h - 1) bbot[r] += h2.x + h2.y;
                       blft[r] += v[0];
                       brgt[r] += v[3];
+                      if constexpr (FCA_E) {
+                        if (gy0 + dy == 0) { ctl[r] = v[0]; ctr[r] = v[3]; }
+                        if (gy0 + dy == h - 1) { cbl[r] = v[0]; cbr[r] = v[3]; }
+                      }
                     }
                   }
                   w6_st4(r_out, lane_off, (unsigned)r * plane_b + (unsigned)dy * row_b, o);
@@ -823,8 +902,36 @@
           const int co = cot * 64 + cb * 16 + 4 * kq + r;
           csum[r] = (co < a.cout && gx < w) ? cs2[r].x + cs2[r].y : 0.f;
         }
+        if constexpr (FCA_E) {
+#pragma unroll
+          for (int k = 0; k < 8; ++k)
+#pragma unroll
+            for (int r = 0; r < 4; ++r) o8[k][r] = 0.f;
+          if (b_tile) {
+            const bool has_top = gy0 == 0 && rows > 0, has_bot = gy0 <= h - 1 && h - 1 < gy0 + M;
+            const bool lft = x0 == 0, rgt = x0 + TOW >= w;
+            const int lr = (lane & 48) | (rgt ? ((w - 4 - x0) >> 2) : 0);
+#pragma unroll
+            for (int r = 0; r < 4; ++r) {
+              float vt = gx < w ? btop[r] : 0.f, vb = gx < w ? bbot[r] : 0.f;
+              vt += __shfl_xor(vt, 8); vb += __shfl_xor(vb, 8);
+              vt += __shfl_xor(vt, 4); vb += __shfl_xor(vb, 4);
+              vt += __shfl_xor(vt, 2); vb += __shfl_xor(vb, 2);
+              vt += __shfl_xor(vt, 1); vb += __shfl_xor(vb, 1);
+              const float rg = __shfl(brgt[r], lr), tr = __shfl(ctr[r], lr), br = __shfl(cbr[r], lr);
+              o8[0][r] = has_top ? vt : 0.f;
+              o8[1][r] = has_bot ? vb : 0.f;
+              o8[2][r] = lft ? blft[r] : 0.f;
+              o8[3][r] = rgt ? rg : 0.f;
+              o8[4][r] = (lft && has_top) ? ctl[r] : 0.f;
+              o8[5][r] = (rgt && has_top) ? tr : 0.f;
+              o8[6][r] = (lft && has_bot) ? cbl[r] : 0.f;
+              o8[7][r] = (rgt && has_bot) ? br : 0.f;
+            }
+          }
+        }
         if constexpr (!RSC) {
-          if (b_tile) {
+          if (b_tile && (!FCA || a.border != nullptr)) {
             const int txi = x0 / TOW, tyi = y0 / TOH;
             float* bp = a.border + (size_t)bn * 4 * a.border_stride * 64 + cb * 16 + 4 * kq;
             const bool has_top = gy0 == 0 && rows > 0, has_bot = gy0 <= h - 1 && h - 1 < gy0 + M;
@@ -968,8 +1075,22 @@
           }
         }
       }
-      if (a.chan_partial) {
-        __syncthreads();
+      [[maybe_unused]] f32x4 wq[18];
+      [[maybe_unused]] auto fca_barrier = [&]() __attribute__((always_inline)) {
+        if constexpr (FCA_E) {
+          asm volatile("s_waitcnt lgkmcnt(0)" ::: "memory");
+          __builtin_amdgcn_s_barrier();
+        } else {
+          __syncthreads();
+        }
+      };
+      if constexpr (FCA_E) {
+        const f32x4* wr4 = reinterpret_cast<const f32x4*>(a.fca_wnext + (size_t)(tid >> 3) * 576) + (tid & 7);
+#pragma unroll
+        for (int i = 0; i < 18; ++i) wq[i] = wr4[8 * i];
+      }
+      if (FCA_E || a.chan_partial) {
+        fca_barrier();
 #pragma unroll
         for (int r = 0; r < 4; ++r) {
           float v = csum[r];
@@ -979,12 +1100,45 @@
           v += __shfl_xor(v, 1);
           if (l15 == 0) s_red[tg * 64 + cb * 16 + 4 * kq + r] = v;
         }
-        __syncthreads();
-        if (tid < 64) {
+        if constexpr (FCA_E) {
+          if (l15 == 0) {
+#pragma unroll
+            for (int k = 0; k < 8; ++k)
+#pragma unroll
+              for (int r = 0; r < 4; ++r) s_fca[(k * 2 + tg) * 64 + cb * 16 + 4 * kq + r] = o8[k][r];
+          }
+        }
+        fca_barrier();
+        if (tid < 64 && (!FCA_E || a.chan_partial != nullptr)) {
           const int co = cot * 64 + tid;
           if (co < a.cout)
             a.chan_partial[((size_t)bn * (a.tiles_x * a.tiles_y) + tile_lin) * a.cout + co] = s_red[tid] + s_red[64 + tid];
         }
+      }
+      if constexpr (FCA_E) {
+        float* const s_S = s_fca + 1024;
+        for (int k = tid; k < 576; k += 64 * NW) {
+          const int ci = k / 9, tap = k - 9 * ci, ky = tap / 3, kx = tap - 3 * ky;
+          auto both = [&](int b) __attribute__((always_inline)) { return s_fca[(b * 2) * 64 + ci] + s_fca[(b * 2 + 1) * 64 + ci]; };
+          const float T = s_red[ci] + s_red[64 + ci];
+          const float Rr = ky == 0 ? both(1) : ky == 2 ? both(0) : 0.f;
+          const float Cc = kx == 0 ? both(3) : kx == 2 ? both(2) : 0.f;
+          const float Xc = (ky == 1 || kx == 1) ? 0.f : both(4 + (ky == 0 ? 2 : 0) + (kx == 0 ? 1 : 0));
+          s_S[k] = (T - Rr) - Cc + Xc;
+        }
+        fca_barrier();
+        const int co = tid >> 3, pt = tid & 7;
+        float v = 0.f;
+#pragma unroll
+        for (int i = 0; i < 18; ++i) {
+          const f32x4 s4 = *reinterpret_cast<const f32x4*>(s_S + 4 * (pt + 8 * i));
+#pragma unroll
+          for (int e = 0; e < 4; ++e) v += wq[i][e] * s4[e];
+        }
+        v += __shfl_xor(v, 1);
+        v += __shfl_xor(v, 2);
+        v += __shfl_xor(v, 4);
+        if (pt == 0) a.fca_mtile[((size_t)bn * (a.tiles_x * a.tiles_y) + tile_lin) * 64 + co] = v;
       }
 #pragma unroll
       for (int x = 0; x < NPOS; ++x) acc[x] = f32x4{0.f, 0.f, 0.f, 0.f};
@@ -1121,7 +1275,7 @@
   constexpr uintptr_t AL = R == 3 ? 15 : 7;
   EAVSR_REQUIRE((((uintptr_t)d->out) & AL) == 0 && (d->residual == nullptr || (((uintptr_t)d->residual) & AL) == 0), -2,
                 "conv_wino6: out / residual must be %d-byte aligned", (int)AL + 1);
-  W4Args a;
+  W4ArgsF a;
   int csum = 0;
   for (int s = 0; s < 5; ++s) {
     a.src[s] = s < d->n_src ? d->src[s] : nullptr;
@@ -1153,6 +1307,29 @@
                   "conv_wino6: border_pieces needs the grouped 3x3 kernel, 64 output channels, no shuffle / scaled residual / prologue");
     EAVSR_REQUIRE(d->border_stride >= a.tiles_x && d->border_stride >= 2 * a.tiles_y, -1,
                   "conv_wino6: border_stride %d < max(tiles_x %d, 2 tiles_y %d)", d->border_stride, a.tiles_x, 2 * a.tiles_y);
+  }
+  const bool fca_first = d->fca_next_weight != nullptr, fca_second = d->fca_w1 != nullptr;
+  a.fca_wnext = d->fca_next_weight; a.fca_mtile = d->fca_mtile;
+  a.fca_w1 = d->fca_w1; a.fca_b1 = d->fca_b1; a.fca_w2 = d->fca_w2; a.fca_b2 = d->fca_b2;
+  a.fca_scale_out = d->fca_scale_out; a.fca_cr = d->fca_cr;
+  if (fca_first || fca_second) {
+    EAVSR_REQUIRE(R == 3 && !(fca_first && fca_second) && d->fca_mtile != nullptr, -1,
+                  "conv_wino6: fca_* describe ONE of the two convolutions (fca_next_weight | fca_w1 ..) and need fca_mtile");
+    EAVSR_REQUIRE(d->cout == 64 && d->out_shuffle == 0 && d->res_scale == nullptr && d->ca_scale == nullptr && (d->cin / CK) % 2 == 0 &&
+                      w6_grouped_schedule(), -2,
+                  "conv_wino6: fca_* need the grouped 3x3 kernel, 64 output channels, no shuffle / res_scale / prologue");
+    if (fca_first) {
+      EAVSR_REQUIRE((((uintptr_t)d->fca_next_weight) & 15) == 0 && d->fca_scale_out == nullptr, -2,
+                    "conv_wino6: fca_next_weight must be 16-byte aligned (and fca_scale_out belongs to the second convolution)");
+    } else {
+      EAVSR_REQUIRE(d->fca_b1 && d->fca_w2 && d->fca_b2 && d->fca_cr >= 1 && d->fca_cr <= 8, -1,
+                    "conv_wino6: the second convolution needs fca_w1 / fca_b1 / fca_w2 / fca_b2 and 1..8 hidden units (fca_cr %d)", d->fca_cr);
+      EAVSR_REQUIRE(d->residual != nullptr && d->act == EAVSR_ACT_NONE && d->chan_partial == nullptr && d->border_pieces == nullptr &&
+                        d->cin == 64, -2,
+                    "conv_wino6: the second convolution of the fused attention is 64 -> 64 with a residual, no activation / sums / border pieces");
+    }
+  } else {
+    EAVSR_REQUIRE(!eavsr_desc_has_fca(d), -1, "conv_wino6: fca_mtile / fca_b1 .. without fca_next_weight or fca_w1");
   }
   EAVSR_REQUIRE(d->res_scale == nullptr || (R == 3 && d->residual != nullptr && d->out_shuffle == 0 && d->ca_scale == nullptr &&
                                             (d->cin / CK) % 2 == 0 && w6_grouped_schedule()), -2,
@@ -1186,6 +1363,12 @@
     if (R == 3 && attr_err == hipSuccess)
       attr_err = hipFuncSetAttribute(reinterpret_cast<const void*>(&conv_wino6_kernel<3, false, true, true>),
                                      hipFuncAttributeMaxDynamicSharedMemorySize, (int)WCfg<3>::LDS_BYTES);
+    if (R == 3 && attr_err == hipSuccess)
+      attr_err = hipFuncSetAttribute(reinterpret_cast<const void*>(&conv_wino6_kernel<3, false, true, false, true>),
+                                     hipFuncAttributeMaxDynamicSharedMemorySize, (int)WCfg<3>::LDS_BYTES_FCA);
+    if (R == 3 && attr_err == hipSuccess)
+      attr_err = hipFuncSetAttribute(reinterpret_cast<const void*>(&conv_wino6_kernel<3, false, true, true, true>),
+                                     hipFuncAttributeMaxDynamicSharedMemorySize, (int)WCfg<3>::LDS_BYTES_FCA);
   });
   if (attr_err != hipSuccess) {
     eavsr::set_error("conv_wino6: hipFuncSetAttribute(%zu B of LDS): %s", C::LDS_BYTES, hipGetErrorString(attr_err));
@@ -1193,23 +1376,28 @@
   }
   const long per_cot = blocks < 256 ? blocks : 256;
   dim3 grid((unsigned)per_cot, eavsr::cdiv(d->cout, 64));
+  const W4Args& a0 = a;
   if (fuse) {
 #if EAVSR_LAB
     if constexpr (R == 3)
-      hipLaunchKernelGGL((conv_wino6_kernel<3, true>), grid, dim3(64 * NW), LDS_FUSE, eavsr::as_stream(stream), a);
+      hipLaunchKernelGGL((conv_wino6_kernel<3, true>), grid, dim3(64 * NW), LDS_FUSE, eavsr::as_stream(stream), a0);
 #endif
   } else {
     const bool grp_on = w6_grouped_schedule();
     if constexpr (R == 3) {
       if (grp_on && (d->cin / CK) % 2 == 0) {
-        if (d->res_scale != nullptr)
-          hipLaunchKernelGGL((conv_wino6_kernel<3, false, true, true>), grid, dim3(64 * NW), C::LDS_BYTES, eavsr::as_stream(stream), a);
+        if (fca_first)
+          hipLaunchKernelGGL((conv_wino6_kernel<3, false, true, false, true>), grid, dim3(64 * NW), C::LDS_BYTES_FCA, eavsr::as_stream(stream), a);
+        else if (fca_second)
+          hipLaunchKernelGGL((conv_wino6_kernel<3, false, true, true, true>), grid, dim3(64 * NW), C::LDS_BYTES_FCA, eavsr::as_stream(stream), a);
+        else if (d->res_scale != nullptr)
+          hipLaunchKernelGGL((conv_wino6_kernel<3, false, true, true>), grid, dim3(64 * NW), C::LDS_BYTES, eavsr::as_stream(stream), a0);
         else
-          hipLaunchKernelGGL((conv_wino6_kernel<3, false, true>), grid, dim3(64 * NW), C::LDS_BYTES, eavsr::as_stream(stream), a);
+          hipLaunchKernelGGL((conv_wino6_kernel<3, false, true>), grid, dim3(64 * NW), C::LDS_BYTES, eavsr::as_stream(stream), a0);
         return eavsr::launch_status("conv_wino6");
       }
     }
-    hipLaunchKernelGGL((conv_wino6_kernel<R, false>), grid, dim3(64 * NW), C::LDS_BYTES, eavsr::as_stream(stream), a);
+    hipLaunchKernelGGL((conv_wino6_kernel<R, false>), grid, dim3(64 * NW), C::LDS_BYTES, eavsr::as_stream(stream), a0);
   }
   return eavsr::launch_status("conv_wino6");
 }
diff --git a/eavsr_amd/csrc/conv_x9.hip b/eavsr_amd/csrc/conv_x9.hip
--- a/eavsr_amd/csrc/conv_x9.hip
+++ b/eavsr_amd/csrc/conv_x9.hip
@@ -285,7 +285,7 @@
   EAVSR_REQUIRE(d->n_src >= 1 && d->n_src <= 5, -1, "conv3x3_f32x9: n_src %d not in 1..5", d->n_src);
   EAVSR_REQUIRE(d->ksize == 3, -2, "conv3x3_f32x9: kernel size %d (3 only)", d->ksize);
   EAVSR_REQUIRE(d->out, -1, "conv3x3_f32x9: NULL out");
-  EAVSR_REQUIRE(d->out_shuffle == 0 && d->res_scale == nullptr && d->border_pieces == nullptr && d->sum_mul == nullptr, -2, "conv3x3_f32x9: the pixel-shuffle and scaled-residual epilogues exist in eavsr_conv3x3_wino4_f32 only");
+  EAVSR_REQUIRE(d->out_shuffle == 0 && d->res_scale == nullptr && d->border_pieces == nullptr && d->sum_mul == nullptr && !eavsr_desc_has_fca(d), -2, "conv3x3_f32x9: the pixel-shuffle and scaled-residual epilogues exist in eavsr_conv3x3_wino4_f32 only");
   EAVSR_REQUIRE(d->n >= 0 && d->h > 0 && d->w > 0 && d->cin > 0 && d->cout > 0, -1, "conv3x3_f32x9: bad dims");
   EAVSR_REQUIRE(d->act >= 0 && d->act <= 2, -1, "conv3x3_f32x9: act %d", d->act);
   EAVSR_REQUIRE(d->act != EAVSR_ACT_LRELU || (d->slope >= 0.f && d->slope <= 1.f), -2,
diff --git a/eavsr_amd/networks.py b/eavsr_amd/networks.py
--- a/eavsr_amd/networks.py
+++ b/eavsr_amd/networks.py
@@ -295,7 +295,12 @@
         if (RCAB_PRE and x.shape[1] == 64 and len(self.res) == 3 and isinstance(self.res[1], _Act) and self.res[1].kind == "relu"
                 and tuple(self.res[2].weight.shape) == (64, 64, 3, 3) and int(a.weight.shape[0]) <= 8):
             c1, c2 = self.res[0], self.res[2]
-            t, tpart, pieces = ops.conv2d(x, c1.weight, c1.bias, act="relu", chan_partial=True, border=True)
+            if RCAB_FUSED_CA:
+                t, tpart, pieces, mtile = ops.conv2d(x, c1.weight, c1.bias, act="relu", chan_partial=True, border=True, fca_next=c2.weight)
+                if mtile is not None:
+                    return ops.conv2d(t, c2.weight, c2.bias, residual=x, fca=(mtile, a.weight, a.bias, b.weight, b.bias))
+            else:
+                t, tpart, pieces = ops.conv2d(x, c1.weight, c1.bias, act="relu", chan_partial=True, border=True)
             if not RCAB_PRE_PIECES:
                 pieces = None
             scale = ops.ca_scale_pre(t, tpart, c2.weight, c2.bias, a.weight, a.bias, b.weight, b.bias, border=pieces)
@@ -311,6 +316,12 @@
 FUSE_CA_TAIL = _os.environ.get("EAVSR_FUSE_CA_TAIL", "0") == "1"
 RCAB_PRE = _os.environ.get("EAVSR_RCAB_PRE", "1") == "1"
 RCAB_PRE_PIECES = _os.environ.get("EAVSR_RCAB_PRE_PIECES", "1") == "1"
+RCAB_FUSED_CA = _os.environ.get("EAVSR_RCAB_FUSED_CA", "1") == "1"
+
+
+def set_rcab_fused_ca(on: bool) -> None:
+    global RCAB_FUSED_CA
+    RCAB_FUSED_CA = bool(on)
 
 
 def set_rcab_pre(on: bool) -> None:
diff --git a/eavsr_amd/ops.py b/eavsr_amd/ops.py
--- a/eavsr_amd/ops.py
+++ b/eavsr_amd/ops.py
@@ -531,11 +531,14 @@
 
 def conv2d(srcs, weight, bias=None, act=None, slope: float = 0.0, residual=None, chan_partial: bool = False, ca=None, ca_out: bool = False,
            pixel_shuffle2: bool = False, sigmoid_from=None, dgrad: bool = False, res_scale=None, border: bool = False, sum_mul=None,
-           precision: str = "fp32"):
+           precision: str = "fp32", fca_next=None, fca=None, fca_scale_out: bool = False):
+    box = [] if fca_next is not None else None
     r = _conv2d(srcs, weight, bias, act, slope, residual, chan_partial, ca, ca_out, pixel_shuffle2, sigmoid_from, dgrad, res_scale, border,
-                sum_mul, precision)
+                sum_mul, precision, fca_next, box, fca, fca_scale_out)
     if border and not (isinstance(r, tuple) and len(r) >= 2 and (r[-1] is None or isinstance(r[-1], BorderPieces))):
         r = (tuple(r) if isinstance(r, tuple) else (r,)) + (None,)
+    if box is not None:
+        r = (tuple(r) if isinstance(r, tuple) else (r,)) + (box[0] if box else None,)
     return r
 
 
@@ -544,7 +547,8 @@
            slope: float = 0.0, residual: Optional[Tensor] = None, chan_partial: bool = False,
            ca: Optional[Tuple[Tensor, Tensor]] = None, ca_out: bool = False, pixel_shuffle2: bool = False,
            sigmoid_from: Optional[int] = None, dgrad: bool = False, res_scale: Optional[Tensor] = None, border: bool = False,
-           sum_mul: Optional[Tensor] = None, precision: str = "fp32"):
+           sum_mul: Optional[Tensor] = None, precision: str = "fp32", fca_next: Optional[Tensor] = None, fca_box: Optional[list] = None,
+           fca=None, fca_scale_out: bool = False):
     check_precision(precision)
     if sum_mul is not None:
         if not dgrad or chan_partial or ca is not None or pixel_shuffle2 or sigmoid_from is not None or res_scale is not None or act == "relu_mask":
@@ -585,6 +589,14 @@
         res_scale = _chk(res_scale, "res_scale")
         if tuple(res_scale.shape) != (n, cout):
             raise ValueError(f"res_scale must be (n, cout) = ({n}, {cout})")
+    if fca is not None:
+        if (residual is None or chan_partial or border or ca is not None or pixel_shuffle2 or sigmoid_from is not None or dgrad
+                or res_scale is not None or act is not None or fca_next is not None or len(fca) != 5):
+            raise ValueError("fca=(mtile, w1, b1, w2, b2): with `residual`; no activation / channel sums / prologue / shuffle / res_scale")
+    elif fca_scale_out:
+        raise ValueError("fca_scale_out needs fca")
+    if fca_next is not None and (not chan_partial or ca is not None or pixel_shuffle2 or dgrad or res_scale is not None or sum_mul is not None):
+        raise ValueError("fca_next: the first convolution of an RCAB (chan_partial=True; no prologue / shuffle / res_scale / dgrad)")
     masked = act == "relu_mask"
     if masked and (residual is None or chan_partial or ca is not None or pixel_shuffle2 or sigmoid_from is not None):
         raise ValueError("act='relu_mask': residual = the ReLU's forward output; no channel sums / prologue / shuffle / sigmoid")
@@ -635,6 +647,13 @@
         use_wino = False
     if res_scale is not None and not (use_wino4 and cin % 8 == 0 and lib().eavsr_wino4_schedule() >= 1):
         return scale_residual(conv2d(srcs, weights, biases, act=act, slope=slope), res_scale, residual)
+    fca_route = (use_wino4 and k == 3 and cout == 64 and cin % 8 == 0 and ca is None and sum_mul is None and not dgrad
+                 and lib().eavsr_wino4_schedule() == 1)
+    fca_first = (fca_next is not None and fca_route and residual is None and tuple(fca_next.shape) == (64, 64, 3, 3)
+                 and fca_next.is_contiguous() and fca_next.dtype == torch.float32 and fca_next.data_ptr() % 16 == 0)
+    if fca is not None and not (fca_route and cin == 64 and 1 <= int(fca[1].shape[0]) <= 8):
+        raise ValueError("fca: this launch does not run the grouped F(4x4,3x3) kernel on 64 -> 64 channels with 1..8 hidden units "
+                         "(use ca_scale_pre + res_scale)")
     if pixel_shuffle2 and not (use_wino4 and FUSE_PIXEL_SHUFFLE):
         return torch.nn.functional.pixel_shuffle(conv2d(srcs, weights, biases, act=act, slope=slope), 2)
     use_wino5 = (CONV_MODE == "winograd4" and k == 5 and ca is None and not masked and w % 4 == 0 and out.data_ptr() % 8 == 0
@@ -654,7 +673,7 @@
     part = None
     if sum_mul is not None:
         part = torch.empty((n, lib().eavsr_conv3x3_x6s_tiles(h, w), cout), device=out.device, dtype=torch.float32)
-    if chan_partial:
+    if chan_partial and not fca_first:
         tiles = (lib().eavsr_conv3x3_x6s_tiles(h, w) if use_x6s else lib().eavsr_conv5x5_wino_tiles(h, w) if use_wino5 else lib().eavsr_conv3x3_wino4_tiles(h, w) if use_wino4 else _wino_tiles(h, w) if use_wino
                  else lib().eavsr_conv2d_tiles(n, h, w, k))
         part = torch.empty((n, tiles, cout), device=out.device, dtype=torch.float32)
@@ -679,7 +698,27 @@
     d.res_scale = _p(res_scale)
     d.sum_mul = _p(sum_mul)
     pieces = None
-    if (border and chan_partial and use_wino4 and cout == 64 and cin % 8 == 0 and ca is None and not pixel_shuffle2 and res_scale is None
+    fca_keep = None
+    if fca_first:
+        mtile = torch.empty((n, lib().eavsr_conv3x3_wino4_tiles(h, w), 64), device=out.device, dtype=torch.float32)
+        fca_keep = fca_next.detach()
+        d.fca_next_weight, d.fca_mtile = _p(fca_keep), _p(mtile)
+        fca_box.append(mtile)
+    scale_out = None
+    if fca is not None:
+        mtile = _chk(fca[0], "fca mtile")
+        if tuple(mtile.shape) != (n, lib().eavsr_conv3x3_wino4_tiles(h, w), 64):
+            raise ValueError("fca: mtile must be (n, tiles, 64) of this launch's shape")
+        fca_keep = [mtile] + [_chk(v.detach(), "fca param") for v in fca[1:]]
+        cr_ = int(fca_keep[1].shape[0])
+        if fca_keep[1].numel() != cr_ * 64 or fca_keep[2].numel() != cr_ or fca_keep[3].numel() != 64 * cr_ or fca_keep[4].numel() != 64:
+            raise ValueError("fca: w1 (cr, 64), b1 (cr), w2 (64, cr), b2 (64)")
+        d.fca_mtile, d.fca_w1, d.fca_b1, d.fca_w2, d.fca_b2 = (_p(v) for v in fca_keep)
+        d.fca_cr = cr_
+        if fca_scale_out:
+            scale_out = torch.empty((n, 64), device=out.device, dtype=torch.float32)
+            d.fca_scale_out = _p(scale_out)
+    if (border and chan_partial and not fca_first and use_wino4 and cout == 64 and cin % 8 == 0 and ca is None and not pixel_shuffle2 and res_scale is None
             and lib().eavsr_wino4_schedule() == 1):
         pr, pc = C.c_int32(0), C.c_int32(0)
         N.check(lib().eavsr_conv3x3_wino4_border_pieces(h, w, C.byref(pr), C.byref(pc)), "conv3x3_wino4_border_pieces")
@@ -728,7 +767,8 @@
         _launch(f"conv3x3_{cin}to{cout}_wino4" + ("_ca" if ca is not None else ""), 2.0 * cin * cout * 9 * px,
                 4.0 * px * (cin * (1 if ca is None else (3 if ca_out else 2)) + cout + (cout if residual is not None else 0)), out,
                 lambda: lib().eavsr_conv3x3_wino4_f32(C.byref(d), _p(wu), st), "conv3x3_wino4")
-        res = [out] + ([part] if chan_partial else []) + ([xs] if xs is not None else []) + ([pieces] if border else [])
+        res = ([out] + ([part] if chan_partial else []) + ([xs] if xs is not None else []) + ([pieces] if border else [])
+               + ([scale_out] if scale_out is not None else []))
         return res[0] if len(res) == 1 else tuple(res)
     if use_wino:
         wu = _packed_wino(weights)
diff --git a/include/eavsr_hip.h b/include/eavsr_hip.h
--- a/include/eavsr_hip.h
+++ b/include/eavsr_hip.h
@@ -92,6 +92,14 @@
   float* border_pieces;
   int32_t border_stride;
   const float* sum_mul;
+  const float* fca_next_weight;
+  float* fca_mtile;
+  const float* fca_w1;
+  const float* fca_b1;
+  const float* fca_w2;
+  const float* fca_b2;
+  float* fca_scale_out;
+  int32_t fca_cr;
 } eavsr_conv2d_desc;
 
 size_t eavsr_conv2d_desc_size(void);
```

After: 129.7. 3.7% lower.
